# 1chizhang/OpenDCVC

Measured on AMD Instinct MI355X. Metric: 1080p YUV420 encode+decode FPS (frames/s through encode AND decode, whole job), higher is better.
Workload: dtype f16

## Files before the change

include/dcvc_amd.h:

```cpp
#ifndef DCVC_AMD_H
#define DCVC_AMD_H

#include <stddef.h>
#include <stdint.h>

#ifdef __cplusplus
extern "C" {
#endif

#define DCVC_ABI_VERSION 1

enum {
    DCVC_F16 = 0,
    DCVC_F32 = 1,
    DCVC_U8 = 2,
    DCVC_U16 = 3
};

enum {
    DCVC_EPI_BIAS = 0,
    DCVC_EPI_BIAS_QUANT = 1,
    DCVC_EPI_SHUFFLE2 = 2,
    DCVC_EPI_WSILU = 3
};

int dcvc_abi_version(void);
const char* dcvc_last_error(void);
int dcvc_device_count(void);

typedef struct dcvc_dcb dcvc_dcb;
typedef struct dcvc_conv dcvc_conv;
int dcvc_dcb_create(int dtype, int cin, int c, int shortcut, const float* adaptor_w,
                    const float* adaptor_b, const float* w1, const float* b1, const float* wd,
                    const float* bd, const float* w2, const float* b2, const float* w3,
                    const float* b3, const float* w4, const float* b4, dcvc_dcb** out);
void dcvc_dcb_destroy(dcvc_dcb* h);
size_t dcvc_dcb_scratch_bytes(const dcvc_dcb* h, int H, int W);
int dcvc_dcb_forward(const dcvc_dcb* h, const void* x0, int64_t ld0, int c0, const void* x1,
                     int64_t ld1, int c1, int H, int W, const float* quant, void* out, int64_t ldo,
                     void* scratch, void* stream);
int dcvc_dcb_forward_chained(const dcvc_dcb* h, const void* x0, int64_t ld0, int c0, const void* x1,
                             int64_t ld1, int c1, int H, int W, const float* quant, void* out,
                             int64_t ldo, void* scratch, void* stream, int head_done, int a_slot,
                             const dcvc_dcb* next);

int dcvc_dcb_forward_then_conv(const dcvc_dcb* h, const void* x0, int64_t ld0, int c0, const void* x1,
                               int64_t ld1, int c1, int H, int W, void* scratch, void* stream,
                               int head_done, int a_slot, const dcvc_conv* conv, const float* conv_quant,
                               void* conv_out, int64_t ldco);

int dcvc_dcb_profile(const dcvc_dcb* h, const void* x0, int64_t ld0, int c0, int H, int W, void* out,
                     int64_t ldo, void* scratch, void* stream, int iters, float* head_ms, float* tail_ms);
int dcvc_dcb_profile_tail(const dcvc_dcb* h, const void* x0, int64_t ld0, int c0, int H, int W, void* out,
                          int64_t ldo, void* scratch, void* stream, int iters, float* tail_ms);

int dcvc_conv_create(int dtype, int cin, int cout, int kh, int kw, int stride, int pad, int epilogue,
                     const float* w, const float* b, dcvc_conv** out);
void dcvc_conv_destroy(dcvc_conv* h);
int dcvc_conv_forward(const dcvc_conv* h, const void* x0, int64_t ld0, int c0, const void* x1,
                      int64_t ld1, int c1, int H, int W, const float* quant, void* out, int64_t ldo,
                      void* stream);
int dcvc_conv_forward_scaled(const dcvc_conv* h, const void* x0, int64_t ld0, int c0, const void* x1,
                             int64_t ld1, int c1, int H, int W, const float* in_scale, const float* quant,
                             void* out, int64_t ldo, void* stream);

int dcvc_unshuffle8(int dtype, const void* x_nchw, int C, int H, int W, void* out_hwc, int64_t ldo,
                    void* stream);
int dcvc_shuffle8_clamp(int dtype, const void* x_hwc, int64_t ld, const float* bias, int C, int H,
                        int W, int do_clamp, void* out_nchw, void* stream);
int dcvc_yuv420_to_frame(int dtype, const uint8_t* y, const uint8_t* u, const uint8_t* v, int H, int W,
                         int pad_b, int pad_r, void* out_nchw, void* stream);
int dcvc_frame_to_yuv420(int dtype, const void* x_nchw, int Hp, int Wp, int H, int W, int round_uv,
                         uint8_t* y, uint8_t* u, uint8_t* v, void* stream);
int dcvc_rgb_to_frame(int dtype, const uint8_t* rgb, int H, int W, int pad_b, int pad_r, void* out_nchw,
                      void* stream);
int dcvc_frame_to_rgb(int dtype, const void* x_nchw, int Hp, int Wp, int H, int W, void* out_chw, void* stream);
int dcvc_replicate_pad_hwc(int dtype, const void* x, int64_t ldx, int H, int W, int C, int pad_b,
                           int pad_r, void* out, int64_t ldo, void* stream);
int dcvc_scale_channels(int dtype, const void* x, int64_t ldx, const float* q, int64_t P, int C,
                        void* out, int64_t ldo, void* stream);
int dcvc_copy_channels(int dtype, const void* x, int64_t ldx, int64_t P, int C, void* out,
                       int64_t ldo, void* stream);
int dcvc_crop_hwc(int dtype, const void* x, int64_t ldx, int W, int H2, int W2, int C, void* out,
                  int64_t ldo, void* stream);

int dcvc_round_z(int dtype, void* z, int64_t ld, int H, int W, int C, int8_t* z_chw, void* stream);
int dcvc_z_from_int8(int dtype, const int8_t* z_chw, int H, int W, int C, void* out, int64_t ldo,
                     void* stream);

int dcvc_prior_enc_step(int dtype, int n_groups, int step, int q_mode, const void* y, int64_t ldy,
                        const void* qsrc, int64_t ldq, const void* scales, int64_t lds_,
                        const void* means, int64_t ldm, int H, int W, int C, float thres,
                        const void* yhat_in, int64_t ldhi, void* yhat_out, int64_t ldho,
                        int16_t* packed_chw, void* stream);
int dcvc_prior_dec_index(int dtype, int n_groups, int step, const void* scales, int64_t lds_, int H,
                         int W, int C, float thres, uint8_t* idx_chw, void* stream);
int dcvc_prior_dec_restore(int dtype, int n_groups, int step, const int8_t* sym_chw,
                           const void* means, int64_t ldm, int H, int W, int C, const void* yhat_in,
                           int64_t ldhi, void* yhat_out, int64_t ldho, void* stream);
int64_t dcvc_prior_dec_compact_ws_bytes(int H, int W, int C, int n_groups);
int dcvc_prior_dec_index_compact(int dtype, int n_groups, int step, const void* scales, int64_t lds_, int H, int W, int C,
                                 float thres, uint8_t* idx_chw, void* workspace, uint8_t* idx_host,
                                 int32_t* count_host, void* stream);
int dcvc_prior_dec_restore_compact(int dtype, int n_groups, int step, const int8_t* sym_host, const uint8_t* idx_chw,
                                   void* workspace, const void* means, int64_t ldm, int H, int W, int C,
                                   const void* yhat_in, int64_t ldhi, void* yhat_out, int64_t ldho, void* stream);
int dcvc_prior_dec_index_compact_dev(int dtype, int n_groups, int step, const void* scales, int64_t lds_, int H, int W, int C,
                                     float thres, uint8_t* idx_chw, void* workspace, uint8_t* idx_dev,
                                     int32_t* count_dev, void* stream);
int dcvc_prior_dec_restore_compact_dev(int dtype, int n_groups, int step, const int8_t* sym_dev, const uint8_t* idx_chw,
                                       void* workspace, const void* means, int64_t ldm, int H, int W, int C,
                                       const void* yhat_in, int64_t ldhi, void* yhat_out, int64_t ldho, void* stream);
int dcvc_prior_finish(int dtype, int q_mode, void* yhat, int64_t ldh, const void* qsrc, int64_t ldq,
                      int H, int W, int C, void* stream);

int dcvc_op_process_with_mask(int dtype, const void* y, const void* scales, const void* means,
                              const void* mask, float thres, void* y_res, void* y_q, void* y_hat,
                              void* s_hat, int64_t n, void* stream);
int dcvc_op_combine_for_reading_2x(int dtype, void* out, const void* x, const void* mask,
                                   int64_t half_n, void* stream);
int dcvc_op_restore_y_2x(int dtype, void* out, const void* y, const void* means, const void* mask,
                         int64_t half_n, void* stream);
int dcvc_op_restore_y_4x(int dtype, void* out, const void* y, const void* means, const void* mask,
                         int64_t quarter_n, void* stream);
int dcvc_op_build_index_dec(int dtype, uint8_t* out, uint8_t* cond_out, const void* scales,
                            float scale_min, float scale_max, float log_scale_min,
                            float log_step_recip, float skip_thres, int64_t n, void* stream);
int dcvc_op_build_index_enc(int dtype, int16_t* out, uint8_t* cond_out, const void* symbols,
                            const void* scales, float scale_min, float scale_max,
                            float log_scale_min, float log_step_recip, float skip_thres, int64_t n,
                            void* stream);
int dcvc_op_round_and_to_int8(int dtype, void* z, int8_t* z_int8, int64_t n, void* stream);
int dcvc_op_clamp_reciprocal_with_quant(int dtype, const void* q_dec, void* y, float min_val,
                                        void* q_out, int64_t n, void* stream);
int dcvc_op_add_and_multiply(int dtype, void* x0, const void* x1, const void* q, int64_t n,
                             void* stream);
int dcvc_op_bias_quant(int dtype, void* x, const void* bias, const void* quant, int C, int64_t HW,
                       void* stream);
int dcvc_op_bias_pixel_shuffle_8(int dtype, void* out, const void* x, const void* bias, int C, int H,
                                 int W, int do_clamp, void* stream);
int dcvc_op_replicate_pad(int dtype, const void* x, int C, int H, int W, int pad_b, int pad_r,
                          void* out, void* stream);
int dcvc_op_bias_wsilu_depthwise_conv2d(int dtype, const void* x, const void* weight,
                                        const void* bias, int C, int H, int W, void* out,
                                        void* stream);
int dcvc_nchw_to_hwc(int dtype, const void* x, int C, int64_t HW, void* out, int64_t ldo, void* stream);
int dcvc_hwc_to_nchw(int dtype, const void* x, int64_t ldx, int C, int64_t HW, void* out, void* stream);

typedef struct dcvc_rans_enc dcvc_rans_enc;
typedef struct dcvc_rans_dec dcvc_rans_dec;
dcvc_rans_enc* dcvc_rans_enc_create(void);
void dcvc_rans_enc_destroy(dcvc_rans_enc*);
int dcvc_rans_enc_add_cdf(dcvc_rans_enc*, const int32_t* cdf, int n, int stride,
                          const int32_t* sizes, const int32_t* offsets);
int dcvc_rans_enc_empty_cdf(dcvc_rans_enc*);
void dcvc_rans_enc_set_use_two(dcvc_rans_enc*, int two);
int dcvc_rans_enc_reset(dcvc_rans_enc*);
int dcvc_rans_enc_encode_y(dcvc_rans_enc*, const int16_t* symbols, int64_t n, int group);
int dcvc_rans_enc_encode_y_borrowed(dcvc_rans_enc*, const int16_t* symbols, int64_t n, int group);
int dcvc_rans_enc_encode_z(dcvc_rans_enc*, const int8_t* symbols, int64_t n, int group,
                           int start_offset, int per_channel_size);
int dcvc_rans_enc_flush(dcvc_rans_enc*);
int64_t dcvc_rans_enc_get_stream(dcvc_rans_enc*, const uint8_t** data);

dcvc_rans_dec* dcvc_rans_dec_create(void);
void dcvc_rans_dec_destroy(dcvc_rans_dec*);
int dcvc_rans_dec_add_cdf(dcvc_rans_dec*, const int32_t* cdf, int n, int stride,
                          const int32_t* sizes, const int32_t* offsets);
int dcvc_rans_dec_empty_cdf(dcvc_rans_dec*);
void dcvc_rans_dec_set_use_two(dcvc_rans_dec*, int two);
int dcvc_rans_dec_set_stream(dcvc_rans_dec*, const uint8_t* data, int64_t n);
int dcvc_rans_dec_decode_y(dcvc_rans_dec*, const uint8_t* indexes, int64_t n, int group);
int dcvc_rans_dec_decode_z(dcvc_rans_dec*, int64_t total, int group, int start_offset,
                           int per_channel_size);
int64_t dcvc_rans_dec_get(dcvc_rans_dec*, int8_t* out, int64_t capacity);
int dcvc_rans_dec_decode_and_get_y(dcvc_rans_dec*, const uint8_t* indexes, int64_t n, int group,
                                   int8_t* out);
int dcvc_rans_dec_decode_compact(dcvc_rans_dec*, const uint8_t* indexes, int64_t count, int group, int8_t* out);
int dcvc_rans_dec_check_end(dcvc_rans_dec*);
int64_t dcvc_rans_chunked_encode_y(dcvc_rans_enc*, const int16_t* symbols, int64_t count, int group, int log2_s,
                                   uint8_t* out, int64_t capacity);
int dcvc_rans_chunked_decode_y(dcvc_rans_dec*, const uint8_t* unit, int64_t unit_bytes, const uint8_t* indexes,
                               int64_t count, int group, int log2_s, int8_t* out);
int dcvc_pmf_to_quantized_cdf(const float* pmf, int n, int precision, uint32_t* out);

void* dcvc_host_alloc(size_t bytes);
void dcvc_host_free(void* p);
void* dcvc_host_device_ptr(void* host);
#define DCVC_COMPACT_BLOCKS 256
int dcvc_compact_symbols(const int16_t* packed, int n_per_part, int n_parts, int16_t* out_host, int32_t* counts_host,
                         int32_t* workspace, void* stream);
int dcvc_compact_symbols_dev(const int16_t* packed, int n_per_part, int n_parts, int16_t* out_dev, int32_t* counts_dev,
                             int32_t* workspace, void* stream);
#define DCVC_RANS_DEV_E_COUNT 1
#define DCVC_RANS_DEV_E_TABLE 2
#define DCVC_RANS_DEV_E_CHUNK 4
#define DCVC_RANS_DEV_E_RANGE 8
typedef struct dcvc_rans_dev dcvc_rans_dev;
int dcvc_rans_dev_create(const int32_t* cdf, int n, int stride, const int32_t* sizes, const int32_t* offsets,
                         dcvc_rans_dev** out);
void dcvc_rans_dev_destroy(dcvc_rans_dev*);
int64_t dcvc_rans_dev_enc_ws_bytes(int64_t max_symbols, int log2_s, int slot_bytes);
// ... 48 lines not shown
```

opendcvc_amd/_lib.py:

```python
import ctypes
import os
import subprocess
from ctypes import (POINTER, c_char_p, c_double, c_float, c_int, c_int8, c_int16, c_int32, c_int64, c_size_t,
                    c_uint8, c_uint32, c_uint64, c_void_p)

_HERE = os.path.dirname(os.path.abspath(__file__))
LIB_PATH = os.path.join(_HERE, os.environ.get("DCVC_AMD_LIB") or
                        ("libdcvc_amd_diag.so" if os.environ.get("DCVC_AMD_DIAG") else "libdcvc_amd.so"))

F16, F32 = 0, 1
U8 = 2
U16 = 3
SSE_BLOCKS = 1024
DIGEST_PASS_WORDS = 1 << 20
EPI_BIAS, EPI_BIAS_QUANT, EPI_SHUFFLE2, EPI_WSILU = 0, 1, 2, 3


class DcvcError(RuntimeError):
    pass


class DigestMismatch(DcvcError):

    def __init__(self, index, is_i, expected, got):
        super().__init__(f"frame {index} ({'I' if is_i else 'P'}): the decoder's reference state has digest {got:#018x}, "
                         f"the stream carries {expected:#018x}")
        self.index, self.is_i, self.expected, self.got = index, is_i, expected, got


def build(force=False):
    csrc = os.path.join(_HERE, "csrc")
    if force:
        subprocess.check_call(["make", "-C", csrc, "clean"])
    subprocess.check_call(["make", "-C", csrc, "-j8"])
    return LIB_PATH


_P = c_void_p
_I = c_int
_L = c_int64
_F = c_float

_SIGS = {
    "dcvc_abi_version": (_I, []),
    "dcvc_last_error": (c_char_p, []),
    "dcvc_device_count": (_I, []),
    "dcvc_dcb_create": (_I, [_I, _I, _I, _I] + [_P] * 12 + [POINTER(_P)]),
    "dcvc_dcb_destroy": (None, [_P]),
    "dcvc_dcb_scratch_bytes": (c_size_t, [_P, _I, _I]),
    "dcvc_dcb_forward": (_I, [_P, _P, _L, _I, _P, _L, _I, _I, _I, _P, _P, _L, _P, _P]),
    "dcvc_dcb_forward_chained": (_I, [_P, _P, _L, _I, _P, _L, _I, _I, _I, _P, _P, _L, _P, _P, _I, _I, _P]),
    "dcvc_dcb_forward_then_conv": (_I, [_P, _P, _L, _I, _P, _L, _I, _I, _I, _P, _P, _I, _I, _P, _P, _P, _L]),
    "dcvc_dcb_profile": (_I, [_P, _P, _L, _I, _I, _I, _P, _L, _P, _P, _I, POINTER(c_float), POINTER(c_float)]),
    "dcvc_dcb_profile_tail": (_I, [_P, _P, _L, _I, _I, _I, _P, _L, _P, _P, _I, POINTER(c_float)]),
    "dcvc_conv_create": (_I, [_I, _I, _I, _I, _I, _I, _I, _I, _P, _P, POINTER(_P)]),
    "dcvc_conv_destroy": (None, [_P]),
    "dcvc_conv_forward": (_I, [_P, _P, _L, _I, _P, _L, _I, _I, _I, _P, _P, _L, _P]),
    "dcvc_conv_forward_scaled": (_I, [_P, _P, _L, _I, _P, _L, _I, _I, _I, _P, _P, _P, _L, _P]),
    "dcvc_unshuffle8": (_I, [_I, _P, _I, _I, _I, _P, _L, _P]),
    "dcvc_shuffle8_clamp": (_I, [_I, _P, _L, _P, _I, _I, _I, _I, _P, _P]),
    "dcvc_yuv420_to_frame": (_I, [_I, _P, _P, _P, _I, _I, _I, _I, _P, _P]),
    "dcvc_frame_to_yuv420": (_I, [_I, _P, _I, _I, _I, _I, _I, _P, _P, _P, _P]),
    "dcvc_rgb_to_frame": (_I, [_I, _P, _I, _I, _I, _I, _P, _P]),
    "dcvc_frame_to_rgb": (_I, [_I, _P, _I, _I, _I, _I, _P, _P]),
    "dcvc_replicate_pad_hwc": (_I, [_I, _P, _L, _I, _I, _I, _I, _I, _P, _L, _P]),
    "dcvc_scale_channels": (_I, [_I, _P, _L, _P, _L, _I, _P, _L, _P]),
    "dcvc_copy_channels": (_I, [_I, _P, _L, _L, _I, _P, _L, _P]),
    "dcvc_crop_hwc": (_I, [_I, _P, _L, _I, _I, _I, _I, _P, _L, _P]),
    "dcvc_round_z": (_I, [_I, _P, _L, _I, _I, _I, _P, _P]),
    "dcvc_z_from_int8": (_I, [_I, _P, _I, _I, _I, _P, _L, _P]),
    "dcvc_prior_enc_step": (_I, [_I, _I, _I, _I, _P, _L, _P, _L, _P, _L, _P, _L, _I, _I, _I, _F, _P, _L, _P, _L, _P, _P]),
    "dcvc_prior_dec_index": (_I, [_I, _I, _I, _P, _L, _I, _I, _I, _F, _P, _P]),
    "dcvc_prior_dec_restore": (_I, [_I, _I, _I, _P, _P, _L, _I, _I, _I, _P, _L, _P, _L, _P]),
    "dcvc_prior_dec_compact_ws_bytes": (_L, [_I, _I, _I, _I]),
    "dcvc_prior_dec_index_compact": (_I, [_I, _I, _I, _P, _L, _I, _I, _I, _F, _P, _P, _P, _P, _P]),
    "dcvc_prior_dec_restore_compact": (_I, [_I, _I, _I, _P, _P, _P, _P, _L, _I, _I, _I, _P, _L, _P, _L, _P]),
    "dcvc_prior_finish": (_I, [_I, _I, _P, _L, _P, _L, _I, _I, _I, _P]),
    "dcvc_op_process_with_mask": (_I, [_I, _P, _P, _P, _P, _F, _P, _P, _P, _P, _L, _P]),
    "dcvc_op_combine_for_reading_2x": (_I, [_I, _P, _P, _P, _L, _P]),
    "dcvc_op_restore_y_2x": (_I, [_I, _P, _P, _P, _P, _L, _P]),
    "dcvc_op_restore_y_4x": (_I, [_I, _P, _P, _P, _P, _L, _P]),
    "dcvc_op_build_index_dec": (_I, [_I, _P, _P, _P, _F, _F, _F, _F, _F, _L, _P]),
    "dcvc_op_build_index_enc": (_I, [_I, _P, _P, _P, _P, _F, _F, _F, _F, _F, _L, _P]),
    "dcvc_op_round_and_to_int8": (_I, [_I, _P, _P, _L, _P]),
    "dcvc_op_clamp_reciprocal_with_quant": (_I, [_I, _P, _P, _F, _P, _L, _P]),
    "dcvc_op_add_and_multiply": (_I, [_I, _P, _P, _P, _L, _P]),
    "dcvc_op_bias_quant": (_I, [_I, _P, _P, _P, _I, _L, _P]),
    "dcvc_op_bias_pixel_shuffle_8": (_I, [_I, _P, _P, _P, _I, _I, _I, _I, _P]),
    "dcvc_op_replicate_pad": (_I, [_I, _P, _I, _I, _I, _I, _I, _P, _P]),
    "dcvc_op_bias_wsilu_depthwise_conv2d": (_I, [_I, _P, _P, _P, _I, _I, _I, _P, _P]),
    "dcvc_nchw_to_hwc": (_I, [_I, _P, _I, _L, _P, _L, _P]),
    "dcvc_hwc_to_nchw": (_I, [_I, _P, _L, _I, _L, _P, _P]),
    "dcvc_rans_enc_create": (_P, []),
    "dcvc_rans_enc_destroy": (None, [_P]),
    "dcvc_rans_enc_add_cdf": (_I, [_P, _P, _I, _I, _P, _P]),
    "dcvc_rans_enc_empty_cdf": (_I, [_P]),
    "dcvc_rans_enc_set_use_two": (None, [_P, _I]),
    "dcvc_rans_enc_reset": (_I, [_P]),
    "dcvc_rans_enc_encode_y": (_I, [_P, _P, _L, _I]),
    "dcvc_rans_enc_encode_y_borrowed": (_I, [_P, _P, _L, _I]),
    "dcvc_rans_enc_encode_z": (_I, [_P, _P, _L, _I, _I, _I]),
    "dcvc_rans_enc_flush": (_I, [_P]),
    "dcvc_rans_enc_get_stream": (_L, [_P, POINTER(_P)]),
    "dcvc_rans_dec_create": (_P, []),
    "dcvc_rans_dec_destroy": (None, [_P]),
    "dcvc_rans_dec_add_cdf": (_I, [_P, _P, _I, _I, _P, _P]),
    "dcvc_rans_dec_empty_cdf": (_I, [_P]),
    "dcvc_rans_dec_set_use_two": (None, [_P, _I]),
    "dcvc_rans_dec_set_stream": (_I, [_P, _P, _L]),
    "dcvc_rans_dec_decode_y": (_I, [_P, _P, _L, _I]),
    "dcvc_rans_dec_decode_z": (_I, [_P, _L, _I, _I, _I]),
    "dcvc_rans_dec_get": (_L, [_P, _P, _L]),
    "dcvc_rans_dec_decode_and_get_y": (_I, [_P, _P, _L, _I, _P]),
    "dcvc_rans_dec_decode_compact": (_I, [_P, _P, _L, _I, _P]),
    "dcvc_rans_dec_check_end": (_I, [_P]),
    "dcvc_pmf_to_quantized_cdf": (_I, [_P, _I, _I, _P]),
    "dcvc_rans_chunked_encode_y": (_L, [_P, _P, _L, _I, _I, _P, _L]),
    "dcvc_rans_chunked_decode_y": (_I, [_P, _P, _L, _P, _L, _I, _I, _P]),
    "dcvc_rans_dev_create": (_I, [_P, _I, _I, _P, _P, POINTER(_P)]),
    "dcvc_rans_dev_destroy": (None, [_P]),
    "dcvc_rans_dev_enc_ws_bytes": (_L, [_L, _I, _I]),
    "dcvc_rans_dev_encode_y": (_I, [_P, _P, _P, _L, _I, _I, _P, _P, _L, _P]),
    "dcvc_rans_dev_dec_ws_bytes": (_L, [_L, _I]),
    "dcvc_rans_dev_decode_y": (_I, [_P, _P, _L, _P, _P, _P, _L, _I, _P, _P, _P, _P]),
    "dcvc_prior_dec_index_compact_dev": (_I, [_I, _I, _I, _P, _L, _I, _I, _I, _F, _P, _P, _P, _P, _P]),
    "dcvc_prior_dec_restore_compact_dev": (_I, [_I, _I, _I, _P, _P, _P, _P, _L, _I, _I, _I, _P, _L, _P, _L, _P]),
    "dcvc_compact_symbols_dev": (_I, [_P, _I, _I, _P, _P, _P, _P]),
    "dcvc_host_alloc": (_P, [c_size_t]),
    "dcvc_host_free": (None, [_P]),
    "dcvc_host_device_ptr": (_P, [_P]),
    "dcvc_compact_symbols": (_I, [_P, _I, _I, _P, _P, _P, _P]),
    "dcvc_frame_to_yuv420_planes": (_I, [_I, _P, _I, _I, _I, _I, _P, _P, _P, _P]),
    "dcvc_sse": (_I, [_I, _P, _I, _P, _L, _P, _P, _P]),
    "dcvc_msssim_ws_bytes": (_L, [_I, _I]),
    "dcvc_msssim_stats": (_I, [_I, _P, _I, _P, _I, _I, c_double, _P, _P, POINTER(_I), _P]),
    "dcvc_planes_to_frame": (_I, [_I, _I, _I, _I, _I, _P, _P, _P, _L, _L, _I, _I, _I, _I, _P, _P]),
    "dcvc_frame_to_planes": (_I, [_I, _I, _I, _I, _I, _P, _I, _I, _I, _I, _P, _P, _P, _L, _L, _P]),
    "dcvc_frame_to_metric_planes": (_I, [_I, _I, _I, _P, _I, _I, _I, _I, _P, _P, _P, _P]),
    "dcvc_resize_frame": (_I, [_I, _P, _I, _I, _I, _I, _P, _I, _I, _I, _I, _P, _P, _I, _P, _P, _I, _P]),
    "dcvc_frame_analysis_ws_bytes": (_L, [_I, _I]),
    "dcvc_frame_analyze": (_I, [_I, _P, _L, _I, _I, _P, _P, _P, _P, _P]),
    "dcvc_rate_estimate_ws_bytes": (_L, [_I, _I, _I]),
    "dcvc_rate_estimate": (_I, [_P, _I, _I, _P, _I, _I, _P, _I, _I, _P, _I, _I, _I, _P, _P, _P]),
    "dcvc_state_digest_ws_bytes": (_L, [_L]),
    "dcvc_state_digest": (_I, [_P, _L, _P, c_uint64, _I, _P, _P]),
    "dcvc_copy_f32": (_I, [_P, _P, _I, _P]),
    "dcvc_memcpy_d2h": (_I, [_P, _P, c_size_t, _P]),
    "dcvc_memcpy_h2d": (_I, [_P, _P, c_size_t, _P]),
    "dcvc_stream_sync": (_I, [_P]),
}

EXPORTS = tuple(_SIGS.keys())
_lib = None


def lib():
    global _lib
    if _lib is None:
        if not os.path.exists(LIB_PATH):
            raise DcvcError(
                f"{LIB_PATH} not found: the HIP extension has not been built "
                "(run `python -c 'import __graft_entry__ as g; g.build()'` or `make -C opendcvc_amd/csrc`). "
                "There is no CPU fallback.")
        try:
            L = ctypes.CDLL(LIB_PATH)
        except OSError as e:
            raise DcvcError(f"cannot load {LIB_PATH}: {e}") from e
        for name, (res, args) in _SIGS.items():
            try:
                fn = getattr(L, name)
            except AttributeError as e:
                raise DcvcError(f"{LIB_PATH} does not export {name}") from e
            fn.restype = res
            fn.argtypes = args
        if L.dcvc_abi_version() != 1:
            raise DcvcError("libdcvc_amd.so ABI version mismatch")
        _lib = L
    return _lib


def check(rc, what=""):
    if rc is not None and rc < 0:
        msg = lib().dcvc_last_error()
        raise DcvcError(f"{what} failed ({rc}): {msg.decode() if msg else ''}")
    return rc


def require_gpu():
    n = lib().dcvc_device_count()
    if n <= 0:
        raise DcvcError("no HIP device visible: the DCVC-RT hot path needs an MI355X (no CPU fallback)")
    return n
```

opendcvc_amd/csrc/dcb_t128.hpp:

```cpp
#pragma once

namespace t128 {

typedef float floatx16 __attribute__((ext_vector_type(16)));

constexpr int TW = 16, TH = 8, M = TW * TH;
constexpr int NW = 8, NTHR = NW * 64;
constexpr int PT = M / 32;
constexpr int PTW = PT / 2;
constexpr int PAD = 8;
constexpr int VC = 64, LDV = VC + PAD;
constexpr int HALO = (TH + 2) * (TW + 2);
constexpr int DW_SLAB = 64;
constexpr int LDS_S = DW_SLAB;

constexpr int PADF = 24;

struct G128 {
    static constexpr int TW = t128::TW, TH = t128::TH, NW = t128::NW, D = 8, DW_SLAB = t128::DW_SLAB, WPS = 2;
};
struct G32 {
    static constexpr int TW = 8, TH = 4, NW = 4, D = 24 , DW_SLAB = 128, WPS = 1;
};
template <class G>
struct Geo : G {
    static constexpr int M = G::TW * G::TH, NTHR = G::NW * 64;
    static constexpr int PTW = (M / 32) / (G::NW / 4);
    static constexpr int HALO = (G::TH + 2) * (G::TW + 2);
    static constexpr int LDS_S = G::DW_SLAB;
    static_assert(M % 32 == 0 && PTW >= 1 && G::NW % 4 == 0, "tile geometry");
};

template <int C>
struct Wcfg {
    static_assert(C % 64 == 0, "DepthConvBlock widths are padded to 64");
    static constexpr int NT = C / 32;
    static constexpr int NTW = (NT + 3) / 4;
    static constexpr bool RAG = NT % 4 != 0;
    static constexpr int KS = C / 16;
    static constexpr int NCH = 2 * C / VC;
    static constexpr int F4 = 4 * NTW;
    static constexpr int LDX = C + PAD;
    static constexpr int FRAGS = KS * NTW + NCH * KS + NCH * F4;
    static constexpr int STREAM = FRAGS + PADF;
};

template <int C, class G = G128, bool HEADIN = false>
struct Cfg : Wcfg<C> {
    using GE = Geo<G>;
    using WC = Wcfg<C>;
    using WC::NT; using WC::NTW; using WC::RAG; using WC::KS; using WC::NCH; using WC::F4; using WC::LDX; using WC::FRAGS; using WC::STREAM;
    static_assert(C % G::DW_SLAB == 0, "whole depthwise slabs");
    static constexpr int D = G::D;
    static_assert(D <= PADF, "stream padding");
    static constexpr size_t slab_elems = (size_t)(HEADIN && C / G::DW_SLAB > 2 ? C / G::DW_SLAB : 2) * GE::HALO * GE::LDS_S;
    static constexpr size_t v_elems = (size_t)2 * GE::M * LDV > slab_elems ? (size_t)2 * GE::M * LDV : slab_elems;
    static constexpr size_t TAB_BYTES = (size_t)9 * C * 2 + (size_t)C * 4 + (size_t)4 * C * 4;
    static constexpr int HROWS = (GE::HALO + 31) / 32 * 32;
    static constexpr size_t HEAD_BYTES = HEADIN ? (size_t)HROWS * LDX * sizeof(half_t) : 0;
    static constexpr size_t LDS = ((size_t)GE::M * LDX + v_elems) * sizeof(half_t) + TAB_BYTES + HEAD_BYTES;
    static_assert(LDS <= 160 * 1024, "LDS budget");
    static_assert(NCH % 2 == 0 && NCH >= 4, "the chunk loop is unrolled by two");
    static_assert((2 * C) % VC == 0, "whole FFN chunks");
    static constexpr int OFF_U0 = (KS * NTW) % D;
    static constexpr int OFF_S0 = (OFF_U0 + KS) % D;
    static constexpr int OFF_ODD = (OFF_S0 + KS) % D;
    static constexpr int OFF_EVEN = (OFF_ODD + F4 + KS) % D;
    static_assert((2 * (F4 + KS)) % D == 0, "the two-step loop body must turn the ring a whole number of times");
    static constexpr int OFF_LAST = OFF_ODD;
    static constexpr int OFF_FIN = (OFF_LAST + F4) % D;
};

__device__ __forceinline__ floatx16 mfma32(const half8& a, const half8& b, const floatx16& c)
{
    return __builtin_amdgcn_mfma_f32_32x32x16_f16(a, b, c, 0, 0, 0);
}


template <int C, class G = G128, bool HEADIN = false>
__global__ __launch_bounds__(Geo<G>::NTHR, G::WPS) void dcb_tail128_kernel(TailParams p)
{
    using TR = Traits<half_t>;
    using CF = Cfg<C, G, HEADIN>;
    using GE = Geo<G>;
    constexpr int TW = GE::TW, TH = GE::TH, M = GE::M, NTHR = GE::NTHR, PTW = GE::PTW, HALO = GE::HALO, DW_SLAB = GE::DW_SLAB,
                  LDS_S = GE::LDS_S;
    constexpr int NTW = CF::NTW, KS = CF::KS, NCH = CF::NCH, D = CF::D, LDX = CF::LDX, V = 8, GC = C / V;
    extern __shared__ __attribute__((aligned(32))) char smem[];
    half_t* bufX = reinterpret_cast<half_t*>(smem);
    half_t* bufV = bufX + M * LDX;
    half_t* tabW = bufV + CF::v_elems;
    float* tabBd = reinterpret_cast<float*>(tabW + 9 * C);
    float* tabB3 = tabBd + C;
    const int tid = threadIdx.x, lane = tid & 63;
    const int wave = __builtin_amdgcn_readfirstlane(tid >> 6);
    const int cqw = wave & 3, ph = wave >> 2;
    const int pl = lane & 31, hh = lane >> 5;
    const int tiles_x = (p.W + TW - 1) / TW;
    const int ty0 = (blockIdx.x / tiles_x) * TH, tx0 = (blockIdx.x % tiles_x) * TW;
    const half_t* a = reinterpret_cast<const half_t*>(p.a);
    const half_t* ident = reinterpret_cast<const half_t*>(p.ident);
    [[maybe_unused]] unsigned long long ts0 = 0, ts1 = 0, ts2 = 0, ts3 = 0, ts4 = 0, ts5 = 0, ts6 = 0;
    [[maybe_unused]] unsigned long long td[8] = {0, 0, 0, 0, 0, 0, 0, 0};
    STAMP(ts0);

    const __amdgpu_buffer_rsrc_t wrsrc = __builtin_amdgcn_make_buffer_rsrc(
        const_cast<char*>(reinterpret_cast<const char*>(p.wt)) + (size_t)cqw * CF::STREAM * 1024, 0, CF::STREAM * 1024, 0x00020000);
    const int wlane = lane * 16;
    int woff = 0;
    auto wload = [&]() __attribute__((always_inline)) {
        typedef unsigned u32x4 __attribute__((ext_vector_type(4)));
        const u32x4 v = __builtin_amdgcn_raw_buffer_load_b128(wrsrc, wlane, woff, 0);
        woff += 1024;
        return __builtin_bit_cast(half8, v);
    };
    half8 ring[D];

    constexpr int HW_ = TW + 2, GS = DW_SLAB / V, NLD = (HALO * GS + NTHR - 1) / NTHR;
    constexpr int nslab = C / DW_SLAB;
    const half_t* wd = reinterpret_cast<const half_t*>(p.wd);
    const int dcs = (tid % GS) * V;
    typedef unsigned u32x4 __attribute__((ext_vector_type(4)));
    constexpr int OOB = 0x7FFFFFF0;
    const __amdgpu_buffer_rsrc_t arsrc = __builtin_amdgcn_make_buffer_rsrc(
        const_cast<half_t*>(a), 0, (int)((long)p.H * p.W * p.lda * 2), 0x00020000);
    int hoff[NLD];
#pragma unroll
    for (int k = 0; k < NLD; ++k) {
        const int hp = tid / GS + k * (NTHR / GS);
        const int y = ty0 - 1 + hp / HW_, x = tx0 - 1 + hp % HW_;
        hoff[k] = (hp < HALO && y >= 0 && y < p.H && x >= 0 && x < p.W) ? ((y * p.W + x) * (int)p.lda + dcs) * 2 : OOB;
#ifdef DCVC_DIAG
        if (p.ablate & 32) hoff[k] = (tid & 255) * 16;
#endif
    }
    Vec16 pre[nslab][NLD];
    auto fetch = [&](int slab) __attribute__((always_inline)) {
#pragma unroll
        for (int k = 0; k < NLD; ++k)
            pre[slab][k] = __builtin_bit_cast(Vec16, __builtin_amdgcn_raw_buffer_load_b128(arsrc, hoff[k], slab * DW_SLAB * 2, 0));
    };
    Vec16 wtap[9];
    floatx4 bd0, bd1;
    auto taps_fetch = [&](int slab) __attribute__((always_inline)) {
        const int c = slab * DW_SLAB + dcs;
#pragma unroll
        for (int t = 0; t < 9; ++t) wtap[t] = *reinterpret_cast<const Vec16*>(tabW + t * C + c);
        bd0 = *reinterpret_cast<const floatx4*>(tabBd + c);
        bd1 = *reinterpret_cast<const floatx4*>(tabBd + c + 4);
    };
    if constexpr (!HEADIN) fetch(0);
    {
        constexpr int NW16 = 9 * C * 2 / 16, NB16 = C * 4 / 16, N316 = 4 * C * 4 / 16;
        for (int i = tid; i < NW16 + NB16 + N316; i += NTHR) {
            const Vec16* src = i < NW16 ? reinterpret_cast<const Vec16*>(wd) + i
                               : i < NW16 + NB16 ? reinterpret_cast<const Vec16*>(p.bd) + (i - NW16)
                                                 : reinterpret_cast<const Vec16*>(p.b3) + (i - NW16 - NB16);
            reinterpret_cast<Vec16*>(tabW)[i] = *src;
        }
    }
    if constexpr (!HEADIN) {
#pragma unroll
        for (int sl = 1; sl < nslab; ++sl) fetch(sl);
    }
    if constexpr (HEADIN) {
        constexpr int HROWS = CF::HROWS, HT = HROWS / 32, NLX = (HROWS * GC + NTHR - 1) / NTHR;
        half_t* xs = reinterpret_cast<half_t*>(reinterpret_cast<char*>(tabW) + CF::TAB_BYTES);
        const __amdgpu_buffer_rsrc_t xrsrc = __builtin_amdgcn_make_buffer_rsrc(
            const_cast<void*>(p.hx), 0, (int)((long)p.H * p.W * p.ldhx * 2), 0x00020000);
        Vec16 xv[NLX];
#pragma unroll
        for (int k = 0; k < NLX; ++k) {
            const int it = tid + k * NTHR, hp = it / GC, c = (it % GC) * V;
            const int y = ty0 - 1 + hp / HW_, x = tx0 - 1 + hp % HW_;
            const int off = (hp < HALO && y >= 0 && y < p.H && x >= 0 && x < p.W) ? ((y * p.W + x) * (int)p.ldhx + c) * 2 : OOB;
            xv[k] = __builtin_bit_cast(Vec16, __builtin_amdgcn_raw_buffer_load_b128(xrsrc, off, 0, 0));
        }
        const __amdgpu_buffer_rsrc_t hrsrc = __builtin_amdgcn_make_buffer_rsrc(
            const_cast<char*>(reinterpret_cast<const char*>(p.hwt)) + (size_t)cqw * (KS * NTW + PADF) * 1024, 0,
            (KS * NTW + PADF) * 1024, 0x00020000);
        constexpr int NF = KS * NTW, HD = NF < D ? NF : D;
        int hoff = 0;
        auto hload = [&]() __attribute__((always_inline)) {
            typedef unsigned u32x4h __attribute__((ext_vector_type(4)));
            const u32x4h v = __builtin_amdgcn_raw_buffer_load_b128(hrsrc, wlane, hoff, 0);
            hoff += 1024;
            return __builtin_bit_cast(half8, v);
        };
#pragma unroll
        for (int k = 0; k < HD; ++k) ring[k] = hload();
#pragma unroll
        for (int k = 0; k < NLX; ++k) {
            const int it = tid + k * NTHR, hp = it / GC, c = (it % GC) * V;
            if (hp < HROWS) *reinterpret_cast<Vec16*>(xs + hp * LDX + c) = xv[k];
        }
        __syncthreads();
        floatx16 hacc[NTW][HT];
#pragma unroll
        for (int s = 0; s < KS; ++s) {
            half8 hb_[HT];
#pragma unroll
            for (int t = 0; t < HT; ++t) hb_[t] = *reinterpret_cast<const half8*>(xs + (32 * t + pl) * LDX + 8 * hh + 16 * s);
#pragma unroll
            for (int i = 0; i < NTW; ++i) {
                const int f = s * NTW + i, k = f % HD;
#pragma unroll
                for (int t = 0; t < HT; ++t) {
                    if (s == 0) {
                        floatx16 zero;
#pragma unroll
                        for (int r = 0; r < 16; ++r) zero[r] = 0.f;
                        hacc[i][t] = mfma32(ring[k], hb_[t], zero);
                    } else {
                        hacc[i][t] = mfma32(ring[k], hb_[t], hacc[i][t]);
                    }
                }
                if (f + HD < NF) ring[k] = hload();
            }
        }
#pragma unroll
        for (int i = 0; i < NTW; ++i) {
            const int chb = 32 * (cqw + 4 * i) + 4 * hh;
#pragma unroll
            for (int g = 0; g < 4; ++g) {
                const floatx4 bias = load_f4(p.hb1 + chb + 8 * g);
#pragma unroll
                for (int t = 0; t < HT; ++t) {
                    const int hp = 32 * t + pl;
                    const int y = ty0 - 1 + hp / HW_, x = tx0 - 1 + hp % HW_;
                    const bool inside = hp < HALO && y >= 0 && y < p.H && x >= 0 && x < p.W;
                    floatx4 v = {hacc[i][t][4 * g], hacc[i][t][4 * g + 1], hacc[i][t][4 * g + 2], hacc[i][t][4 * g + 3]};
                    v = v + bias;
#pragma unroll
// ... 158 lines not shown
#pragma unroll
        for (int g = 0; g < 4; ++g) {
            const floatx4 bias = ebias_get(p.b2, i, g);
#pragma unroll
            for (int t = 0; t < PTW; ++t) {
                floatx4 v = {acc[i][t][4 * g], acc[i][t][4 * g + 1], acc[i][t][4 * g + 2], acc[i][t][4 * g + 3]};
                lds_store_quad<half_t>(bufX, LDX, prow + 32 * t, chb + 8 * g, v + bias);
            }
        }
    }
    __syncthreads();
#pragma unroll
    for (int k = 0; k < NID; ++k) {
        int m, icg;
        idmap(k, m, icg);
        const half8 o = __builtin_bit_cast(half8, lds_load_vec<half_t>(bufX, LDX, m, icg)) + __builtin_bit_cast(half8, idv[k]);
        lds_store_vec<half_t>(bufX, LDX, m, icg, __builtin_bit_cast(Vec16, o));
    }
    __syncthreads();

    STAMP(ts3);
#pragma unroll
    for (int i = 0; i < NTW; ++i)
#pragma unroll
        for (int t = 0; t < PTW; ++t)
#pragma unroll
            for (int r = 0; r < 16; ++r) acc[i][t][r] = 0.f;
    floatx16 ua[PTW], ub[PTW];
    const float* b3w = tabB3 + 16 * cqw + 4 * hh;
    floatx16 biasv;
    auto bias_load = [&](int j) __attribute__((always_inline)) {
        j = j < NCH ? j : NCH - 1;
        const floatx4 l0 = load_f4(b3w + 64 * j), l1 = load_f4(b3w + 64 * j + 8);
        const floatx4 h0 = load_f4(b3w + 64 * j + 2 * C), h1 = load_f4(b3w + 64 * j + 2 * C + 8);
#pragma unroll
        for (int r = 0; r < 4; ++r) {
            biasv[r] = l0[r];
            biasv[4 + r] = l1[r];
            biasv[8 + r] = h0[r];
            biasv[12 + r] = h1[r];
        }
    };
    constexpr int NPIECE = 4 * PTW * 6;
    float ge[4], gr[4];
    floatx4 vq;
    auto gate_piece = [&](const floatx16 (&u)[PTW], half_t* vbuf, int i) __attribute__((always_inline)) {
        const int n = i / 6, phs = i % 6, t = n >> 2, g = (n >> 1) & 1, hf = n & 1;
        const float lo0 = u[t][4 * g + 2 * hf], lo1 = u[t][4 * g + 2 * hf + 1];
        const float hi0 = u[t][8 + 4 * g + 2 * hf], hi1 = u[t][8 + 4 * g + 2 * hf + 1];
        if (phs == 0) {
            ge[0] = __builtin_amdgcn_exp2f(lo0);
            ge[1] = __builtin_amdgcn_exp2f(lo1);
        } else if (phs == 1) {
            ge[2] = __builtin_amdgcn_exp2f(hi0);
            ge[3] = __builtin_amdgcn_exp2f(hi1);
        } else if (phs == 2) {
            gr[0] = __builtin_amdgcn_rcpf(1.0f + ge[0]);
            gr[1] = __builtin_amdgcn_rcpf(1.0f + ge[1]);
        } else if (phs == 3) {
            gr[2] = __builtin_amdgcn_rcpf(1.0f + ge[2]);
            gr[3] = __builtin_amdgcn_rcpf(1.0f + ge[3]);
        } else if (phs == 4) {
            vq[2 * hf] = DCVC_FMAF(hi0, gr[2], lo0 * gr[0]);
        } else {
            vq[2 * hf + 1] = DCVC_FMAF(hi1, gr[3], lo1 * gr[1]);
            if (hf == 1) lds_store_quad<half_t>(vbuf, LDV, prow + 32 * t, 16 * cqw + 8 * g + 4 * hh, vq);
        }
    };
    auto wload_ffn = [&]() __attribute__((always_inline)) {
#ifdef DCVC_DIAG
        if (p.ablate & 256) {
            typedef unsigned u32x4 __attribute__((ext_vector_type(4)));
            return __builtin_bit_cast(half8, __builtin_amdgcn_raw_buffer_load_b128(wrsrc, wlane, 0, 0));
        }
#endif
        return wload();
    };
    auto step = [&](auto G4c, auto G3c, auto GATEc, auto OFFc, const floatx16 (&ug)[PTW], floatx16 (&un)[PTW], half_t* vcur,
                    const half_t* vprev, int jb) __attribute__((always_inline)) {
        constexpr bool G4 = decltype(G4c)::value, G3 = decltype(G3c)::value, GATE = decltype(GATEc)::value;
        constexpr int OFF = decltype(OFFc)::value;
        constexpr int N4 = G4 ? 4 : 0, NS = N4 + (G3 ? KS : 0);
        constexpr int TM = N4 * NTW * PTW + (G3 ? KS * PTW : 0);
        constexpr int PPS = GATE ? (NPIECE + TM - 1) / TM : 0;
        auto load_b1 = [&](int idx, int t) __attribute__((always_inline)) {
#ifdef DCVC_DIAG
            if (p.ablate & 512) idx = idx < N4 ? 0 : N4;
#endif
            if (idx < N4) return *reinterpret_cast<const half8*>(vprev + (prow + 32 * t) * LDV + 8 * hh + idx * 16);
            return bfrag_x(t, idx - N4);
        };
        half8 bc[PTW], bn[PTW];
#pragma unroll
        for (int t = 0; t < PTW; ++t) bc[t] = load_b1(0, t);
        __builtin_amdgcn_sched_barrier(0);
        int m = 0;
#pragma unroll
        for (int idx = 0; idx < NS; ++idx) {
            const int nm = idx < N4 ? NTW * PTW : PTW;
#pragma unroll
            for (int q = 0; q < NTW * PTW; ++q) {
                if (q < nm) {
                    if (idx + 1 < NS && q < PTW) bn[q] = load_b1(idx + 1, q);
                    const int t = q % PTW;
                    if (idx < N4) {
                        const int i = q / PTW, k = (OFF + idx * NTW + i) % D;
                        acc[i][t] = mfma32(ring[k], bc[t], acc[i][t]);
                        if (t == PTW - 1) ring[k] = wload_ffn();
                    } else {
                        const int k = (OFF + N4 * NTW + (idx - N4)) % D;
                        un[t] = mfma32(ring[k], bc[t], idx == N4 ? biasv : un[t]);
                        if (t == PTW - 1) ring[k] = wload_ffn();
                        if (idx == N4 && t == PTW - 1) bias_load(jb);
                    }
                    if constexpr (GATE) {
#ifdef DCVC_DIAG
                        if (!(p.ablate & 64))
#endif
#pragma unroll
                        for (int pp = 0; pp < PPS; ++pp)
                            if (m * PPS + pp < NPIECE) gate_piece(ug, vcur, m * PPS + pp);
                    }
                    ++m;
                    __builtin_amdgcn_sched_barrier(0);
                }
            }
#pragma unroll
            for (int t = 0; t < PTW; ++t) bc[t] = bn[t];
        }
#ifdef DCVC_DIAG
        if (p.ablate & 128) return;
#endif
        if constexpr (GATE) __syncthreads();
    };
    using T_ = std::true_type;
    using F_ = std::false_type;
    half_t* vA = bufV;
    half_t* vB = bufV + M * LDV;
#define T128_OFF(x) std::integral_constant<int, CF::x>{}
    bias_load(0);
    step(F_{}, T_{}, F_{}, T128_OFF(OFF_U0), ub, ua, vA, vB, 1);
    STAMP(ts4);
    step(F_{}, T_{}, T_{}, T128_OFF(OFF_S0), ua, ub, vA, vB, 2);
    for (int j = 1; j + 2 < NCH; j += 2) {
        step(T_{}, T_{}, T_{}, T128_OFF(OFF_ODD), ub, ua, vB, vA, j + 2);
        step(T_{}, T_{}, T_{}, T128_OFF(OFF_EVEN), ua, ub, vA, vB, j + 3);
    }
    step(T_{}, F_{}, T_{}, T128_OFF(OFF_LAST), ub, ua, vB, vA, 0);
    ebias_load(p.b4);
    step(T_{}, F_{}, F_{}, T128_OFF(OFF_FIN), ub, ua, vA, vB, 0);
#undef T128_OFF

    STAMP(ts5);
    const bool fused_next = p.nwt != nullptr;
    const __amdgpu_buffer_rsrc_t nrsrc = __builtin_amdgcn_make_buffer_rsrc(
        const_cast<char*>(reinterpret_cast<const char*>(fused_next ? p.nwt : p.wt)) + (size_t)cqw * (KS * NTW + PADF) * 1024, 0,
        (KS * NTW + PADF) * 1024, 0x00020000);
    int noff = 0;
    auto nload = [&]() __attribute__((always_inline)) {
        typedef unsigned u32x4_ __attribute__((ext_vector_type(4)));
        const u32x4_ v = __builtin_amdgcn_raw_buffer_load_b128(nrsrc, wlane, noff, 0);
        noff += 1024;
        return __builtin_bit_cast(half8, v);
    };
    if (fused_next) {
#pragma unroll
        for (int k = 0; k < D; ++k) ring[k] = nload();
    }
#pragma unroll
    for (int i = 0; i < NTW; ++i) {
        if (!tile_exists(i)) continue;
        const int chb = 32 * tile_of(i) + 4 * hh;
#pragma unroll
        for (int g = 0; g < 4; ++g) {
            const floatx4 bias = ebias_get(p.b4, i, g);
#pragma unroll
            for (int t = 0; t < PTW; ++t) {
                const floatx4 o = lds_load_quad<half_t>(bufX, LDX, prow + 32 * t, chb + 8 * g);
                floatx4 v = {acc[i][t][4 * g], acc[i][t][4 * g + 1], acc[i][t][4 * g + 2], acc[i][t][4 * g + 3]};
                lds_store_quad<half_t>(bufX, LDX, prow + 32 * t, chb + 8 * g, (v + bias) + o);
            }
        }
    }
    __syncthreads();
    half_t* out = reinterpret_cast<half_t*>(p.out);
    if (out != nullptr) {
#pragma unroll
        for (int k = 0; k < NID; ++k) {
            int m, icg;
            idmap(k, m, icg);
            const int y = ty0 + m / TW, x = tx0 + m % TW;
            if (y < p.H && x < p.W) {
                const long pix = (long)y * p.W + x;
                float r[V];
                unpack16<half_t>(lds_load_vec<half_t>(bufX, LDX, m, icg), r);
                if (p.shortcut) {
                    float id[V];
                    unpack16<half_t>(*reinterpret_cast<const Vec16*>(ident + pix * p.ldi + icg), id);
#pragma unroll
                    for (int j = 0; j < V; ++j) r[j] = r[j] + id[j];
                }
                if (p.q != nullptr) {
#pragma unroll
                    for (int j = 0; j < V; ++j) r[j] = r[j] * ((icg + j) < p.c_log ? p.q[icg + j] : 1.0f);
                }
                *reinterpret_cast<Vec16*>(out + pix * p.ldo + icg) = pack16<half_t>(r);
            }
        }
    }
    STAMP(ts6);
#ifdef DCVC_DIAG
    if (p.stamps && tid == 0) {
        unsigned long long* o = p.stamps + (size_t)blockIdx.x * 16;
#pragma unroll
        for (int k = nslab + 1; k <= 4; ++k) td[k] = td[nslab < 4 ? nslab : 4];
        o[0] = ts1 - ts0;
        o[1] = ts2 - ts1;
        o[2] = ts3 - ts2;
        o[3] = ts4 - ts3;
        o[4] = ts5 - ts4;
        o[5] = ts6 - ts5;
        o[6] = ts0;
        o[7] = ts6;
        o[8] = td[0] - ts0;
        o[9] = td[1] - td[0];
        o[10] = td[2] - td[1];
        o[11] = td[3] - td[2];
        o[12] = td[4] - td[3];
        o[13] = ts1 - td[4];
    }
#endif
    if (fused_next) {
        gemm_c(nload);
        __syncthreads();
#pragma unroll
        for (int i = 0; i < NTW; ++i) {
            if (!tile_exists(i)) continue;
            const int chb = 32 * tile_of(i) + 4 * hh;
#pragma unroll
            for (int g = 0; g < 4; ++g) {
                const int ch0 = chb + 8 * g;
                const floatx4 bias = load_f4(p.nb1 + ch0);
                floatx4 qv = {1.f, 1.f, 1.f, 1.f};
                if (p.nplain && p.nq != nullptr) {
#pragma unroll
                    for (int r = 0; r < 4; ++r) qv[r] = (ch0 + r) < p.n_log ? p.nq[ch0 + r] : 1.0f;
                }
#pragma unroll
                for (int t = 0; t < PTW; ++t) {
                    floatx4 v = {acc[i][t][4 * g], acc[i][t][4 * g + 1], acc[i][t][4 * g + 2], acc[i][t][4 * g + 3]};
                    v = v + bias;
                    if (p.nplain) {
                        if (p.nq != nullptr) v = v * qv;
                    } else {
#pragma unroll
                        for (int r = 0; r < 4; ++r) v[r] = TR::gate(v[r]);
                    }
                    lds_store_quad<half_t>(bufX, LDX, prow + 32 * t, ch0, v);
                }
            }
        }
        __syncthreads();
        half_t* na = reinterpret_cast<half_t*>(p.na_out);
#pragma unroll
        for (int k = 0; k < NID; ++k) {
            int m, icg;
            idmap(k, m, icg);
            const int y = ty0 + m / TW, x = tx0 + m % TW;
            if (y < p.H && x < p.W)
                *reinterpret_cast<Vec16*>(na + ((long)y * p.W + x) * p.nlda + icg) = lds_load_vec<half_t>(bufX, LDX, m, icg);
        }
    }
#ifdef DCVC_DIAG
    if (p.stamps && tid == 0) {
        unsigned long long ts7 = 0;
        STAMP(ts7);
        p.stamps[(size_t)blockIdx.x * 16 + 14] = ts7 - ts6;
    }
#endif
}

template <int C, class G = G128>
struct HeadCfg {
    using CF = Wcfg<C>;
    static constexpr int DH = 4 * CF::NTW;
    static constexpr int KCH = 128;
    static constexpr int LDS_S = KCH + PAD;
    static constexpr size_t LDS = ((size_t)Geo<G>::M * LDS_S + (size_t)Geo<G>::M * CF::LDX) * sizeof(half_t);
};

template <int C, bool ADAPT, class G = G128>
__global__ __launch_bounds__(Geo<G>::NTHR, 1) void dcb_head128_kernel(HeadParams p)
{
    using TR = Traits<half_t>;
    using CF = Wcfg<C>;
    using HC = HeadCfg<C, G>;
    using GE = Geo<G>;
    constexpr int TW = GE::TW, TH = GE::TH, M = GE::M, NTHR = GE::NTHR, PTW = GE::PTW;
    constexpr int RPP = NTHR / 8, NPASS = M / RPP;
    static_assert(M % RPP == 0, "staging passes");
    constexpr int NTW = CF::NTW, KS = CF::KS, LDX = CF::LDX, V = 8, DH = HC::DH, KCH = HC::KCH, LDS_S = HC::LDS_S, G8 = C / 64;
    extern __shared__ __attribute__((aligned(32))) char smem[];
    half_t* bufY = reinterpret_cast<half_t*>(smem);
    half_t* bufS = bufY + M * LDX;
    const int tid = threadIdx.x, lane = tid & 63;
    const int wave = __builtin_amdgcn_readfirstlane(tid >> 6);
    const int cqw = wave & 3, ph = wave >> 2;
    const int pl = lane & 31, hh = lane >> 5;
    const int tiles_x = (p.W + TW - 1) / TW;
    const int ty0 = (blockIdx.x / tiles_x) * TH, tx0 = (blockIdx.x % tiles_x) * TW;
    const int prow = (ph * PTW) * 32 + pl;
    typedef unsigned u32x4 __attribute__((ext_vector_type(4)));
    constexpr int OOB = 0x7FFFFFF0;
    auto tile_of = [&](int i) __attribute__((always_inline)) { return cqw + 4 * i; };
    auto tile_exists = [&](int i) __attribute__((always_inline)) { return !CF::RAG || cqw + 4 * i < CF::NT; };

    int pix2[NPASS];
#pragma unroll
    for (int k = 0; k < NPASS; ++k) {
        const int m = (tid >> 3) + RPP * k;
        const int y = ty0 + m / TW, x = tx0 + m % TW;
        pix2[k] = (y < p.H && x < p.W) ? y * p.W + x : -1;
    }
    auto make_stream = [&](const void* base, int frags) __attribute__((always_inline)) {
        return __builtin_amdgcn_make_buffer_rsrc(
            const_cast<char*>(reinterpret_cast<const char*>(base)) + (size_t)cqw * (frags + PADF) * 1024, 0, (frags + PADF) * 1024,
            0x00020000);
    };
    floatx16 acc[NTW][PTW];
    half8 ring[DH];
    auto zero_all = [&]() __attribute__((always_inline)) {
#pragma unroll
        for (int i = 0; i < NTW; ++i)
#pragma unroll
            for (int t = 0; t < PTW; ++t)
#pragma unroll
                for (int r = 0; r < 16; ++r) acc[i][t][r] = 0.f;
    };
    auto gemm = [&](const half_t* X, int ldx, int nb, auto next) __attribute__((always_inline)) {
        const half_t* xb = X + prow * ldx + 8 * hh;
        half8 bc[PTW], bn[PTW];
#pragma unroll
        for (int t = 0; t < PTW; ++t) bc[t] = *reinterpret_cast<const half8*>(xb + t * 32 * ldx);
        __builtin_amdgcn_sched_barrier(0);
        for (int b = 0; b < nb; ++b) {
#pragma unroll
            for (int ss = 0; ss < 4; ++ss) {
                const int sn = (ss < 3 || b + 1 < nb) ? 4 * b + ss + 1 : 4 * b + ss;
#pragma unroll
                for (int q = 0; q < NTW * PTW; ++q) {
                    const int i = q / PTW, t = q % PTW, k = ss * NTW + i;
                    if (q < PTW) bn[q] = *reinterpret_cast<const half8*>(xb + q * 32 * ldx + sn * 16);
                    acc[i][t] = mfma32(ring[k], bc[t], acc[i][t]);
                    if (t == PTW - 1) ring[k] = next();
                    __builtin_amdgcn_sched_barrier(0);
                }
#pragma unroll
                for (int t = 0; t < PTW; ++t) bc[t] = bn[t];
            }
        }
    };
    auto store_tile = [&](void* g, long ldg) __attribute__((always_inline)) {
        half_t* gp = reinterpret_cast<half_t*>(g);
#pragma unroll
        for (int k = 0; k < NPASS * G8; ++k) {
            const int m = (tid >> 3) + RPP * (k / G8), c = ((tid & 7) + 8 * (k % G8)) * V;
            const int px = pix2[k / G8];
            if (px >= 0) *reinterpret_cast<Vec16*>(gp + (long)px * ldg + c) = *reinterpret_cast<const Vec16*>(bufY + m * LDX + c);
        }
    };
    auto epilogue = [&](const float* bias_p, bool gate) __attribute__((always_inline)) {
#pragma unroll
        for (int i = 0; i < NTW; ++i) {
            if (!tile_exists(i)) continue;
            const int chb = 32 * tile_of(i) + 4 * hh;
#pragma unroll
            for (int g = 0; g < 4; ++g) {
                const floatx4 bias = load_f4(bias_p + chb + 8 * g);
#pragma unroll
                for (int t = 0; t < PTW; ++t) {
                    floatx4 v = {acc[i][t][4 * g], acc[i][t][4 * g + 1], acc[i][t][4 * g + 2], acc[i][t][4 * g + 3]};
                    v = v + bias;
                    if (gate) {
#pragma unroll
                        for (int r = 0; r < 4; ++r) v[r] = TR::gate(v[r]);
                    }
                    lds_store_quad<half_t>(bufY, LDX, prow + 32 * t, chb + 8 * g, v);
                }
            }
        }
    };

    const __amdgpu_buffer_rsrc_t wrs = make_stream(p.w1128, KS * NTW);
    int woff = lane * 16;
    auto wnext = [&]() __attribute__((always_inline)) {
        const u32x4 v = __builtin_amdgcn_raw_buffer_load_b128(wrs, woff, 0, 0);
        woff += 1024;
        return __builtin_bit_cast(half8, v);
    };
    zero_all();
    if constexpr (ADAPT) {
        const int Kin = p.src.c0 + p.src.c1;
        const __amdgpu_buffer_rsrc_t ars = make_stream(p.wa128, (Kin / 16) * NTW);
        int aoff = lane * 16;
        auto anext = [&]() __attribute__((always_inline)) {
            const u32x4 v = __builtin_amdgcn_raw_buffer_load_b128(ars, aoff, 0, 0);
            aoff += 1024;
            return __builtin_bit_cast(half8, v);
        };
        const __amdgpu_buffer_rsrc_t rs0 = __builtin_amdgcn_make_buffer_rsrc(
            const_cast<void*>(p.src.x0), 0, (int)((long)p.H * p.W * p.src.ld0 * 2), 0x00020000);
        const __amdgpu_buffer_rsrc_t rs1 = __builtin_amdgcn_make_buffer_rsrc(
            const_cast<void*>(p.src.c1 > 0 ? p.src.x1 : p.src.x0), 0, (int)((long)p.H * p.W * (p.src.c1 > 0 ? p.src.ld1 : p.src.ld0) * 2),
            0x00020000);
        const int n0 = (p.src.c0 + KCH - 1) / KCH, nchunk = n0 + (p.src.c1 + KCH - 1) / KCH;
        u32x4 pre[2 * NPASS];
        auto fetch = [&](int i) __attribute__((always_inline)) {
            const bool s1 = i >= n0;
            const int cb = (s1 ? i - n0 : i) * KCH;
            const int left = (s1 ? p.src.c1 : p.src.c0) - cb, cnt = left < KCH ? left : KCH;
            const int ld = (int)(s1 ? p.src.ld1 : p.src.ld0);
#pragma unroll
            for (int k = 0; k < 2 * NPASS; ++k) {
                const int c = ((tid & 7) + 8 * (k & 1)) * V, px = pix2[k >> 1];
// ... 319 lines not shown
```

opendcvc_amd/csrc/dcvc_nn.hip:

```cpp
#include <algorithm>
#include <cstdio>
#include <cstdlib>
#include <functional>
#include <memory>
#include <mutex>
#include <type_traits>
#include <unordered_map>
#include <vector>

#include "common.hpp"
#include "gemm_core.hpp"

namespace {

using dcvc::round_up;

template <int MT>
struct Tile {
    static constexpr int M = 16 * MT;
    static constexpr int TW = MT >= 8 ? 16 : 8;
    static constexpr int TH = M / TW;
};

#ifndef DCVC_PF_SMALL
#define DCVC_PF_SMALL 4
#endif
template <typename T, int MT = 4>
struct Pf {
    static constexpr int value = (sizeof(T) == 2 && MT == 2) ? DCVC_PF_SMALL : 2;
};

struct SrcPair {
    const void* x0;
    long ld0;
    int c0;
    const void* x1;
    long ld1;
    int c1;
};

template <typename T>
__device__ __forceinline__ Vec16 load_src(const SrcPair& s, long pix, int c, bool valid)
{
    Vec16 v = VEC16_ZERO;
    if (valid) {
        if (c < s.c0)
            v = *reinterpret_cast<const Vec16*>(reinterpret_cast<const T*>(s.x0) + pix * s.ld0 + c);
        else
            v = *reinterpret_cast<const Vec16*>(reinterpret_cast<const T*>(s.x1) + pix * s.ld1 + (c - s.c0));
    }
    return v;
}

__device__ __forceinline__ floatx4 load_f4(const float* p) { return *reinterpret_cast<const floatx4*>(p); }

template <typename T>
__device__ __forceinline__ Vec16 scale_vec(const Vec16& v, const float* __restrict__ q, int c, int qn)
{
    constexpr int V = Traits<T>::kVec;
    float f[V];
    unpack16<T>(v, f);
#pragma unroll
    for (int j = 0; j < V; ++j) f[j] = f[j] * ((c + j) < qn ? q[c + j] : 1.0f);
    return pack16<T>(f);
}

struct HeadParams {
    SrcPair src;
    int H, W, C;
    const void* wa;
    const float* ba;
    void* ident;
    long ldi;
    const void* w1;
    const float* b1;
    void* a_out;
    long lda;
    int split;
    const void* wa128;
    const void* w1128;
};

template <typename T, int MT, int NTW, bool ADAPT>
__global__ __launch_bounds__(NTHREADS) void dcb_head_kernel(HeadParams p)
{
    using TR = Traits<T>;
    using frag_t = typename TR::frag_t;
    constexpr int M = Tile<MT>::M, TW = Tile<MT>::TW, TH = Tile<MT>::TH, V = TR::kVec, PF = Pf<T, MT>::value;
    extern __shared__ __attribute__((aligned(32))) char smem[];
    const int tid = threadIdx.x, lane = tid & 63, wave = tid >> 6;
    const int Kin = p.src.c0 + p.src.c1;
    const int C = p.C;
    const bool split = ADAPT && p.split;
    const int kstage = split ? (p.src.c0 > p.src.c1 ? p.src.c0 : p.src.c1) : Kin;
    const int ldx = (kstage > C ? kstage : C) + TR::kPad;
    const int ldy = C + TR::kPad;
    T* bufX = reinterpret_cast<T*>(smem);
    T* bufY = bufX + M * ldx;

    const int tiles_x = (p.W + TW - 1) / TW;
    const int ty0 = (blockIdx.x / tiles_x) * TH, tx0 = (blockIdx.x % tiles_x) * TW;

    auto stage = [&](int cbeg, int cnt) {
        const int G = cnt / V;
        for (int it = tid; it < M * G; it += NTHREADS) {
            const int m = it / G, c = (it - m * G) * V;
            const int y = ty0 + m / TW, x = tx0 + m % TW;
            const bool valid = (y < p.H) && (x < p.W);
            lds_store_vec<T>(bufX, ldx, m, c, load_src<T>(p.src, (long)y * p.W + x, cbeg + c, valid));
        }
    };
    stage(0, split ? p.src.c0 : Kin);
    __syncthreads();

    int tiles[NTW];
#pragma unroll
    for (int i = 0; i < NTW; ++i) tiles[i] = wave + NWAVE * i;
    const int pl = lane & 15, cq = (lane >> 4) * 4;
    floatx4 acc[MT][NTW];
    const int GC = C / V;

    if (ADAPT) {
        zero_acc(acc);
        if (split) {
            gemm_acc<T, MT, NTW, PF>(acc, bufX, ldx, p.src.c0 / KG, reinterpret_cast<const frag_t*>(p.wa), Kin / KG, 0, tiles, lane);
            __syncthreads();
            stage(p.src.c0, p.src.c1);
            __syncthreads();
            gemm_acc<T, MT, NTW, PF>(acc, bufX, ldx, p.src.c1 / KG, reinterpret_cast<const frag_t*>(p.wa), Kin / KG, p.src.c0 / KG, tiles, lane);
        } else {
            gemm_acc<T, MT, NTW, PF>(acc, bufX, ldx, Kin / KG, reinterpret_cast<const frag_t*>(p.wa), Kin / KG, 0, tiles, lane);
        }
#pragma unroll
        for (int i = 0; i < NTW; ++i) {
            const int ch0 = tiles[i] * 16 + cq;
            const floatx4 bias = load_f4(p.ba + ch0);
#pragma unroll
            for (int m = 0; m < MT; ++m) lds_store_quad<T>(bufY, ldy, m * 16 + pl, ch0, acc[m][i] + bias);
        }
        __syncthreads();
        for (int it = tid; it < M * GC; it += NTHREADS) {
            const int m = it / GC, c = (it - m * GC) * V;
            const int y = ty0 + m / TW, x = tx0 + m % TW;
            if (y < p.H && x < p.W)
                *reinterpret_cast<Vec16*>(reinterpret_cast<T*>(p.ident) + ((long)y * p.W + x) * p.ldi + c) =
                    lds_load_vec<T>(bufY, ldy, m, c);
        }
    }

    zero_acc(acc);
    if (ADAPT)
        gemm_acc<T, MT, NTW, PF>(acc, bufY, ldy, C / KG, reinterpret_cast<const frag_t*>(p.w1), C / KG, 0, tiles, lane);
    else
        gemm_acc<T, MT, NTW, PF>(acc, bufX, ldx, Kin / KG, reinterpret_cast<const frag_t*>(p.w1), Kin / KG, 0, tiles, lane);
    if (!ADAPT) __syncthreads();
#pragma unroll
    for (int i = 0; i < NTW; ++i) {
        const int ch0 = tiles[i] * 16 + cq;
        const floatx4 bias = load_f4(p.b1 + ch0);
#pragma unroll
        for (int m = 0; m < MT; ++m) {
            floatx4 v = acc[m][i] + bias;
#pragma unroll
            for (int r = 0; r < 4; ++r) v[r] = TR::gate(v[r]);
            lds_store_quad<T>(bufX, ldx, m * 16 + pl, ch0, v);
        }
    }
    __syncthreads();
    for (int it = tid; it < M * GC; it += NTHREADS) {
        const int m = it / GC, c = (it - m * GC) * V;
        const int y = ty0 + m / TW, x = tx0 + m % TW;
        if (y < p.H && x < p.W)
            *reinterpret_cast<Vec16*>(reinterpret_cast<T*>(p.a_out) + ((long)y * p.W + x) * p.lda + c) =
                lds_load_vec<T>(bufX, ldx, m, c);
    }
}

struct TailParams {
    const void* a;
    long lda;
    const void* ident;
    long ldi;
    int H, W, C, c_log;
    const void* wd;
    const float* bd;
    const void* w2;
    const float* b2;
    const void* w3;
    const float* b3;
    const void* w4;
    const float* b4;
    int shortcut;
    const float* q;
    void* out;
    long ldo;
    const void* nw1;
    const float* nb1;
    void* na_out;
    long nlda;
    int nplain;
    const float* nq;
    int n_log;
    const void* hx;
    long ldhx;
    const void* hw1;
    const float* hb1;
    const void* hwt;
    const void* wt;
    const void* nwt;
    int ablate;
    unsigned long long* stamps;
};

#ifdef DCVC_DIAG
#define ABLATED(bit) ((p.ablate & (bit)) != 0)
#define STAMP(var)                                                   \
    do {                                                             \
        if (p.stamps) {                                              \
            __builtin_amdgcn_sched_barrier(0);                       \
            var = __builtin_amdgcn_s_memtime();                      \
            __builtin_amdgcn_sched_barrier(0);                       \
        }                                                            \
    } while (0)
#else
#define ABLATED(bit) false
#define STAMP(var) \
    do {           \
    } while (0)
#endif

template <typename T>
__host__ __device__ constexpr int dw_slab_max() { return sizeof(T) == 2 ? 128 : 64; }

template <int MT, int NTW, int NW>
struct TailCfg {
    static constexpr bool two_per_cu = (MT <= 4 && NTW * NW <= 16);
    static constexpr int NTV = (two_per_cu || NW == 8) ? 1 : 2;
    static constexpr int waves_per_simd = (two_per_cu ? 2 : 1) * NW / 4;
};

template <typename T, int MT, int NTV, int NW>
struct TailLds {
    using TR = Traits<T>;
    static constexpr int M = Tile<MT>::M;
    static constexpr int VC = NW * NTV * 16;
    static constexpr int HALO = (Tile<MT>::TH + 2) * (Tile<MT>::TW + 2);
    static constexpr int HPASS = (HALO + M - 1) / M;
    static constexpr int lds_slab = dw_slab_max<T>() + TR::kPad;
    static constexpr int ldv = VC + TR::kPad;
    static constexpr size_t v_elems = (size_t)M * ldv > (size_t)HALO * lds_slab ? (size_t)M * ldv : (size_t)HALO * lds_slab;
    static size_t bytes(int C, bool headin = false)
    {
        const size_t halo_elems = (size_t)HPASS * M * (C + TR::kPad);
        return ((size_t)M * (C + TR::kPad) + (headin && halo_elems > v_elems ? halo_elems : v_elems)) * sizeof(T);
    }
};

template <typename T, int MT, int NTW, int NW, bool RAG = false, bool HEADIN = false>
__global__ __launch_bounds__(NW * 64, (TailCfg<MT, NTW, NW>::waves_per_simd)) void dcb_tail_kernel(TailParams p)
{
    using TR = Traits<T>;
    using frag_t = typename TR::frag_t;
    constexpr int NTV = TailCfg<MT, NTW, NW>::NTV;
    constexpr int NTHREADS_ = NW * 64;
    using LD = TailLds<T, MT, NTV, NW>;
    constexpr int M = Tile<MT>::M, TW = Tile<MT>::TW, TH = Tile<MT>::TH, V = TR::kVec;
    constexpr int PF = Pf<T, MT>::value;
    constexpr int PF3 = PF;
    constexpr int VC = NW * NTV * 16;
    static_assert(VC == LD::VC, "chunk width");
    extern __shared__ __attribute__((aligned(32))) char smem[];
    const int tid = threadIdx.x, lane = tid & 63, wave = tid >> 6;
    const int C = p.C;
    const int ldx = C + TR::kPad;
    constexpr int ldv = LD::ldv;
    T* bufX = reinterpret_cast<T*>(smem);
    T* bufV = bufX + M * ldx;

    const int tiles_x = (p.W + TW - 1) / TW;
    const int ty0 = (blockIdx.x / tiles_x) * TH, tx0 = (blockIdx.x % tiles_x) * TW;
    const T* a = reinterpret_cast<const T*>(p.a);
    const T* ident = reinterpret_cast<const T*>(p.ident);
    const int GC = C / V;
    [[maybe_unused]] unsigned long long ts0 = 0, ts1 = 0, ts2 = 0, ts3 = 0, ts4 = 0, tg3 = 0, tep = 0, tg4 = 0, tt = 0, tt2 = 0;
    STAMP(ts0);
    const int pl = lane & 15, cq = (lane >> 4) * 4;
    int tiles[NTW], wtiles[NTW];
#pragma unroll
    for (int i = 0; i < NTW; ++i) {
        tiles[i] = wave + NW * i;
        wtiles[i] = RAG ? min(tiles[i], C / 16 - 1) : tiles[i];
    }
    auto tile_exists = [&](int i) { return !RAG || tiles[i] < C / 16; };
    WPre<T, NTW, PF> pre2;
    if constexpr (!HEADIN)
        gemm_prefetch<T, NTW, PF>(pre2, C / KG, reinterpret_cast<const frag_t*>(p.w2), C / KG, 0, wtiles, lane);

    if constexpr (HEADIN) {
        constexpr int HW_ = TW + 2, HALO = LD::HALO, HROWS = LD::HPASS * M;
        const T* hx = reinterpret_cast<const T*>(p.hx);
        for (int it = tid; it < HROWS * GC; it += NTHREADS_) {
            const int hp = it / GC, c = (it - hp * GC) * V;
            const int y = ty0 - 1 + hp / HW_, x = tx0 - 1 + hp % HW_;
            Vec16 v = VEC16_ZERO;
            if (hp < HALO && y >= 0 && y < p.H && x >= 0 && x < p.W)
                v = *reinterpret_cast<const Vec16*>(hx + ((long)y * p.W + x) * p.ldhx + c);
            lds_store_vec<T>(bufV, ldx, hp, c, v);
        }
        __syncthreads();
        floatx4 hacc[LD::HPASS][MT][NTW];
#pragma unroll
        for (int ps = 0; ps < LD::HPASS; ++ps) {
            zero_acc(hacc[ps]);
            gemm_acc<T, MT, NTW, PF>(hacc[ps], bufV + ps * M * ldx, ldx, C / KG, reinterpret_cast<const frag_t*>(p.hw1), C / KG, 0,
                                     wtiles, lane);
        }
        __syncthreads();
#pragma unroll
        for (int i = 0; i < NTW; ++i) {
            const int ch0 = tiles[i] * 16 + cq;
            const floatx4 bias = load_f4(p.hb1 + wtiles[i] * 16 + cq);
            if (tile_exists(i)) {
#pragma unroll
                for (int ps = 0; ps < LD::HPASS; ++ps)
#pragma unroll
                    for (int m = 0; m < MT; ++m) {
                        const int hp = ps * M + m * 16 + pl;
                        const int y = ty0 - 1 + hp / HW_, x = tx0 - 1 + hp % HW_;
                        const bool inside = hp < HALO && y >= 0 && y < p.H && x >= 0 && x < p.W;
                        floatx4 v = hacc[ps][m][i] + bias;
#pragma unroll
                        for (int r = 0; r < 4; ++r) v[r] = inside ? TR::gate(v[r]) : 0.f;
                        lds_store_quad<T>(bufV, ldx, hp, ch0, v);
                    }
            }
        }
        gemm_prefetch<T, NTW, PF>(pre2, C / KG, reinterpret_cast<const frag_t*>(p.w2), C / KG, 0, wtiles, lane);
        __syncthreads();
    }

    {
        constexpr int DW_SLAB = (!RAG && dw_slab_max<T>() == 128 && (NTW * NW) % 8 == 0) ? 128 : 64;
        constexpr int HW_ = TW + 2, HALO = LD::HALO, GS = DW_SLAB / V, lds_s = LD::lds_slab;
        constexpr int NLD = (HALO * GS + NTHREADS_ - 1) / NTHREADS_;
        const T* wd = reinterpret_cast<const T*>(p.wd);
        const int nslab = C / DW_SLAB;
        const int tap_ld = HEADIN ? ldx : lds_s;
        Vec16 pre[HEADIN ? 1 : NLD];
        auto fetch = [&](int slab) {
            if constexpr (!HEADIN) {
#pragma unroll
                for (int k = 0; k < NLD; ++k) {
                    const int it = tid + k * NTHREADS_;
                    Vec16 v = VEC16_ZERO;
                    if (it < HALO * GS) {
                        const int hp = it / GS, c = slab * DW_SLAB + (it - hp * GS) * V;
                        const int y = ty0 - 1 + hp / HW_, x = tx0 - 1 + hp % HW_;
                        if (y >= 0 && y < p.H && x >= 0 && x < p.W && !ABLATED(1))
                            v = *reinterpret_cast<const Vec16*>(a + ((long)y * p.W + x) * p.lda + c);
                    }
                    pre[k] = v;
                }
            }
        };
        fetch(0);
        for (int slab = 0; slab < nslab; ++slab) {
// ... 378 lines not shown
#pragma unroll
            for (int u = 0; u < U; ++u) {
                const int it = it0 + u * NTHREADS;
                const int hp = it / G, c = (it - hp * G) * TR::kVec;
                if (p.in_q != nullptr) v[u] = scale_vec<T>(v[u], p.in_q, c, p.in_qn);
                if (it < total) lds_store_vec<T>(bufX, ldx, hp, c, v[u]);
            }
        }
        __syncthreads();
#pragma unroll
        for (int m = 0; m < MT; ++m) {
            const int pix = m * 16 + (lane & 15);
            xrow[m] = bufX + ((pix / TW) * p.stride * HT_W + (pix % TW) * p.stride) * ldx + (lane >> 4) * 8;
        }
    }
    const int pass_lo = p.split_n ? (int)blockIdx.y : 0, pass_hi = p.split_n ? (int)blockIdx.y + 1 : passes;
    for (int pass = pass_lo; pass < pass_hi; ++pass) {
        int tiles[NTW];
        bool tvalid[NTW];
#pragma unroll
        for (int i = 0; i < NTW; ++i) {
            const int t = pass * NWAVE * NTW + wave + NWAVE * i;
            tvalid[i] = t < ntiles;
            tiles[i] = tvalid[i] ? t : ntiles - 1;
        }
        floatx4 acc[MT][NTW];
        zero_acc(acc);
        if (taps == 1) {
            gemm_acc<T, MT, NTW, PF>(acc, bufX, ldx, kgin, reinterpret_cast<const frag_t*>(p.w), kgin, 0, tiles, lane);
        } else if constexpr (HALO) {
            gemm_taps<T, MT, NTW, PF>(acc, xrow, ldx, taps, p.KW, HT_W, kgin, reinterpret_cast<const frag_t*>(p.w), tiles, lane);
        } else {
            for (int tap = 0; tap < taps; ++tap) {
                __syncthreads();
                stage(tap);
                __syncthreads();
                gemm_acc<T, MT, NTW, PF>(acc, bufX, ldx, kgin, reinterpret_cast<const frag_t*>(p.w), taps * kgin,
                                         tap * kgin, tiles, lane);
            }
        }
#pragma unroll
        for (int i = 0; i < NTW; ++i) {
            if (!tvalid[i]) continue;
            const int ch0 = tiles[i] * 16 + cq;
            const floatx4 bias = load_f4(p.b + ch0);
            floatx4 qv = {1.f, 1.f, 1.f, 1.f};
            if (p.epi == DCVC_EPI_BIAS_QUANT) {
#pragma unroll
                for (int r = 0; r < 4; ++r) qv[r] = (ch0 + r) < p.n_log ? p.q[ch0 + r] : 1.0f;
            }
            int sdy = 0, sdx = 0, sch0 = ch0;
            if (p.epi == DCVC_EPI_SHUFFLE2) {
                const int s = ch0 / p.cs_p;
                sch0 = ch0 - s * p.cs_p;
                sdy = s >> 1;
                sdx = s & 1;
            }
#pragma unroll
            for (int m = 0; m < MT; ++m) {
                const int row = m * 16 + pl;
                const int oy = ty0 + row / TW, ox = tx0 + row % TW;
                if (oy >= p.Ho || ox >= p.Wo) continue;
                floatx4 v = acc[m][i] + bias;
                if (p.epi == DCVC_EPI_BIAS_QUANT) v = v * qv;
                if (p.epi == DCVC_EPI_WSILU) {
#pragma unroll
                    for (int r = 0; r < 4; ++r) v[r] = TR::wsilu(v[r]);
                }
                if (p.epi == DCVC_EPI_SHUFFLE2)
                    global_store_quad<T>(out + ((long)(2 * oy + sdy) * (2 * p.Wo) + (2 * ox + sdx)) * p.ldo + sch0, v);
                else
                    global_store_quad<T>(out + ((long)oy * p.Wo + ox) * p.ldo + ch0, v);
            }
        }
    }
}

struct DevBuf {
    void* p = nullptr;
    ~DevBuf()
    {
        if (p) (void)hipFree(p);
    }
    int upload(const void* src, size_t bytes)
    {
        if (hipMalloc(&p, bytes ? bytes : 16) != hipSuccess) {
            p = nullptr;
            dcvc::set_error("hipMalloc(%zu) failed", bytes);
            return dcvc::E_MEM;
        }
        if (bytes && hipMemcpy(p, src, bytes, hipMemcpyHostToDevice) != hipSuccess) {
            dcvc::set_error("hipMemcpy H2D failed");
            return dcvc::E_HIP;
        }
        return 0;
    }
};

using Mat = std::function<float(int, int)>;
using Taps = std::function<float(int, int, int)>;

template <typename T>
int pack_upload(DevBuf& dst, int Np, int Kp, const Mat& get)
{
    const int kgs = Kp / KG, nt = Np / 16;
    std::vector<T> buf((size_t)nt * kgs * 64 * 8);
    for (int t = 0; t < nt; ++t)
        for (int g = 0; g < kgs; ++g)
            for (int lane = 0; lane < 64; ++lane) {
                const int r = lane & 15, q = lane >> 4;
                for (int j = 0; j < 8; ++j) {
                    const int k = g * KG + (sizeof(T) == 2 ? 8 * q + j : 4 * j + q);
                    buf[(((size_t)t * kgs + g) * 64 + lane) * 8 + j] = (T)get(t * 16 + r, k);
                }
            }
    return dst.upload(buf.data(), buf.size() * sizeof(T));
}

int pack_any(int dtype, DevBuf& dst, int Np, int Kp, const Mat& get)
{
    return dtype == DCVC_F16 ? pack_upload<half_t>(dst, Np, Kp, get) : pack_upload<float>(dst, Np, Kp, get);
}

int upload_f32(DevBuf& dst, int n, const std::function<float(int)>& get)
{
    std::vector<float> v(n);
    for (int i = 0; i < n; ++i) v[i] = get(i);
    return dst.upload(v.data(), v.size() * sizeof(float));
}

template <typename T>
int upload_T(DevBuf& dst, int n, const std::function<float(int)>& get)
{
    std::vector<T> v(n);
    for (int i = 0; i < n; ++i) v[i] = (T)get(i);
    return dst.upload(v.data(), v.size() * sizeof(T));
}


}

struct dcvc_dcb {
    int dtype, cin, c, cin_p, c_p, shortcut, adapt;
    DevBuf wa, ba, w1, b1, wd, bd, w2, b2, w3, b3, w4, b4;
    DevBuf wa_t128;
    DevBuf w1_t128;
    DevBuf wt128;
};

struct dcvc_conv {
    int dtype, cin, cout, cin_p, n_p, cs_p, kh, kw, stride, pad, epi;
    DevBuf w, b;
    DevBuf w_t128;
    DevBuf w_c128[2];
    DevBuf w_s2;
};

namespace {

template <typename T, int MT>
size_t head_lds(int kstage, int c, bool adapt)
{
    const int kx = kstage > c ? kstage : c;
    return (size_t)Tile<MT>::M * ((kx + Traits<T>::kPad) + (adapt ? c + Traits<T>::kPad : 0)) * sizeof(T);
}
template <typename K>
int set_lds(K kernel, size_t bytes)
{
    if (bytes > 160 * 1024) {
        dcvc::set_error("kernel needs %zu bytes of LDS (> 160 KiB)", bytes);
        return dcvc::E_ARG;
    }
    if (bytes > 64 * 1024) {
        static std::mutex mu;
        static std::unordered_map<const void*, size_t> granted;
        const void* key = reinterpret_cast<const void*>(kernel);
        std::lock_guard<std::mutex> lk(mu);
        size_t& have = granted[key];
        if (have < bytes) {
            DCVC_HIP(hipFuncSetAttribute(key, hipFuncAttributeMaxDynamicSharedMemorySize, (int)bytes));
            have = bytes;
        }
    }
    return 0;
}


template <typename F, typename R>
void put_frag(half_t* o, F&& W, R&& row, int s)
{
    for (int l = 0; l < 64; ++l)
        for (int j = 0; j < 8; ++j) o[l * 8 + j] = (half_t)W(row(l & 31), 16 * s + 8 * (l >> 5) + j);
}

template <int C>
int pack_t128(DevBuf& dst, const Mat& W2, const Mat& W3, const Mat& W4)
{
    using CF = t128::Wcfg<C>;
    std::vector<half_t> buf((size_t)4 * CF::STREAM * 512, (half_t)0.f);
    for (int wave = 0; wave < 4; ++wave) {
        size_t f = 0;
        auto next = [&] { return &buf[((size_t)wave * CF::STREAM + f++) * 512]; };
        auto tile = [&](int i) { return [=](int r) { return 32 * (wave + 4 * i) + r; }; };
        auto g3 = [&](int j) {
            for (int s = 0; s < CF::KS; ++s)
                put_frag(next(), W3, [&](int r) { return (r < 16 ? 0 : 2 * C - 16) + 64 * j + 16 * wave + r; }, s);
        };
        auto g4 = [&](int j) {
            for (int s4 = 0; s4 < 4; ++s4)
                for (int i = 0; i < CF::NTW; ++i) put_frag(next(), W4, tile(i), 4 * j + s4);
        };
        for (int s = 0; s < CF::KS; ++s)
            for (int i = 0; i < CF::NTW; ++i) put_frag(next(), W2, tile(i), s);
        g3(0);
        for (int j = 0; j < CF::NCH; ++j) {
            if (j >= 1) g4(j - 1);
            if (j + 1 < CF::NCH) g3(j + 1);
        }
        g4(CF::NCH - 1);
        if (f != (size_t)CF::FRAGS) {
            dcvc::set_error("pack_t128: %zu fragments packed, %d expected", f, CF::FRAGS);
            return dcvc::E_ARG;
        }
    }
    return dst.upload(buf.data(), buf.size() * sizeof(half_t));
}

inline bool t128_width_ok(int c_p) { return c_p == 128 || c_p == 256 || c_p == 320 || c_p == 384 || c_p == 512; }

inline int pack_quarters(DevBuf& dst, int nsl, int ntw, int taps, int ks, int padf, const Taps& W)
{
    const int LEN = taps * ks * ntw + padf;
    std::vector<half_t> buf((size_t)nsl * 4 * LEN * 512, (half_t)0.f);
    for (int q = 0; q < nsl * 4; ++q) {
        half_t* o = &buf[(size_t)q * LEN * 512];
        for (int tap = 0; tap < taps; ++tap)
            for (int s = 0; s < ks; ++s)
                for (int i = 0; i < ntw; ++i, o += 512)
                    put_frag(o, [&](int n, int k) { return W(n, tap, k); },
                             [&](int r) { return (q / 4) * 128 * ntw + 32 * (q % 4 + 4 * i) + r; }, s);
    }
    return dst.upload(buf.data(), buf.size() * sizeof(half_t));
}

template <typename F>
int visit_t128_width(int c_p, F&& f)
{
    switch (c_p) {
    case 128: return f(std::integral_constant<int, 128>());
    case 256: return f(std::integral_constant<int, 256>());
    case 320: return f(std::integral_constant<int, 320>());
    case 384: return f(std::integral_constant<int, 384>());
    case 512: return f(std::integral_constant<int, 512>());
    default: dcvc::set_error("no fragment-stream form for width %d", c_p); return dcvc::E_ARG;
    }
}

inline int pack_t128_matrix(DevBuf& dst, int c_p, int Kp, const Mat& W)
{
    return visit_t128_width(c_p, [&](auto w) {
        return pack_quarters(dst, 1, t128::Wcfg<decltype(w)::value>::NTW, 1, Kp / 16, t128::PADF, [&](int n, int, int k) { return W(n, k); });
    });
}

struct Switches {
    bool t128, t32, h128, c128;
#ifdef DCVC_DIAG
    int mt, conv_mt, ablate;
    bool stamps;
#endif
};

static const Switches& switches()
{
    static const Switches sw = [] {
        auto on = [](const char* name) { const char* v = getenv(name); return !(v && atoi(v) == 0); };
        auto num = [](const char* name) { const char* v = getenv(name); return v ? atoi(v) : 0; };
        Switches s{};
        s.t128 = on("DCVC_T128");
        s.t32 = on("DCVC_T32");
        s.h128 = on("DCVC_H128");
        s.c128 = on("DCVC_C128");
#ifdef DCVC_DIAG
        s.mt = num("DCVC_MT");
        s.conv_mt = num("DCVC_CONV_MT");
        s.ablate = num("DCVC_ABLATE");
        s.stamps = getenv("DCVC_STAMPS") != nullptr;
#endif
        (void)num;
        return s;
    }();
    return sw;
}

constexpr int tile_grid(int H, int W, int th, int tw) { return ((H + th - 1) / th) * ((W + tw - 1) / tw); }

template <typename K, typename P>
int launch_kernel(K kernel, dim3 grid, int threads, size_t lds, hipStream_t st, const P& p)
{
    int rc = set_lds(kernel, lds);
    if (rc) return rc;
    hipLaunchKernelGGL(kernel, grid, dim3(threads), lds, st, p);
    return 0;
}

#ifdef DCVC_DIAG
static int stamp_medians(unsigned long long* d, int grid, int per, const char* const* names, const char* tag, int& calls,
                         hipStream_t st, std::vector<unsigned long long>& hs, bool& printed)
{
    DCVC_HIP(hipStreamSynchronize(st));
    hs.resize((size_t)grid * per);
    DCVC_HIP(hipMemcpy(hs.data(), d, hs.size() * 8, hipMemcpyDeviceToHost));
    (void)hipFree(d);
    printed = calls++ % 16 == 15;
    if (!printed) return 0;
    fprintf(stderr, "[%s]", tag);
    for (int k = 0; k < per; ++k) {
        if (!names[k]) continue;
        std::vector<unsigned long long> v(grid);
        for (int b = 0; b < grid; ++b) v[b] = hs[(size_t)b * per + k];
        std::sort(v.begin(), v.end());
        fprintf(stderr, " %s=%llu", names[k], v[grid / 2]);
    }
    return 0;
}

template <int C, class G, bool HEADIN>
int stamped_tail128(TailParams tp, int grid, size_t lds, hipStream_t st)
{
    DCVC_HIP(hipMalloc(&tp.stamps, (size_t)grid * 16 * sizeof(unsigned long long)));
    int rc = launch_kernel(t128::dcb_tail128_kernel<C, G, HEADIN>, dim3(grid), t128::Geo<G>::NTHR, lds, st, tp);
    if (rc) return rc;
    const char* names[16] = {"loads+dw", "gemm2", "o_pass", "u0", "ffn", "r+store", nullptr, nullptr, "dw:issue+stage0",
                             "barrier0", "slab0", "slab1", "slab2", "slab3", "fused", nullptr};
    for (int k = C / G::DW_SLAB; k < 4; ++k) names[10 + k] = nullptr;
    char tag[64];
    snprintf(tag, sizeof tag, "t128 stamps C=%d tile=%d grid=%d", C, t128::Geo<G>::M, grid);
    static int calls = 0;
    std::vector<unsigned long long> hs;
    bool printed = false;
    rc = stamp_medians(tp.stamps, grid, 16, names, tag, calls, st, hs, printed);
    if (rc || !printed) return rc;
    std::vector<unsigned long long> du(grid);
    for (int b = 0; b < grid; ++b) du[b] = hs[(size_t)b * 16 + 7] - hs[(size_t)b * 16 + 6];
    std::sort(du.begin(), du.end());
    fprintf(stderr, " | wg total min/med/max %llu %llu %llu\n", du[0], du[grid / 2], du[grid - 1]);
    return 0;
}

template <int MT, typename K>
int stamped_tail(K kernel, int threads, TailParams tp, int grid, size_t lds, hipStream_t st)
{
    DCVC_HIP(hipMalloc(&tp.stamps, (size_t)grid * 8 * sizeof(unsigned long long)));
    int rc = launch_kernel(kernel, dim3(grid), threads, lds, st, tp);
    if (rc) return rc;
    const char* names[8] = {"dw", "gemm2", "o_pass", "gemm3", "ffn_epi", "gemm4", "final", "total"};
    char tag[64];
    snprintf(tag, sizeof tag, "stamps C=%d MT=%d grid=%d", tp.C, MT, grid);
    static int calls = 0;
    std::vector<unsigned long long> hs;
    bool printed = false;
    rc = stamp_medians(tp.stamps, grid, 8, names, tag, calls, st, hs, printed);
    if (rc || !printed) return rc;
    fprintf(stderr, "\n");
    if (tp.ablate & 16) {
        unsigned long long t0 = ~0ull, t1 = 0;
        for (int b = 0; b < grid; ++b) {
            t0 = std::min(t0, hs[(size_t)b * 8]);
            t1 = std::max(t1, hs[(size_t)b * 8 + 1]);
        }
        std::vector<unsigned long long> s(grid), e(grid), du(grid);
        for (int b = 0; b < grid; ++b) {
            s[b] = hs[(size_t)b * 8] - t0;
            e[b] = hs[(size_t)b * 8 + 1] - t0;
            du[b] = hs[(size_t)b * 8 + 7];
        }
        std::sort(s.begin(), s.end());
        std::sort(e.begin(), e.end());
        std::sort(du.begin(), du.end());
        fprintf(stderr, "[span %llu] start min/med/p90/max %llu %llu %llu %llu | end med/p90/max %llu %llu %llu | dur min/med/p90/max %llu %llu %llu %llu\n",
                t1 - t0, s[0], s[grid / 2], s[grid * 9 / 10], s[grid - 1], e[grid / 2], e[grid * 9 / 10],
                e[grid - 1], du[0], du[grid / 2], du[grid * 9 / 10], du[grid - 1]);
    }
    return 0;
}
#endif

template <int C, class G = t128::G128, bool HEADIN = false>
int launch_tail128(const TailParams& tp, int H, int W, hipStream_t st)
{
    const int grid = tile_grid(H, W, G::TH, G::TW);
    const size_t lds = t128::Cfg<C, G, HEADIN>::LDS;
#ifdef DCVC_DIAG
    if (switches().stamps) return stamped_tail128<C, G, HEADIN>(tp, grid, lds, st);
#endif
    return launch_kernel(t128::dcb_tail128_kernel<C, G, HEADIN>, dim3(grid), t128::Geo<G>::NTHR, lds, st, tp);
}

template <typename T, int MT, int NTW, int NW, bool RAG = false, bool HEADIN = false>
int launch_tail(const TailParams& tp, int grid, int C, hipStream_t st)
{
    const size_t lds = TailLds<T, MT, TailCfg<MT, NTW, NW>::NTV, NW>::bytes(C, HEADIN);
#ifdef DCVC_DIAG
    if (switches().stamps) return stamped_tail<MT>(dcb_tail_kernel<T, MT, NTW, NW, RAG, HEADIN>, NW * 64, tp, grid, lds, st);
#endif
    return launch_kernel(dcb_tail_kernel<T, MT, NTW, NW, RAG, HEADIN>, dim3(grid), NW * 64, lds, st, tp);
}

struct ChainArgs {
    int head_done = 0, a_slot = 0;
    int separate_head = 0;
    const dcvc_dcb* next = nullptr;
    const dcvc_conv* conv = nullptr;
    const float* conv_q = nullptr;
    void* conv_out = nullptr;
    int64_t ldco = 0;
};

static int pick_mt_f16(int H, int W)
{
#ifdef DCVC_DIAG
    if (switches().mt == 2 || switches().mt == 4) return switches().mt;
#endif
    return (long)H * W >= 12000 ? 4 : 2;
}

constexpr bool has_tail128(bool f16, int mt, int ntw, bool headin)
{
    return f16 && (mt == 4 ? !headin && (ntw == 4 || ntw == 5 || ntw == 6)
                           : headin ? (ntw == 2 || ntw == 4) : (ntw == 4 || ntw == 6 || ntw == 8));
}
constexpr bool has_head128(bool f16, int mt, int ntw)
{
    return f16 && (mt == 4 ? (ntw == 4 || ntw == 5 || ntw == 6) : (ntw == 4 || ntw == 6 || ntw == 8));
}
constexpr bool has_tail_headin(bool f16, int mt, int ntw) { return f16 && mt == 2 && (ntw <= 4 || ntw == 6); }

struct TailForm {
    int ntw, nw;
    bool rag;
};
constexpr TailForm tail_form(bool f16, int ntw)
{
    return !f16 ? TailForm{ntw, 4, false} : ntw == 5 ? TailForm{3, 8, true}
                                          : ntw >= 6 && ntw % 2 == 0 ? TailForm{ntw / 2, 8, false} : TailForm{ntw, 4, false};
}

struct DcbPlan {
    enum class Head { none, head128, head } head = Head::none;
    bool head_adapt = false;
    bool head_t32 = false;
    enum class Tail { tail128, tail } tail = Tail::tail;
    bool headin = false;
    int mt = 2, ntw = 1;
    TailForm form{1, 4, false};
    const void* nwt = nullptr;
};

static DcbPlan plan_dcb(const dcvc_dcb* h, const SrcPair& src, int H, int W, const ChainArgs& ch)
{
    const Switches& sw = switches();
    const bool f16 = h->dtype == DCVC_F16;
    DcbPlan pl;
    pl.mt = f16 ? pick_mt_f16(H, W) : 2;
    pl.ntw = h->c_p / 64;
    const int mt = pl.mt, ntw = pl.ntw;
    pl.nwt = ch.next ? ch.next->w1_t128.p : ch.conv ? ch.conv->w_t128.p : nullptr;
    const bool t128 = sw.t128 && h->wt128.p != nullptr && (pl.nwt != nullptr || (!ch.next && !ch.conv));
    const bool own_head = !ch.head_done && !ch.separate_head && !h->adapt && src.c1 == 0;

    if (has_tail128(f16, mt, ntw, true) && t128 && sw.t32 && h->w1_t128.p != nullptr && own_head) {
        pl.tail = DcbPlan::Tail::tail128;
        pl.headin = true;
    } else if (has_tail128(f16, mt, ntw, false) && t128 && (mt == 4 || sw.t32)) {
        pl.tail = DcbPlan::Tail::tail128;
    } else {
        pl.tail = DcbPlan::Tail::tail;
        pl.headin = has_tail_headin(f16, mt, ntw) && own_head;
        pl.form = tail_form(f16, ntw);
    }

    const int kin = src.c0 + src.c1;
    if (ch.head_done || pl.headin) {
        pl.head = DcbPlan::Head::none;
    } else if (sw.t128 && sw.h128 && has_head128(f16, mt, ntw) && (mt == 4 || pl.tail == DcbPlan::Tail::tail128) &&
               h->w1_t128.p != nullptr &&
               (h->adapt ? (h->wa_t128.p != nullptr && src.c0 % 64 == 0 && src.c1 % 64 == 0 && kin == h->cin_p)
                         : (src.c1 == 0 && src.c0 == ntw * 64))) {
        pl.head = DcbPlan::Head::head128;
        pl.head_adapt = h->adapt;
    } else {
        pl.head = DcbPlan::Head::head;
        pl.head_adapt = h->adapt;
        const int kstage = src.c1 > 0 ? std::max(src.c0, src.c1) : kin;
        pl.head_t32 = h->adapt && mt == 4 && head_lds<half_t, 4>(kstage, h->c_p, true) > 80 * 1024;
    }
    return pl;
}

static int not_built(const char* what, const DcbPlan& pl)
{
    dcvc::set_error("%s is not instantiated for mt %d, ntw %d", what, pl.mt, pl.ntw);
    return dcvc::E_ARG;
}

template <typename T, int MT, int NTW>
int launch_dcb(const DcbPlan& pl, const dcvc_dcb* h, const SrcPair& src, int H, int W, const float* quant, void* out,
               int64_t ldo, void* scratch, hipStream_t st, hipEvent_t* ev, const ChainArgs& ch)
{
    constexpr bool f16 = sizeof(T) == 2;
    using G = typename std::conditional<MT == 4, t128::G128, t128::G32>::type;
    const int C = h->c_p;
    const int grid = tile_grid(H, W, Tile<MT>::TH, Tile<MT>::TW);
    const size_t P = (size_t)H * W;
    T* slots = reinterpret_cast<T*>(scratch);
    T* a_buf = slots + (size_t)(ch.a_slot & 1) * P * C;
    T* a_next = slots + (size_t)((ch.a_slot & 1) ^ 1) * P * C;
    T* id_buf = slots + 2 * P * C;
    HeadParams hp{};
    hp.src = src;
    hp.H = H;
    hp.W = W;
    hp.C = C;
    hp.wa = h->wa.p;
    hp.ba = (const float*)h->ba.p;
    hp.ident = id_buf;
    hp.ldi = C;
    hp.w1 = h->w1.p;
    hp.b1 = (const float*)h->b1.p;
    hp.a_out = a_buf;
    hp.lda = C;
    hp.split = src.c1 > 0;
    hp.wa128 = h->wa_t128.p;
    hp.w1128 = h->w1_t128.p;
    TailParams tp{};
    tp.a = a_buf;
    tp.lda = C;
    tp.ident = h->adapt ? (const void*)id_buf : src.x0;
    tp.ldi = h->adapt ? C : src.ld0;
    tp.H = H;
    tp.W = W;
    tp.C = C;
    tp.c_log = h->c;
    tp.wd = h->wd.p;
    tp.bd = (const float*)h->bd.p;
    tp.w2 = h->w2.p;
    tp.b2 = (const float*)h->b2.p;
    tp.w3 = h->w3.p;
    tp.b3 = (const float*)h->b3.p;
    tp.w4 = h->w4.p;
    tp.b4 = (const float*)h->b4.p;
    tp.shortcut = h->shortcut;
    tp.q = quant;
    tp.out = out;
    tp.ldo = ldo;
    tp.hx = src.x0;
    tp.ldhx = src.ld0;
    tp.hw1 = h->w1.p;
    tp.hb1 = (const float*)h->b1.p;
    tp.hwt = h->w1_t128.p;
    tp.wt = h->wt128.p;
    tp.nwt = pl.nwt;
    if (ch.next) {
        tp.nw1 = ch.next->w1.p;
        tp.nb1 = (const float*)ch.next->b1.p;
        tp.na_out = a_next;
        tp.nlda = C;
    } else if (ch.conv) {
        tp.nw1 = ch.conv->w.p;
        tp.nb1 = (const float*)ch.conv->b.p;
        tp.na_out = ch.conv_out;
        tp.nlda = ch.ldco;
        tp.nplain = 1;
        tp.nq = ch.conv_q;
        tp.n_log = ch.conv->cout;
    }
#ifdef DCVC_DIAG
    tp.ablate = switches().ablate;
#endif

    if (ev) DCVC_HIP(hipEventRecord(ev[0], st));
    int rc = 0;
    if (pl.head == DcbPlan::Head::head128) {
        if constexpr (has_head128(f16, MT, NTW)) {
            const dim3 g128(tile_grid(H, W, G::TH, G::TW));
            const size_t lds = t128::HeadCfg<NTW * 64, G>::LDS;
            rc = pl.head_adapt ? launch_kernel(t128::dcb_head128_kernel<NTW * 64, true, G>, g128, t128::Geo<G>::NTHR, lds, st, hp)
                               : launch_kernel(t128::dcb_head128_kernel<NTW * 64, false, G>, g128, t128::Geo<G>::NTHR, lds, st, hp);
        } else {
            rc = not_built("dcb_head128_kernel", pl);
        }
    } else if (pl.head == DcbPlan::Head::head) {
        const int kstage = pl.head_adapt && hp.split ? std::max(src.c0, src.c1) : src.c0 + src.c1;
        if (!pl.head_adapt) {
            rc = launch_kernel(dcb_head_kernel<T, MT, NTW, false>, dim3(grid), NTHREADS, head_lds<T, MT>(kstage, C, false), st, hp);
        } else if (pl.head_t32) {
            const int grid2 = tile_grid(H, W, Tile<2>::TH, Tile<2>::TW);
            rc = launch_kernel(dcb_head_kernel<T, 2, NTW, true>, dim3(grid2), NTHREADS, head_lds<T, 2>(kstage, C, true), st, hp);
        } else {
            rc = launch_kernel(dcb_head_kernel<T, MT, NTW, true>, dim3(grid), NTHREADS, head_lds<T, MT>(kstage, C, true), st, hp);
        }
    }
    if (rc) return rc;
    DCVC_LAUNCH_CHECK();
    if (ev) DCVC_HIP(hipEventRecord(ev[1], st));

    if (pl.tail == DcbPlan::Tail::tail128) {
        if (pl.headin) {
            if constexpr (has_tail128(f16, MT, NTW, true)) rc = launch_tail128<NTW * 64, G, true>(tp, H, W, st);
            else rc = not_built("dcb_tail128_kernel<..., HEADIN>", pl);
        } else {
            if constexpr (has_tail128(f16, MT, NTW, false)) rc = launch_tail128<NTW * 64, G>(tp, H, W, st);
            else rc = not_built("dcb_tail128_kernel", pl);
        }
    } else {
        constexpr TailForm F = tail_form(f16, NTW);
        if (pl.headin) {
            if constexpr (has_tail_headin(f16, MT, NTW)) rc = launch_tail<T, MT, F.ntw, F.nw, F.rag, true>(tp, grid, C, st);
            else rc = not_built("dcb_tail_kernel<..., HEADIN>", pl);
        } else {
            rc = launch_tail<T, MT, F.ntw, F.nw, F.rag>(tp, grid, C, st);
        }
    }
    if (rc) return rc;
    DCVC_LAUNCH_CHECK();
    if (ev) DCVC_HIP(hipEventRecord(ev[2], st));
    return 0;
}

template <typename T, int MT>
int dispatch_dcb(const DcbPlan& pl, const dcvc_dcb* h, const SrcPair& src, int H, int W, const float* quant, void* out,
                 int64_t ldo, void* scratch, hipStream_t st, hipEvent_t* ev, const ChainArgs& ch)
{
    switch (pl.ntw) {
    case 1: return launch_dcb<T, MT, 1>(pl, h, src, H, W, quant, out, ldo, scratch, st, ev, ch);
    case 2: return launch_dcb<T, MT, 2>(pl, h, src, H, W, quant, out, ldo, scratch, st, ev, ch);
    case 3: return launch_dcb<T, MT, 3>(pl, h, src, H, W, quant, out, ldo, scratch, st, ev, ch);
    case 4: return launch_dcb<T, MT, 4>(pl, h, src, H, W, quant, out, ldo, scratch, st, ev, ch);
    case 5: return launch_dcb<T, MT, 5>(pl, h, src, H, W, quant, out, ldo, scratch, st, ev, ch);
    case 6: return launch_dcb<T, MT, 6>(pl, h, src, H, W, quant, out, ldo, scratch, st, ev, ch);
    case 8: return launch_dcb<T, MT, 8>(pl, h, src, H, W, quant, out, ldo, scratch, st, ev, ch);
    default: dcvc::set_error("DepthConvBlock width %d not instantiated", h->c_p); return dcvc::E_ARG;
    }
}

static int run_dcb(const dcvc_dcb* h, const SrcPair& src, int H, int W, const float* quant, void* out, int64_t ldo,
                   void* scratch, hipStream_t st, hipEvent_t* ev, ChainArgs ch = ChainArgs())
{
    const DcbPlan pl = plan_dcb(h, src, H, W, ch);
    if (h->dtype != DCVC_F16) return dispatch_dcb<float, 2>(pl, h, src, H, W, quant, out, ldo, scratch, st, ev, ch);
    if (pl.mt == 2) return dispatch_dcb<half_t, 2>(pl, h, src, H, W, quant, out, ldo, scratch, st, ev, ch);
    return dispatch_dcb<half_t, 4>(pl, h, src, H, W, quant, out, ldo, scratch, st, ev, ch);
}

template <typename T, int MT, int NTW>
int launch_conv(const ConvParams& cp, hipStream_t st)
{
    const int grid = tile_grid(cp.Ho, cp.Wo, Tile<MT>::TH, Tile<MT>::TW);
    const size_t row = (size_t)(cp.src.c0 + cp.src.c1 + Traits<T>::kPad) * sizeof(T);
    size_t lds = (size_t)Tile<MT>::M * row;
    ConvParams p = cp;
    if (cp.KH * cp.KW > 1) {
        const size_t halo = (size_t)((Tile<MT>::TH - 1) * cp.stride + cp.KH) * ((Tile<MT>::TW - 1) * cp.stride + cp.KW) * row;
        p.halo = cp.stride == 1 && halo <= 96 * 1024;
        if (p.halo) lds = halo;
    }
    const int passes = (cp.N / 16 + NWAVE * NTW - 1) / (NWAVE * NTW);
    p.split_n = passes > 1 && grid < 400;
    const dim3 g(grid, p.split_n ? passes : 1);
    int rc = p.halo ? launch_kernel(conv_kernel<T, MT, NTW, true>, g, NTHREADS, lds, st, p)
                    : launch_kernel(conv_kernel<T, MT, NTW, false>, g, NTHREADS, lds, st, p);
    if (rc) return rc;
    DCVC_LAUNCH_CHECK();
    return 0;
}

template <typename T, int MT>
int dispatch_conv(int ntw, const ConvParams& cp, hipStream_t st)
{
    if (ntw == 2) return launch_conv<T, MT, 2>(cp, st);
    if (ntw == 3) return launch_conv<T, MT, 3>(cp, st);
    return launch_conv<T, MT, 4>(cp, st);
}

struct ConvPlan {
    enum class Kind { s2_t32, c3_t128, conv } kind = Kind::conv;
    int ntw = 2;
    int mt = 2;
};

static ConvPlan plan_conv(const dcvc_conv* h, const ConvParams& cp)
{
    const Switches& sw = switches();
    ConvPlan pl;
    if (h->dtype == DCVC_F16 && h->w_s2.p != nullptr && sw.c128 && cp.src.c1 == 0 && (long)cp.Ho * cp.Wo < 12000) {
        pl.kind = ConvPlan::Kind::s2_t32;
        pl.ntw = cp.N / 128;
    } else if (h->dtype == DCVC_F16 && h->w_c128[0].p != nullptr && sw.c128 && cp.src.c1 == 0 && cp.in_q == nullptr) {
        const int tiles = tile_grid(cp.H, cp.W, t128::TH, t128::TW);
        pl.kind = ConvPlan::Kind::c3_t128;
        pl.ntw = tiles * (cp.N / 256) <= 256 ? 2 : 1;
    } else {
        const int nt = cp.N / 16;
        pl.ntw = nt <= 8 ? 2 : nt <= 12 ? 3 : 4;
        pl.mt = h->dtype != DCVC_F16 ? 2 : (long)cp.Ho * cp.Wo >= 12000 ? 4 : 2;
#ifdef DCVC_DIAG
        if (h->dtype == DCVC_F16 && (sw.conv_mt == 2 || sw.conv_mt == 4 || sw.conv_mt == 8)) pl.mt = sw.conv_mt;
#endif
    }
    return pl;
}

static int run_conv(const dcvc_conv* h, const ConvParams& cp, hipStream_t st)
{
    const ConvPlan pl = plan_conv(h, cp);
    int rc = 0;
    switch (pl.kind) {
    case ConvPlan::Kind::s2_t32: {
        t128::ConvS2Params p{};
        p.x = cp.src.x0;
        p.ldx = cp.src.ld0;
        p.H = cp.H;
        p.W = cp.W;
        p.Ho = cp.Ho;
        p.Wo = cp.Wo;
        p.kin = cp.src.c0;
        p.k = cp.KH;
        p.pad = cp.pad;
        p.wt = h->w_s2.p;
        p.b = cp.b;
        p.in_q = cp.in_q;
        p.in_qn = cp.in_qn;
        p.out = cp.out;
        p.ldo = cp.ldo;
        const size_t lds = t128::conv_s2_lds(p.kin, p.k, pl.ntw);
        const dim3 g(tile_grid(cp.Ho, cp.Wo, t128::S2_TH, t128::S2_TW));
        rc = pl.ntw == 2 ? launch_kernel(t128::conv_s2_t32_kernel<2>, g, 256, lds, st, p)
                         : launch_kernel(t128::conv_s2_t32_kernel<1>, g, 256, lds, st, p);
        break;
    }
    case ConvPlan::Kind::c3_t128: {
        t128::Conv128Params p{};
        p.x = cp.src.x0;
        p.ldx = cp.src.ld0;
        p.H = cp.H;
        p.W = cp.W;
        p.kin = cp.src.c0;
        p.wt = h->w_c128[pl.ntw - 1].p;
        p.b = cp.b;
        p.out = cp.out;
        p.ldo = cp.ldo;
        p.shuffle = cp.epi == DCVC_EPI_SHUFFLE2;
        p.cs_p = cp.cs_p;
        const size_t lds = t128::conv128_lds(p.kin, pl.ntw);
        const dim3 g(tile_grid(cp.H, cp.W, t128::TH, t128::TW), cp.N / (128 * pl.ntw));
        rc = pl.ntw == 2 ? launch_kernel(t128::conv3x3_t128_kernel<2>, g, t128::NTHR, lds, st, p)
                         : launch_kernel(t128::conv3x3_t128_kernel<1>, g, t128::NTHR, lds, st, p);
        break;
    }
    case ConvPlan::Kind::conv:
        if (h->dtype != DCVC_F16) return dispatch_conv<float, 2>(pl.ntw, cp, st);
#ifdef DCVC_DIAG
        if (pl.mt == 8) return dispatch_conv<half_t, 8>(pl.ntw, cp, st);
#endif
        return pl.mt == 4 ? dispatch_conv<half_t, 4>(pl.ntw, cp, st) : dispatch_conv<half_t, 2>(pl.ntw, cp, st);
    }
    if (rc) return rc;
    DCVC_LAUNCH_CHECK();
    return 0;
}

static int check_src(const char* who, const SrcPair& s, int cin_p, bool two_ok, int dtype, int H, int W, bool head_done = false)
{
    DCVC_REQUIRE(H > 0 && W > 0, "%s: empty input %dx%d", who, H, W);
    DCVC_REQUIRE(s.c0 % 32 == 0 && s.c1 % 32 == 0 && s.c0 + s.c1 == cin_p,
                 "%s: input channels %d+%d do not match the layer (%d physical)", who, s.c0, s.c1, cin_p);
    DCVC_REQUIRE((s.x1 != nullptr) == (s.c1 > 0), "%s: x1/c1 mismatch", who);
    DCVC_REQUIRE(two_ok || s.c1 == 0, "%s: a block without adaptor takes a single source", who);
    DCVC_REQUIRE(!head_done || !two_ok, "%s: a block with adaptor computes its own head", who);
    DCVC_REQUIRE(s.ld0 >= s.c0 && (s.c1 == 0 || s.ld1 >= s.c1), "%s: input row stride too small", who);
    const size_t es = dcvc::elem_size(dtype);
    DCVC_REQUIRE(((uintptr_t)s.x0 % 16) == 0 && (s.ld0 * es) % 16 == 0 &&
                     (s.c1 == 0 || (((uintptr_t)s.x1 % 16) == 0 && (s.ld1 * es) % 16 == 0)),
                 "%s: inputs must be 16-byte aligned", who);
    return 0;
}

}

extern "C" {

int dcvc_dcb_create(int dtype, int cin, int c, int shortcut, const float* adaptor_w, const float* adaptor_b,
                    const float* w1, const float* b1, const float* wd, const float* bd, const float* w2,
                    const float* b2, const float* w3, const float* b3, const float* w4, const float* b4,
                    dcvc_dcb** out)
{
    DCVC_REQUIRE(out && w1 && b1 && wd && bd && w2 && b2 && w3 && b3 && w4 && b4, "dcvc_dcb_create: null weight pointer");
    DCVC_REQUIRE(dtype == DCVC_F16 || dtype == DCVC_F32, "dcvc_dcb_create: bad dtype %d", dtype);
    DCVC_REQUIRE(c > 0 && cin > 0 && (adaptor_w != nullptr || cin == c), "dcvc_dcb_create: cin %d != c %d needs an adaptor", cin, c);
    std::unique_ptr<dcvc_dcb> h(new dcvc_dcb());
    h->dtype = dtype;
    h->cin = cin;
    h->c = c;
    h->shortcut = shortcut ? 1 : 0;
    h->adapt = adaptor_w != nullptr;
    const int Cp = h->c_p = round_up(c, 64);
    const int Kp = h->cin_p = h->adapt ? round_up(cin, 32) : Cp;
    const int C = c;
    const float ka = dtype == DCVC_F16 ? Traits<half_t>::kAct : 1.0f;
    auto u_row = [&](int n) { const int half = n / (2 * Cp), cc = n % (2 * Cp); return cc < 2 * C ? half * 2 * C + cc : -1; };
    const Mat WA = [&](int n, int k) { return (n < C && k < cin) ? adaptor_w[(size_t)n * cin + k] : 0.f; };
    const Mat W1 = [&](int n, int k) { return (n < C && k < C) ? ka * w1[(size_t)n * C + k] : 0.f; };
    const Mat W2 = [&](int n, int k) { return (n < C && k < C) ? w2[(size_t)n * C + k] : 0.f; };
    const Mat W3 = [&](int n, int k) { const int rr = u_row(n); return (rr >= 0 && k < C) ? ka * w3[(size_t)rr * C + k] : 0.f; };
    const Mat W4 = [&](int n, int k) { return (n < C && k < 2 * C) ? w4[(size_t)n * 2 * C + k] / ka : 0.f; };
    int rc = 0;
    if (h->adapt) {
        rc |= pack_any(dtype, h->wa, Cp, Kp, WA);
        rc |= upload_f32(h->ba, Cp, [&](int n) { return n < C ? adaptor_b[n] : 0.f; });
    }
    rc |= pack_any(dtype, h->w1, Cp, Cp, W1);
    rc |= upload_f32(h->b1, Cp, [&](int n) { return n < C ? ka * b1[n] : 0.f; });
    auto dwget = [&](int i) { const int t = i / Cp, ch = i % Cp; return ch < C ? wd[(size_t)ch * 9 + t] / ka : 0.f; };
    rc |= dtype == DCVC_F16 ? upload_T<half_t>(h->wd, 9 * Cp, dwget) : upload_T<float>(h->wd, 9 * Cp, dwget);
    rc |= upload_f32(h->bd, Cp, [&](int n) { return n < C ? bd[n] : 0.f; });
    rc |= pack_any(dtype, h->w2, Cp, Cp, W2);
    rc |= upload_f32(h->b2, Cp, [&](int n) { return n < C ? b2[n] : 0.f; });
    rc |= pack_any(dtype, h->w3, 4 * Cp, Cp, W3);
    rc |= upload_f32(h->b3, 4 * Cp, [&](int n) { const int rr = u_row(n); return rr >= 0 ? ka * b3[rr] : 0.f; });
    rc |= pack_any(dtype, h->w4, Cp, 2 * Cp, W4);
    rc |= upload_f32(h->b4, Cp, [&](int n) { return n < C ? b4[n] : 0.f; });
    if (rc == 0 && dtype == DCVC_F16 && t128_width_ok(Cp)) {
        if (h->adapt && Kp % 64 == 0) rc |= pack_t128_matrix(h->wa_t128, Cp, Kp, WA);
        rc |= pack_t128_matrix(h->w1_t128, Cp, Cp, W1);
        rc |= visit_t128_width(Cp, [&](auto w) { return pack_t128<decltype(w)::value>(h->wt128, W2, W3, W4); });
    }
    if (rc) return rc < 0 ? rc : dcvc::E_MEM;
    *out = h.release();
    return 0;
}

void dcvc_dcb_destroy(dcvc_dcb* h) { delete h; }

size_t dcvc_dcb_scratch_bytes(const dcvc_dcb* h, int H, int W)
{
    if (!h) return 0;
    return (size_t)H * W * h->c_p * dcvc::elem_size(h->dtype) * 3;
}

int dcvc_dcb_forward(const dcvc_dcb* h, const void* x0, int64_t ld0, int c0, const void* x1, int64_t ld1, int c1,
                     int H, int W, const float* quant, void* out, int64_t ldo, void* scratch, void* stream)
{
    return dcvc_dcb_forward_chained(h, x0, ld0, c0, x1, ld1, c1, H, W, quant, out, ldo, scratch, stream, 0, 0, nullptr);
}

int dcvc_dcb_forward_chained(const dcvc_dcb* h, const void* x0, int64_t ld0, int c0, const void* x1, int64_t ld1, int c1,
                             int H, int W, const float* quant, void* out, int64_t ldo, void* scratch, void* stream,
                             int head_done, int a_slot, const dcvc_dcb* next)
{
    DCVC_REQUIRE(h && x0 && out && scratch, "dcvc_dcb_forward: null pointer");
    if (next)
        DCVC_REQUIRE(!next->adapt && next->c_p == h->c_p && next->dtype == h->dtype && !quant && !h->shortcut,
                     "dcvc_dcb_forward_chained: cannot fuse the next block's head (needs same width and type, no "
                     "adaptor there, no shortcut / quant step here)");
    const SrcPair src{x0, (long)ld0, c0, x1, (long)ld1, c1};
    if (int rc = check_src("dcvc_dcb_forward", src, h->cin_p, h->adapt != 0, h->dtype, H, W, head_done != 0)) return rc;
    DCVC_REQUIRE(ldo >= h->c_p, "dcvc_dcb_forward: output row stride too small");
    hipStream_t st = (hipStream_t)stream;
    ChainArgs ch;
    ch.head_done = head_done;
    ch.a_slot = a_slot;
    ch.next = next;
    return run_dcb(h, src, H, W, quant, out, ldo, scratch, st, nullptr, ch);
}

int dcvc_dcb_forward_then_conv(const dcvc_dcb* h, const void* x0, int64_t ld0, int c0, const void* x1, int64_t ld1, int c1,
                               int H, int W, void* scratch, void* stream, int head_done, int a_slot,
                               const dcvc_conv* conv, const float* conv_quant, void* conv_out, int64_t ldco)
{
    DCVC_REQUIRE(h && x0 && scratch && conv && conv_out, "dcvc_dcb_forward_then_conv: null pointer");
    DCVC_REQUIRE(!h->shortcut, "dcvc_dcb_forward_then_conv: a block with shortcut cannot feed a fused conv");
    DCVC_REQUIRE(conv->dtype == h->dtype && conv->kh == 1 && conv->kw == 1 && conv->stride == 1 && conv->pad == 0 &&
                     conv->cin_p == h->c_p && conv->n_p == h->c_p && conv->cin == h->c &&
                     (conv->epi == DCVC_EPI_BIAS || conv->epi == DCVC_EPI_BIAS_QUANT),
                 "dcvc_dcb_forward_then_conv: the conv must be 1x1, stride 1, of the block's width (%d -> %d given, block %d), "
                 "epilogue bias or bias*quant", conv->cin, conv->cout, h->c);
    DCVC_REQUIRE((conv->epi == DCVC_EPI_BIAS_QUANT) == (conv_quant != nullptr), "dcvc_dcb_forward_then_conv: quant vector / epilogue mismatch");
    const SrcPair src{x0, (long)ld0, c0, x1, (long)ld1, c1};
    if (int rc = check_src("dcvc_dcb_forward_then_conv", src, h->cin_p, h->adapt != 0, h->dtype, H, W, head_done != 0)) return rc;
    DCVC_REQUIRE(ldco >= h->c_p && ((uintptr_t)conv_out % 16) == 0 && (ldco * dcvc::elem_size(h->dtype)) % 16 == 0,
                 "dcvc_dcb_forward_then_conv: output row stride too small or not 16-byte aligned");
    ChainArgs ch;
    ch.head_done = head_done;
    ch.a_slot = a_slot;
    ch.conv = conv;
    ch.conv_q = conv_quant;
    ch.conv_out = conv_out;
    ch.ldco = ldco;
    return run_dcb(h, src, H, W, nullptr, nullptr, 0, scratch, (hipStream_t)stream, nullptr, ch);
}

int dcvc_dcb_profile(const dcvc_dcb* h, const void* x0, int64_t ld0, int c0, int H, int W, void* out, int64_t ldo,
                     void* scratch, void* stream, int iters, float* head_ms, float* tail_ms)
{
    DCVC_REQUIRE(h && x0 && out && scratch && head_ms && tail_ms && iters > 0, "dcvc_dcb_profile: bad arguments");
    DCVC_REQUIRE(c0 == h->cin_p && ld0 >= c0 && ldo >= h->c_p, "dcvc_dcb_profile: shape mismatch");
    SrcPair src{x0, (long)ld0, c0, nullptr, 0, 0};
    hipStream_t st = (hipStream_t)stream;
    std::vector<hipEvent_t> ev((size_t)iters * 3);
    for (auto& e : ev) DCVC_HIP(hipEventCreate(&e));
    int rc = 0;
    for (int i = 0; i < iters && rc == 0; ++i)
        rc = run_dcb(h, src, H, W, nullptr, out, ldo, scratch, st, &ev[3 * i]);
    if (rc == 0) {
        DCVC_HIP(hipStreamSynchronize(st));
        double th = 0, tt = 0;
        for (int i = 0; i < iters; ++i) {
            float a = 0, b = 0;
            DCVC_HIP(hipEventElapsedTime(&a, ev[3 * i], ev[3 * i + 1]));
            DCVC_HIP(hipEventElapsedTime(&b, ev[3 * i + 1], ev[3 * i + 2]));
            th += a;
            tt += b;
        }
        *head_ms = (float)(th / iters);
        *tail_ms = (float)(tt / iters);
    }
    for (auto& e : ev) (void)hipEventDestroy(e);
    return rc;
}

int dcvc_dcb_profile_tail(const dcvc_dcb* h, const void* x0, int64_t ld0, int c0, int H, int W, void* out, int64_t ldo,
                          void* scratch, void* stream, int iters, float* tail_ms)
{
    DCVC_REQUIRE(h && x0 && out && scratch && tail_ms && iters > 0, "dcvc_dcb_profile_tail: bad arguments");
    DCVC_REQUIRE(c0 == h->cin_p && ld0 >= c0 && ldo >= h->c_p && !h->adapt, "dcvc_dcb_profile_tail: shape mismatch or block with adaptor");
    SrcPair src{x0, (long)ld0, c0, nullptr, 0, 0};
    hipStream_t st = (hipStream_t)stream;
    hipEvent_t e0, e1;
    DCVC_HIP(hipEventCreate(&e0));
    DCVC_HIP(hipEventCreate(&e1));
    ChainArgs first;
    first.separate_head = 1;
    int rc = run_dcb(h, src, H, W, nullptr, out, ldo, scratch, st, nullptr, first);
    ChainArgs tail_only;
    tail_only.head_done = 1;
    if (rc == 0) rc = hipEventRecord(e0, st) == hipSuccess ? 0 : dcvc::E_HIP;
    for (int i = 0; i < iters && rc == 0; ++i) rc = run_dcb(h, src, H, W, nullptr, out, ldo, scratch, st, nullptr, tail_only);
    if (rc == 0) {
        float ms = 0;
        DCVC_HIP(hipEventRecord(e1, st));
        DCVC_HIP(hipStreamSynchronize(st));
        DCVC_HIP(hipEventElapsedTime(&ms, e0, e1));
        *tail_ms = ms / iters;
    }
    (void)hipEventDestroy(e0);
    (void)hipEventDestroy(e1);
    return rc;
}

int dcvc_conv_create(int dtype, int cin, int cout, int kh, int kw, int stride, int pad, int epilogue,
                     const float* w, const float* b, dcvc_conv** out)
{
    DCVC_REQUIRE(out && w && b, "dcvc_conv_create: null pointer");
    DCVC_REQUIRE(dtype == DCVC_F16 || dtype == DCVC_F32, "dcvc_conv_create: bad dtype %d", dtype);
    DCVC_REQUIRE(kh >= 1 && kh <= 3 && kw >= 1 && kw <= 3 && stride >= 1 && stride <= 2 && pad >= 0 && pad <= 1,
                 "dcvc_conv_create: unsupported geometry k=%dx%d s=%d p=%d", kh, kw, stride, pad);
    DCVC_REQUIRE(epilogue >= DCVC_EPI_BIAS && epilogue <= DCVC_EPI_WSILU, "dcvc_conv_create: bad epilogue %d", epilogue);
    DCVC_REQUIRE(epilogue != DCVC_EPI_SHUFFLE2 || cout % 4 == 0, "dcvc_conv_create: shuffle needs cout %% 4 == 0");
    std::unique_ptr<dcvc_conv> h(new dcvc_conv());
    h->dtype = dtype;
    h->cin = cin;
    h->cout = cout;
    h->kh = kh;
    h->kw = kw;
    h->stride = stride;
    h->pad = pad;
    h->epi = epilogue;
    const int Kp = h->cin_p = round_up(cin, 32);
    const int taps = kh * kw;
    int Np;
    std::function<int(int)> to_log;
    if (epilogue == DCVC_EPI_SHUFFLE2) {
        const int cs = cout / 4, csp = h->cs_p = round_up(cs, 32);
        Np = 4 * csp;
        to_log = [=](int n) { const int s = n / csp, cc = n % csp; return cc < cs ? cc * 4 + s : -1; };
    } else {
        h->cs_p = 0;
        Np = round_up(cout, 32);
        to_log = [=](int n) { return n < cout ? n : -1; };
    }
    h->n_p = Np;
    const Taps WC = [&](int n, int t, int ci) {
        const int nl = to_log(n);
        return (nl >= 0 && ci < cin) ? w[((size_t)nl * cin + ci) * taps + t] : 0.f;
    };
    int rc = pack_any(dtype, h->w, Np, taps * Kp, [&](int n, int k) { return WC(n, k / Kp, k % Kp); });
    rc |= upload_f32(h->b, Np, [&](int n) { const int nl = to_log(n); return nl >= 0 ? b[nl] : 0.f; });
    const bool f16 = rc == 0 && dtype == DCVC_F16;
    if (f16 && taps == 1 && epilogue != DCVC_EPI_SHUFFLE2 && Np == Kp && Np == round_up(cout, 64) && t128_width_ok(Np))
        rc |= pack_t128_matrix(h->w_t128, Np, Kp, [&](int n, int k) { return WC(n, 0, k); });
    if (f16 && kh == 3 && kw == 3 && stride == 1 && pad == 1 && Kp % 64 == 0 && Kp <= 256 && Np % 256 == 0 &&
        (epilogue == DCVC_EPI_BIAS || (epilogue == DCVC_EPI_SHUFFLE2 && h->cs_p % 256 == 0))) {
        rc |= pack_quarters(h->w_c128[0], Np / 128, 1, 9, Kp / 16, 4, WC);
        rc |= pack_quarters(h->w_c128[1], Np / 256, 2, 9, Kp / 16, 8, WC);
    }
    if (f16 && stride == 2 && ((kh == 2 && kw == 2 && pad == 0) || (kh == 3 && kw == 3 && pad == 1)) &&
        Kp % 128 == 0 && Kp <= 384 && (Np == 128 || Np == 256) && epilogue == DCVC_EPI_BIAS)
        rc |= pack_quarters(h->w_s2, 1, Np / 128, taps, Kp / 16, 8 * (Np / 128), WC);
    if (rc) return rc < 0 ? rc : dcvc::E_MEM;
    *out = h.release();
    return 0;
}

void dcvc_conv_destroy(dcvc_conv* h) { delete h; }

int dcvc_conv_forward(const dcvc_conv* h, const void* x0, int64_t ld0, int c0, const void* x1, int64_t ld1, int c1,
                      int H, int W, const float* quant, void* out, int64_t ldo, void* stream)
{
    return dcvc_conv_forward_scaled(h, x0, ld0, c0, x1, ld1, c1, H, W, nullptr, quant, out, ldo, stream);
}

int dcvc_conv_forward_scaled(const dcvc_conv* h, const void* x0, int64_t ld0, int c0, const void* x1, int64_t ld1, int c1,
                             int H, int W, const float* in_scale, const float* quant, void* out, int64_t ldo, void* stream)
{
    DCVC_REQUIRE(h && x0 && out, "dcvc_conv_forward: null pointer");
    DCVC_REQUIRE(h->epi != DCVC_EPI_BIAS_QUANT || quant != nullptr, "dcvc_conv_forward: quant vector required");
    ConvParams cp{};
    cp.src = SrcPair{x0, (long)ld0, c0, x1, (long)ld1, c1};
    if (int rc = check_src("dcvc_conv_forward", cp.src, h->cin_p, true, h->dtype, H, W)) return rc;
    cp.H = H;
    cp.W = W;
    cp.Ho = (H + 2 * h->pad - h->kh) / h->stride + 1;
    cp.Wo = (W + 2 * h->pad - h->kw) / h->stride + 1;
    DCVC_REQUIRE(cp.Ho > 0 && cp.Wo > 0, "dcvc_conv_forward: empty output");
    cp.KH = h->kh;
    cp.KW = h->kw;
    cp.stride = h->stride;
    cp.pad = h->pad;
    cp.N = h->n_p;
    cp.n_log = h->cout;
    cp.cs_p = h->cs_p;
    cp.w = h->w.p;
    cp.b = (const float*)h->b.p;
    cp.q = quant;
    cp.in_q = in_scale;
    cp.in_qn = h->cin;
    cp.epi = h->epi;
    cp.out = out;
    cp.ldo = ldo;
    DCVC_REQUIRE(ldo >= (h->epi == DCVC_EPI_SHUFFLE2 ? h->cs_p : h->n_p), "dcvc_conv_forward: output row stride too small");
    hipStream_t st = (hipStream_t)stream;
    return run_conv(h, cp, st);
}

}
```

opendcvc_amd/models.py:

```python
import ctypes
import functools
import os

import numpy as np
import torch
from torch import nn as tnn

from . import _lib, arch, entropy, handoff
from . import nn as L
from ._lib import DcvcError, check
from .entropy import CHUNK_LOG2_DEFAULT


def _register(root, dotted, tensor):
    parts = dotted.split(".")
    m = root
    for p in parts[:-1]:
        if not hasattr(m, p):
            m.add_module(p, tnn.Module())
        m = getattr(m, p)
    m.register_parameter(parts[-1], tnn.Parameter(tensor, requires_grad=False))


class _CaptureGuard:
# ... 226 lines not shown
    def load_state_dict(self, state_dict, *args, **kwargs):
        pre = "bit_estimator_z."
        z_in = {k[len(pre):]: v for k, v in state_dict.items() if k.startswith(pre) and torch.is_tensor(v)}
        res = super().load_state_dict(state_dict, *args, **kwargs)
        master = {k: v.detach().float().cpu().clone() for k, v in z_in.items() if v.dtype == torch.float32}
        if master:
            self._z_master = master
        elif z_in and self._z_master is not None:
            same = set(z_in) == set(self._z_master) and all(
                z_in[k].dtype == torch.float16 and z_in[k].shape == self._z_master[k].shape and
                torch.equal(z_in[k].detach().cpu(), self._z_master[k].half()) for k in z_in)
            if not same:
                self._z_master = None
        return res

    def set_use_two_entropy_coders(self, use_two_entropy_coders):
        self.entropy_coder.set_use_two_entropy_coders(use_two_entropy_coders)

    def _dtype_device(self):
        p = next(self.parameters())
        return p.dtype, p.device

    def _ensure_layers(self):
        dtype, device = self._dtype_device()
        if device.type != "cuda":
            raise DcvcError("the DCVC-RT hot path runs on an MI355X only: move the model to a cuda device "
                            "(there is no CPU fallback)")
        if self.entropy_coder is None:
            raise DcvcError("call update(force_zero_thres) before compress/decompress")
        key = (dtype, str(device))
        if self._layers_key != key:
            _lib.require_gpu()
            torch.cuda.set_device(device)
            sd = {k: v.detach().float().cpu() for k, v in self.state_dict().items()}
            self._layers = self._build_layers(sd, dtype)
            self._q = {k: v.reshape(v.shape[0], v.shape[1]).to(device=device, dtype=torch.float32).contiguous()
                       for k, v in sd.items() if k.startswith("q_")}
            self._layers_key = key
            self._graphs.clear()
            self._persist = {}
            names = sorted(self._q)
            self._q_cat = torch.cat([self._q[k] for k in names], dim=1).contiguous() if names else None
            self._q_row = torch.zeros_like(self._q_cat[0]) if names else None
            self._qv, off = {}, 0
            for k in names:
                n = self._q[k].shape[1]
                self._qv[k] = self._q_row[off:off + n]
                off += n
        return dtype, device

    def _stage_q(self, qp):
        row = self._q_cat[qp]
        check(_lib.lib().dcvc_copy_f32(L._p(self._q_row), L._p(row), row.numel(), self._stream()), "copy_f32")
        return self._qv

    def _buffer(self, name, shape, dtype, device):
        key = (name, tuple(shape), dtype)
        b = self._persist.get(key)
        if b is None:
            b = self._persist[key] = torch.zeros(shape, dtype=dtype, device=device)
        return b

    def _picture_out(self, head):
        return self._shuffle8_clamp(head)

    def _thres(self):
        return -1.0 if self.force_zero_thres is None else float(self.force_zero_thres)

    def _stream(self):
        return ctypes.c_void_p(torch.cuda.current_stream().cuda_stream)

    def _pad_for_y(self, y):
        H, W, C = y.shape
        pr, pb = self.get_padding_size(H, W, 4)
        if pr == 0 and pb == 0:
            return y
        out = torch.empty((H + pb, W + pr, C), dtype=y.dtype, device=y.device)
        check(_lib.lib().dcvc_replicate_pad_hwc(L.dtype_code(y.dtype), L._p(y), C, H, W, C, pb, pr, L._p(out), C,
                                                self._stream()), "replicate_pad")
        return out

    def _unshuffle8(self, x, out=None):
        _, C, H, W = x.shape
        x = x.contiguous()
        if out is None:
            out = torch.empty((H // 8, W // 8, C * 64), dtype=x.dtype, device=x.device)
        check(_lib.lib().dcvc_unshuffle8(L.dtype_code(x.dtype), L._p(x), C, H, W, L._p(out), C * 64, self._stream()),
              "unshuffle8")
        return out

    def _shuffle8_clamp(self, x, bias=None, out=None):
        H, W, C, ld = L._geom(x)
        if out is None:
            out = torch.empty((1, 3, H * 8, W * 8), dtype=x.dtype, device=x.device)
        check(_lib.lib().dcvc_shuffle8_clamp(L.dtype_code(x.dtype), L._p(x), ld, L._p(bias), 3, H, W, 1, L._p(out),
                                             self._stream()), "shuffle8_clamp")
        return out

    def _crop(self, x, H2, W2, out=None):
        H, W, C, ld = L._geom(x)
        if out is None:
            if (H, W) == (H2, W2):
                return x
            out = torch.empty((H2, W2, C), dtype=x.dtype, device=x.device)
        _, _, _, ldo = L._geom(out)
        check(_lib.lib().dcvc_crop_hwc(L.dtype_code(x.dtype), L._p(x), ld, W, H2, W2, C, L._p(out), ldo,
                                       self._stream()), "crop")
        return out

    def _quantize_z(self, z):
        H, W, C, ld = L._geom(z)
        z8 = torch.empty(C * H * W, dtype=torch.int8, device=z.device)
        check(_lib.lib().dcvc_round_z(L.dtype_code(z.dtype), L._p(z), ld, H, W, C, L._p(z8), self._stream()), "round_z")
        return z, z8

    def _z_to_device(self, z_pinned, zh, zw, dtype, device):
        out = torch.empty((zh, zw, self.z_channel), dtype=dtype, device=device)
        check(_lib.lib().dcvc_z_from_int8(L.dtype_code(dtype), ctypes.c_void_p(z_pinned.dptr), zh, zw, self.z_channel,
                                          L._p(out), self.z_channel, self._stream()), "z_from_int8")
        return out

    def _device_coder(self):
        if self._dev_coder is None:
            self._dev_coder = entropy.DeviceCoder(*self._g_tables)
        return self._dev_coder

    def _open_frame(self, bit_stream, sps, chunked, units, prefix):
        chunked = self.entropy == "device" if chunked is None else bool(chunked)
        return handoff.open_frame(self, bit_stream, sps, units, prefix, chunked, DEC_COMPACT)

    def _prior_enc_step(self, groups, step, q_mode, y, qsrc, scales, means, yhat, packed):
        H, W, C, ldy = L._geom(y)
        check(_lib.lib().dcvc_prior_enc_step(
            L.dtype_code(y.dtype), groups, step, q_mode, L._p(y), ldy, L._p(qsrc), qsrc.stride(1), L._p(scales),
            scales.stride(1), L._p(means), means.stride(1), H, W, C, self._thres(), L._p(yhat), yhat.stride(1),
            L._p(yhat), yhat.stride(1), L._p(packed), self._stream()), "prior_enc_step")

    def _prior_finish(self, q_mode, yhat, qsrc):
        H, W, C, ld = L._geom(yhat)
        check(_lib.lib().dcvc_prior_finish(L.dtype_code(yhat.dtype), q_mode, L._p(yhat), ld, L._p(qsrc), qsrc.stride(1),
                                           H, W, C, self._stream()), "prior_finish")



class DMC(CompressionModel):

    def __init__(self, entropy="host", chunk_log2=None):
        super().__init__("dmc", arch.DMC_CH_Z, arch.QP_NUM + arch.DMC_EXTRA_QP, entropy=entropy, chunk_log2=chunk_log2)
        self.qp_shift = list(arch.DMC_QP_SHIFT)
        self.dpb = []
        self.max_dpb_size = 1
        self.curr_poc = 0
        self._ahead = None
        self._pending = None
        self._stream_pending = None
        self._stream_parity = 0
        self._branch = None

    def _build_layers(self, sd, dt):
        D, C2, R = L.DepthConvBlock, L.Conv2d, L.ResidualBlockWithStride2
        n = {}
        n["fa_i"] = D(sd, "feature_adaptor_i", dt)
        fused = {"m" + k[len("feature_extractor.conv1.0"):]: v for k, v in sd.items() if k.startswith("feature_extractor.conv1.0.")}
        fused["m.adaptor.weight"], fused["m.adaptor.bias"] = sd["feature_adaptor_p.weight"], sd["feature_adaptor_p.bias"]
        n["fe1_p"] = [D(fused, "m", dt)]
        n["fe1"] = [D(sd, f"feature_extractor.conv1.{i}", dt) for i in range(2)]
        n["fe2"] = [D(sd, f"feature_extractor.conv2.{i}", dt) for i in range(4)]
        n["enc_conv1"] = C2(sd, "encoder.conv1", dt)
        n["enc_conv2"] = [D(sd, f"encoder.conv2.{i}", dt) for i in range(2)]
        n["enc_conv3"] = D(sd, "encoder.conv3", dt)
        n["enc_down"] = C2(sd, "encoder.down", dt, 2, 1)
        n["hyper_enc"] = [D(sd, "hyper_encoder.conv.0", dt), R(sd, "hyper_encoder.conv.1", dt), R(sd, "hyper_encoder.conv.2", dt)]
        n["hyper_dec"] = [L.ResidualBlockUpsample(sd, "hyper_decoder.conv.0", dt),
                          L.ResidualBlockUpsample(sd, "hyper_decoder.conv.1", dt), D(sd, "hyper_decoder.conv.2", dt)]
        n["temporal"] = R(sd, "temporal_prior_encoder", dt)
        n["fusion"] = [D(sd, f"y_prior_fusion.conv.{i}", dt) for i in range(3)]
        n["fusion_out"] = C2(sd, "y_prior_fusion.conv.3", dt)
        n["spatial"] = [D(sd, "y_spatial_prior.conv.0", dt), D(sd, "y_spatial_prior.conv.1", dt)]
        w, b = sd["y_spatial_prior.conv.2.weight"], sd["y_spatial_prior.conv.2.bias"]
        if w.shape[0] < w.shape[1] and w.shape[2:] == (1, 1):
            wp = torch.zeros((w.shape[1], w.shape[1], 1, 1), dtype=w.dtype)
            wp[:w.shape[0]] = w
            bp = torch.zeros(w.shape[1], dtype=b.dtype)
            bp[:b.shape[0]] = b
            n["spatial_out"] = C2({"c.weight": wp, "c.bias": bp}, "c", dt)
        else:
            n["spatial_out"] = C2(sd, "y_spatial_prior.conv.2", dt)
        n["dec_up"] = L.SubpelConv2x(sd, "decoder.up", dt, 1)
        n["dec_conv1"] = [D(sd, f"decoder.conv1.{i}", dt) for i in range(3)]
        n["dec_conv2"] = C2(sd, "decoder.conv2", dt, epilogue=_lib.EPI_BIAS_QUANT)
        n["recon"] = [D(sd, f"recon_generation_net.conv.{i}", dt) for i in range(4)]
        n["recon_head"] = C2(sd, "recon_generation_net.head", dt)
        return n

    def reset_ref_feature(self):
        self._ahead = None
        if len(self.dpb) > 0:
            self.dpb[0].feature = None

    def add_ref_frame(self, feature=None, frame=None, increase_poc=True):
        self._ahead = None
        ref = RefFrame()
        ref.poc = self.curr_poc
        ref.frame = frame
        ref.feature = feature
        if len(self.dpb) >= self.max_dpb_size:
            self.dpb.pop(-1)
        self.dpb.insert(0, ref)
        if increase_poc:
            self.curr_poc += 1

    def clear_dpb(self):
        self._ahead = None
        self.dpb.clear()

    def set_curr_poc(self, poc):
        self.curr_poc = poc

    def shift_qp(self, qp, fa_idx):
        return qp + self.qp_shift[fa_idx]

    def prepare_feature_adaptor_i(self, last_qp):
        if self.dpb[0].frame is None:
            self._ensure_layers()
            self.dpb[0].frame = self._recon(self.dpb[0].feature, self._q["q_recon"][last_qp])
            self.reset_ref_feature()

    def _fe1(self, variant):
        n = self._layers
        return n["fe1_p"] + n["fe1"][1:] if variant == "p" else [n["fa_i"]] + n["fe1"]

    def _fe_input(self, variant, ref_buf):
        return ref_buf if variant == "p" else self._unshuffle8(ref_buf)

    def _extractor_part1(self, variant, ref_buf):
        return L.dcb_chain(self._fe1(variant), self._fe_input(variant, ref_buf))

    def _extractor_part2(self, x1):
        return L.dcb_chain(self._layers["fe2"], x1)

    def _extractor_both(self, variant, ref_buf):
        blocks = self._fe1(variant)
        outs = L.dcb_chain(blocks + self._layers["fe2"], self._fe_input(variant, ref_buf), return_all=True)
        return outs[len(blocks) - 1], outs[-1]

    def _branch_stream(self, device):
        if self._branch is None:
            self._branch = torch.cuda.Stream(device)
        return self._branch

    def _prior_params(self, z_hat, x1, q_feature, yh, yw):
        n = self._layers
        cat = torch.empty((yh, yw, 3 * arch.DMC_CH_Y), dtype=z_hat.dtype, device=z_hat.device)
        main = torch.cuda.current_stream()
        side = self._branch_stream(z_hat.device) if _FORK else None
        if side is not None:
            side.wait_stream(main)
            with torch.cuda.stream(side):
                n["temporal"](x1, in_scale=q_feature, out=cat[:, :, arch.DMC_CH_Y:])
        h = n["hyper_dec"][1](n["hyper_dec"][0](z_hat))
        if h.shape[0] == yh and h.shape[1] == yw:
            n["hyper_dec"][2](h, out=cat[:, :, :arch.DMC_CH_Y])
        else:
            self._crop(n["hyper_dec"][2](h), yh, yw, out=cat[:, :, :arch.DMC_CH_Y])
        if side is not None:
            main.wait_stream(side)
        else:
            n["temporal"](x1, in_scale=q_feature, out=cat[:, :, arch.DMC_CH_Y:])
        return L.dcb_chain(n["fusion"], cat, then_conv=n["fusion_out"])

    def _spatial_prior(self, y_hat, params):
        n = self._layers
        return L.dcb_chain(n["spatial"], y_hat, params, then_conv=n["spatial_out"])

    def _decoder(self, y_hat, ctx, q_decoder, out=None):
        n = self._layers
        return L.dcb_chain(n["dec_conv1"], n["dec_up"](y_hat), ctx, then_conv=n["dec_conv2"], conv_quant=q_decoder, out=out)

    def _recon_head(self, feature, q_recon):
        n = self._layers
        o = L.dcb_chain(n["recon"], feature, quant=q_recon)
        return n["recon_head"](o)

    def _recon(self, feature, q_recon):
        return self._picture_out(self._recon_head(feature, q_recon))

    def _recon_first(self, feature):
        return L.dcb_chain(self._layers["recon"][:2], feature)

    def _recon_second(self, mid, q_recon):
        n = self._layers
        return n["recon_head"](L.dcb_chain(n["recon"][2:], mid, quant=q_recon))

    def _pending_half(self, which):
        pd = self._pending
        if pd is None:
            return
        if which == 0 and pd["mid"] is None:
            pd["mid"] = self._graphs.run(("dec_ra",) + pd["key"], lambda: self._recon_first(pd["feature"]))
        elif which == 1 and pd["mid"] is not None and pd["x_hat"] is None:
            mid, qrec = pd["mid"], pd["q_recon"]
            head = self._graphs.run(("dec_rb",) + pd["key"], lambda: self._recon_second(mid, qrec))
            pd["x_hat"] = self._picture_out(head)

    @_frame_scoped
    def finish_output(self):
        if self._pending is None:
            return None
        self._pending_half(0)
        self._pending_half(1)
        x_hat = self._pending["x_hat"]
        self._pending = None
        if self.dpb and self.dpb[0].frame is None:
            self.dpb[0].frame = x_hat
        return x_hat

    def _stage_reference(self, dtype, device):
        ref = self.dpb[0]
        if ref.feature is None:
            f = ref.frame
            buf = self._buffer("ref_frame", f.shape, dtype, device)
            buf.copy_(f, non_blocking=True)
            return "i", buf
        if ref.feature.data_ptr() != self._feature_buf(ref.feature.shape, dtype, device).data_ptr():
            self._feature_buf(ref.feature.shape, dtype, device).copy_(ref.feature, non_blocking=True)
        return "p", self._feature_buf(ref.feature.shape, dtype, device)

    def _feature_buf(self, shape, dtype, device):
        return self._buffer("feature", shape, dtype, device)

    @_frame_scoped
    def finish_stream(self):
        job, self._stream_pending = self._stream_pending, None
        return None if job is None else handoff.code(self, job)

    @_frame_scoped
    def compress(self, x, qp, defer_stream=False, chunked=None):
        dtype, device = self._ensure_layers()
        form = handoff.encoder_form(self, chunked)
        n = self._layers
        C = arch.DMC_CH_Y
        x = x.to(device=device, dtype=dtype)
        _, _, H, W = x.shape
        xin = self._buffer("x_unshuffled", (H // 8, W // 8, 192), dtype, device)
        self._unshuffle8(x, out=xin)
        q = self._stage_q(qp)
        variant, ref_buf = self._stage_reference(dtype, device)
        fbuf = self._feature_buf((H // 8, W // 8, arch.DMC_CH_D), dtype, device)
        key = (variant, H, W)
        ahead = self._ahead if (variant == "p" and self._ahead is not None and self._ahead[:2] == (H, W)) else None

        def front():
            if ahead is not None:
                x1, ctx = ahead[2], ahead[3]
            else:
                x1, ctx = self._extractor_both(variant, ref_buf)
            e = L.dcb_chain(n["enc_conv2"] + [n["enc_conv3"]], n["enc_conv1"](xin), ctx, quant=q["q_encoder"])
            y = n["enc_down"](e)
            yh, yw = y.shape[0], y.shape[1]
            z = n["hyper_enc"][2](n["hyper_enc"][1](n["hyper_enc"][0](self._pad_for_y(y))))
            z_hat, z8 = self._quantize_z(z)
            params = self._prior_params(z_hat, x1, q["q_feature"], yh, yw)
            nsym = (C // 2) * yh * yw
            y_hat = torch.empty((yh, yw, C), dtype=dtype, device=device)
            packed = torch.empty((2, nsym), dtype=torch.int16, device=device)
            self._prior_enc_step(2, 0, 0, y, params[:, :, :C], params[:, :, C:2 * C], params[:, :, 2 * C:], y_hat, packed[0])
            sp = self._spatial_prior(y_hat, params)
            self._prior_enc_step(2, 1, 0, y, params[:, :, :C], sp[:, :, :C], sp[:, :, C:], y_hat, packed[1])
            self._prior_finish(0, y_hat, params[:, :, :C])
            return y_hat, ctx, z8, packed, z.shape[0] * z.shape[1]

        y_hat, ctx, z8, packed, zhw = self._graphs.run(
            ("enc_front_ahead" if ahead is not None else "enc_front",) + key, front)
        par = self._stream_parity
        self._stream_parity ^= 1
        job = handoff.stage(self, f"enc{par}", form, z8, packed, qp, zhw)
        self._graphs.run(("enc_back", "ahead" if ahead is not None else "full") + key,
                         lambda: self._decoder(y_hat, ctx, q["q_decoder"], out=fbuf))
        nxt = None
        if self._graphs.enabled:
            def extractor_ahead():
                return self._extractor_both("p", fbuf)
            nxt = (H, W) + tuple(self._graphs.run(("enc_ahead", H, W), extractor_ahead))

        prev = self.finish_stream()
        self.add_ref_frame(fbuf, None)
        self._ahead = nxt
        mode = {} if form == handoff.REFERENCE else {"chunked": True}
        if job.est is not None:
            mode["est_bytes"] = handoff.estimated_bytes(self, job)
        if defer_stream:
            self._stream_pending = job
            return dict({"bit_stream": None, "bit_stream_prev": prev}, **mode)
        bit_stream = handoff.code(self, job)
        return dict({"bit_stream": bit_stream} if prev is None else {"bit_stream": bit_stream, "bit_stream_prev": prev}, **mode)

    @_frame_scoped
    def decompress(self, bit_stream, sps, qp, defer_output=False, chunked=None):
        dtype, device = self._ensure_layers()
        C = arch.DMC_CH_Y
        forced = None
        if self._pending is not None and (not defer_output or (self.dpb and self.dpb[0].feature is None)):
            forced = self.finish_output()
        prev = self._pending
        ec = self.entropy_coder
        fr = self._open_frame(bit_stream, sps, chunked, 2, "p")
        zh, zw = self.get_downsampled_shape(sps["height"], sps["width"], 64)
        yh, yw = self.get_downsampled_shape(sps["height"], sps["width"], 16)
        nz = self.z_channel * zh * zw
        ec.decode_z(nz, self._z_group, qp * self.z_channel, zh * zw)

        q = self._stage_q(qp)
        variant, ref_buf = self._stage_reference(dtype, device)
        fbuf = self._feature_buf((2 * yh, 2 * yw, arch.DMC_CH_D), dtype, device)
        key = (variant, sps["height"], sps["width"])
        zb = ec.pinned("z_dec", nz)

        x1 = self._graphs.run(("dec_0",) + key, lambda: self._extractor_part1(variant, ref_buf))
        ec.get_decoded(zb.view(np.int8, nz))
        fr.end_z()
        key = key + fr.suffix

        def after_z():
            z_hat = self._z_to_device(zb, zh, zw, dtype, device)
            params = self._prior_params(z_hat, x1, q["q_feature"], yh, yw)
            y_hat = torch.empty((yh, yw, C), dtype=dtype, device=device)
            return params, y_hat, fr.index(2, 0, params[:, :, C:2 * C], yh, yw, C)

        params, y_hat, st0 = self._graphs.run(("dec_1",) + key, after_z)
        ev = torch.cuda.Event()
        ev.record()
        ctx = self._graphs.run(("dec_2",) + key[:3], lambda: self._extractor_part2(x1))
        self._pending_half(0)
        if fr.host_waits:
            ev.synchronize()
        fr.decode(0, st0)

        def after_step0():
            fr.restore(st0, 2, 0, params[:, :, 2 * C:], y_hat, yh, yw, C, out=y_hat)
            sp = self._spatial_prior(y_hat, params)
            return sp, fr.index(2, 1, sp[:, :, :C], yh, yw, C)

        sp, st1 = self._graphs.run(("dec_3",) + key, after_step0)
        ev = torch.cuda.Event()
        ev.record()
        self._pending_half(1)
        if fr.host_waits:
            ev.synchronize()
        fr.decode(1, st1)

        def after_step1():
            y_fin = torch.empty_like(y_hat)
            fr.restore(st1, 2, 1, sp[:, :, C:], y_hat, yh, yw, C, out=y_fin)
            self._prior_finish(0, y_fin, params[:, :, :C])
            feature = self._decoder(y_fin, ctx, q["q_decoder"], out=fbuf)
            return None if defer_output else self._recon_head(feature, q["q_recon"])

        x_prev = None
        if prev is not None:
            x_prev = prev["x_hat"]
            self._pending = None
        head = self._graphs.run(("dec_4d" if defer_output else "dec_4",) + key, after_step1)
        x_hat = None if head is None else self._picture_out(head)
        try:
            fr.close()
        except DcvcError:
            if prev is not None:
                self._pending = prev
            raise
        self.add_ref_frame(fbuf, x_hat)
        if defer_output:
            qrec = self._buffer("q_recon_pending", q["q_recon"].shape, torch.float32, device)
            qrec.copy_(q["q_recon"], non_blocking=True)
            self._pending = dict(key=(sps["height"], sps["width"]), feature=fbuf, q_recon=qrec, mid=None, x_hat=None)
            return {"x_hat": None, "x_hat_prev": x_prev if x_prev is not None else forced}
        return {"x_hat": x_hat} if forced is None else {"x_hat": x_hat, "x_hat_prev": forced}


DMC.encode_one_frame = DMC.compress
DMC.decode_one_frame = DMC.decompress



class DMCI(CompressionModel):

    def __init__(self, N=arch.DMCI_N, z_channel=arch.DMCI_CH_Z, entropy="host", chunk_log2=None):
        if N != arch.DMCI_N or z_channel != arch.DMCI_CH_Z:
            raise DcvcError("only the published DCVC-RT-Intra configuration (N=256, z=128) is built")
        super().__init__("dmci", z_channel, arch.QP_NUM, entropy=entropy, chunk_log2=chunk_log2)

    def _build_layers(self, sd, dt):
        D, C2, R, U = L.DepthConvBlock, L.Conv2d, L.ResidualBlockWithStride2, L.ResidualBlockUpsample
        n = {}
        n["enc_1"] = D(sd, "enc.enc_1", dt)
        n["enc_2"] = [D(sd, f"enc.enc_2.{i}", dt) for i in range(6)]
        n["enc_down"] = C2(sd, "enc.enc_2.6", dt, 2, 1)
        n["hyper_enc"] = [D(sd, "hyper_enc.0", dt), R(sd, "hyper_enc.1", dt), R(sd, "hyper_enc.2", dt)]
        n["hyper_dec"] = [U(sd, "hyper_dec.0", dt), U(sd, "hyper_dec.1", dt), D(sd, "hyper_dec.2", dt)]
        n["fusion"] = [D(sd, f"y_prior_fusion.{i}", dt) for i in range(3)]
        n["fusion_out"] = C2(sd, "y_prior_fusion.3", dt)
        n["reduction"] = C2(sd, "y_spatial_prior_reduction", dt)
        n["sp_adaptor"] = [None] + [D(sd, f"y_spatial_prior_adaptor_{i}", dt) for i in (1, 2, 3)]
        n["spatial"] = [D(sd, f"y_spatial_prior.{i}", dt) for i in range(3)]
        n["spatial_out"] = C2(sd, "y_spatial_prior.3", dt)
        n["dec_up"] = U(sd, "dec.dec_1.0", dt)
        n["dec_1"] = [D(sd, f"dec.dec_1.{i}", dt) for i in range(1, 13)]
        n["dec_2"] = D(sd, "dec.dec_2", dt)
        return n

    def _enc(self, x, q):
        n = self._layers
        o = n["enc_1"](self._unshuffle8(x), quant=q)
        return n["enc_down"](L.dcb_chain(n["enc_2"], o))

    def _dec(self, y_hat, q):
        n = self._layers
        o = L.dcb_chain(n["dec_1"], n["dec_up"](y_hat), quant=q)
        return n["dec_2"](o)

    def _prior_params(self, z_hat, yh, yw):
        n = self._layers
        p = n["hyper_dec"][2](n["hyper_dec"][1](n["hyper_dec"][0](z_hat)))
        return self._crop(L.dcb_chain(n["fusion"], p, then_conv=n["fusion_out"]), yh, yw)

    def _spatial_prior(self, y_hat, common, step):
        n = self._layers
        return L.dcb_chain([n["sp_adaptor"][step]] + n["spatial"], y_hat, common, then_conv=n["spatial_out"])

    @_frame_scoped
    def compress(self, x, qp, chunked=None):
        dtype, device = self._ensure_layers()
        form = handoff.encoder_form(self, chunked)
        n = self._layers
        C = arch.DMCI_N
        x = x.to(device=device, dtype=dtype)
        _, _, H, W = x.shape
        xin = self._buffer("x_unshuffled", (H // 8, W // 8, 192), dtype, device)
        self._unshuffle8(x, out=xin)
        q = self._stage_q(qp)
        key = (H, W)

        def front():
            y = n["enc_down"](L.dcb_chain(n["enc_2"], n["enc_1"](xin, quant=q["q_scale_enc"])))
            yh, yw = y.shape[0], y.shape[1]
            z = n["hyper_enc"][2](n["hyper_enc"][1](n["hyper_enc"][0](self._pad_for_y(y))))
            z_hat, z8 = self._quantize_z(z)
            params = self._prior_params(z_hat, yh, yw)
            common = n["reduction"](params)
            scales, means = params[:, :, 2:2 + C], params[:, :, 2 + C:2 + 2 * C]
            nsym = (C // 4) * yh * yw
            y_hat = torch.empty((yh, yw, C), dtype=dtype, device=device)
            packed = torch.empty((4, nsym), dtype=torch.int16, device=device)
            self._prior_enc_step(4, 0, 1, y, params, scales, means, y_hat, packed[0])
            for step in (1, 2, 3):
                sp = self._spatial_prior(y_hat, common, step)
                self._prior_enc_step(4, step, 1, y, params, sp[:, :, :C], sp[:, :, C:], y_hat, packed[step])
            self._prior_finish(1, y_hat, params)
            return y_hat, z8, packed, z.shape[0] * z.shape[1]

        y_hat, z8, packed, zhw = self._graphs.run(("ienc_front",) + key, front)
        job = handoff.stage(self, "ienc", form, z8, packed, qp, zhw)
        x_hat = self._picture_out(self._graphs.run(("ienc_back",) + key, lambda: self._dec(y_hat, q["q_scale_dec"])))

        res = {"bit_stream": handoff.code(self, job), "x_hat": x_hat}
        if job.est is not None:
            res["est_bytes"] = handoff.estimated_bytes(self, job)
        return res if form == handoff.REFERENCE else dict(res, chunked=True)

    @_frame_scoped
    def decompress(self, bit_stream, sps, qp, chunked=None):
        dtype, device = self._ensure_layers()
        n = self._layers
        C = arch.DMCI_N
        ec = self.entropy_coder
        fr = self._open_frame(bit_stream, sps, chunked, 4, "i")
        zh, zw = self.get_downsampled_shape(sps["height"], sps["width"], 64)
        yh, yw = self.get_downsampled_shape(sps["height"], sps["width"], 16)
        nz = self.z_channel * zh * zw
        key = (sps["height"], sps["width"]) + fr.suffix
        q = self._stage_q(qp)
        ec.decode_z(nz, self._z_group, qp * self.z_channel, zh * zw)
        zb = ec.pinned("z_dec", nz)
        ec.get_decoded(zb.view(np.int8, nz))
        fr.end_z()

        def first():
            z_hat = self._z_to_device(zb, zh, zw, dtype, device)
            params = self._prior_params(z_hat, yh, yw)
            common = n["reduction"](params)
            return params, common, fr.index(4, 0, params[:, :, 2:2 + C], yh, yw, C)

        params, common, st = self._graphs.run(("idec_0",) + key, first)
        means = params[:, :, 2 + C:2 + 2 * C]
        y_prev = None
        for step in (0, 1, 2, 3):
            if fr.host_waits:
                ev = torch.cuda.Event()
                ev.record()
                ev.synchronize()
            fr.decode(step, st)

            def after(step=step, st=st, means=means, y_prev=y_prev):
                y_new = torch.empty((yh, yw, C), dtype=dtype, device=device)
                fr.restore(st, 4, step, means, y_new if y_prev is None else y_prev, yh, yw, C, out=y_new)
                if step == 3:
                    self._prior_finish(1, y_new, params)
                    return y_new, self._dec(y_new, q["q_scale_dec"])
                sp = self._spatial_prior(y_new, common, step + 1)
                return y_new, sp, fr.index(4, step + 1, sp[:, :, :C], yh, yw, C)

            res = self._graphs.run((f"idec_{step + 1}",) + key, after)
            if step == 3:
                x_hat = res[1]
            else:
                y_prev, sp, st = res
                means = sp[:, :, C:]
        x_hat = self._picture_out(x_hat)
        fr.close()
        return {"x_hat": x_hat}


DMCI.encode_one_frame = DMCI.compress
DMCI.decode_one_frame = DMCI.decompress
# ... 1 lines not shown
```

opendcvc_amd/nn.py:

```python
import ctypes

import numpy as np
import torch

from . import _lib
from ._lib import DcvcError, check

F16, F32 = _lib.F16, _lib.F32


def dtype_code(dt):
    if dt == torch.float16:
        return F16
    if dt == torch.float32:
        return F32
    raise DcvcError(f"unsupported dtype {dt}: the HIP path computes in float16 or float32")


def cpad(c, m=32):
    return (c + m - 1) // m * m


def _stream():
    return ctypes.c_void_p(torch.cuda.current_stream().cuda_stream)


def _p(t):
    return ctypes.c_void_p(t.data_ptr()) if t is not None else None


def _host(a):
    a = np.ascontiguousarray(a.detach().cpu().float().numpy() if isinstance(a, torch.Tensor) else a, dtype=np.float32)
    return a


def _hp(a):
    return a.ctypes.data_as(ctypes.c_void_p) if a is not None else None


def _geom(x):
    if x.dim() != 3 or x.stride(2) != 1 or x.stride(0) != x.shape[1] * x.stride(1):
        raise DcvcError(f"expected an HWC tensor with contiguous channels and uniform row stride, got "
                        f"shape {tuple(x.shape)} strides {tuple(x.stride())}")
    return x.shape[0], x.shape[1], x.shape[2], x.stride(1)


def _io(x0, x1, out, out_shape, dtype):
    for name, t in (("x0", x0), ("x1", x1), ("out", out)):
        if t is not None and t.dtype != dtype:
            raise DcvcError(f"{name} is {t.dtype}, the layer computes in {dtype}")
    H, W, c0, ld0 = _geom(x0)
    c1, ld1 = 0, 0
    if x1 is not None:
        H1, W1, c1, ld1 = _geom(x1)
        if (H1, W1) != (H, W):
            raise DcvcError(f"concat inputs differ in size: {(H, W)} and {(H1, W1)}")
    Ho, Wo, co = out_shape(H, W)
    if out is None:
        out = torch.empty((Ho, Wo, co), dtype=dtype, device=x0.device)
    H2, W2, c2, ldo = _geom(out)
    if (H2, W2) != (Ho, Wo) or c2 < co:
        raise DcvcError(f"output view {tuple(out.shape)} does not fit the layer's output {(Ho, Wo, co)}")
    return (_p(x0), ld0, c0, _p(x1), ld1, c1, H, W), out, ldo


class Scratch:
    _pool = {}
    _retired = []

    @classmethod
    def get(cls, nbytes, device):
        key = (str(device), torch.cuda.current_stream().cuda_stream)
        buf = cls._pool.get(key)
        if buf is None or buf.numel() < nbytes:
            if buf is not None:
                cls._retired.append(buf)
            buf = torch.empty(int(nbytes * 2) + 256, dtype=torch.uint8, device=device)
            cls._pool[key] = buf
        return buf


class DepthConvBlock:

    def __init__(self, sd, prefix, dtype, shortcut=False):
        L = _lib.lib()
        g = lambda n: _host(sd[prefix + n])
        self.has_adaptor = (prefix + ".adaptor.weight") in sd
        w1 = g(".dc.0.weight")
        self.c = w1.shape[0]
        wa = g(".adaptor.weight") if self.has_adaptor else None
        ba = g(".adaptor.bias") if self.has_adaptor else None
        self.cin = wa.shape[1] if self.has_adaptor else self.c
        self.c_p = cpad(self.c, 64)
        self.cin_p = cpad(self.cin, 32) if self.has_adaptor else self.c_p
        self.dtype = dtype
        self.shortcut = bool(shortcut)
        arrs = [wa, ba, w1, g(".dc.0.bias"), g(".dc.2.weight"), g(".dc.2.bias"), g(".dc.3.weight"),
                g(".dc.3.bias"), g(".ffn.0.weight"), g(".ffn.0.bias"), g(".ffn.2.weight"), g(".ffn.2.bias")]
        h = ctypes.c_void_p()
        check(L.dcvc_dcb_create(dtype_code(dtype), self.cin, self.c, int(shortcut), *[_hp(a) for a in arrs],
                                ctypes.byref(h)), "dcvc_dcb_create")
        self.h = h

    def __del__(self):
        try:
            if getattr(self, "h", None):
                _lib.lib().dcvc_dcb_destroy(self.h)
        except Exception:
            pass

    def __call__(self, x0, x1=None, quant=None, out=None, head_done=False, a_slot=0, next_block=None):
        L = _lib.lib()
        src, out, ldo = _io(x0, x1, out, lambda H, W: (H, W, self.c_p), self.dtype)
        scratch = Scratch.get(L.dcvc_dcb_scratch_bytes(self.h, *src[6:]), x0.device)
        check(L.dcvc_dcb_forward_chained(self.h, *src, _p(quant), _p(out), ldo, _p(scratch), _stream(), int(head_done),
                                         int(a_slot), next_block.h if next_block is not None else None), "dcvc_dcb_forward")
        return out

    def then_conv(self, x0, x1, conv, conv_quant=None, out=None, head_done=False, a_slot=0):
        L = _lib.lib()
        src, out, ldo = _io(x0, x1, out, lambda H, W: (H, W, conv.cout_p), self.dtype)
        scratch = Scratch.get(L.dcvc_dcb_scratch_bytes(self.h, *src[6:]), x0.device)
        check(L.dcvc_dcb_forward_then_conv(self.h, *src, _p(scratch), _stream(), int(head_done), int(a_slot), conv.h,
                                           _p(conv_quant), _p(out), ldo), "dcvc_dcb_forward_then_conv")
        return out

    def can_follow(self, prev, prev_quant):
        return (not self.has_adaptor and self.c_p == prev.c_p and self.dtype == prev.dtype and prev_quant is None
                and not prev.shortcut)


def dcb_chain(blocks, x0, x1=None, quant=None, out=None, return_all=False, then_conv=None, conv_quant=None):
    x = x0
    fused = False
    outs = []
    for i, b in enumerate(blocks):
        last = i + 1 == len(blocks)
        if last and then_conv is not None and quant is None and not return_all and then_conv.fusable_after(b):
            return b.then_conv(x, x1 if i == 0 else None, then_conv, conv_quant, out=out, head_done=fused, a_slot=i & 1)
        qi = quant if last else None
        nxt = None if last or not blocks[i + 1].can_follow(b, qi) else blocks[i + 1]
        x = b(x, x1 if i == 0 else None, quant=qi, out=out if (last and then_conv is None) else None, head_done=fused, a_slot=i & 1,
              next_block=nxt)
        fused = nxt is not None
        outs.append(x)
    if then_conv is not None:
        return then_conv(x, quant=conv_quant, out=out)
    return outs if return_all else x


class Conv2d:

    def __init__(self, sd, prefix, dtype, stride=1, pad=0, epilogue=_lib.EPI_BIAS):
        L = _lib.lib()
        w = _host(sd[prefix + ".weight"])
        b = _host(sd[prefix + ".bias"])
        self.cout, self.cin, self.kh, self.kw = w.shape
        self.stride, self.pad, self.epi, self.dtype = stride, pad, epilogue, dtype
        self.cin_p = cpad(self.cin, 32)
        if epilogue == _lib.EPI_SHUFFLE2:
            self.cout_p = cpad(self.cout // 4, 32)
        else:
            self.cout_p = cpad(self.cout, 32)
        h = ctypes.c_void_p()
        check(L.dcvc_conv_create(dtype_code(dtype), self.cin, self.cout, self.kh, self.kw, stride, pad, epilogue,
                                 _hp(w), _hp(b), ctypes.byref(h)), "dcvc_conv_create")
        self.h = h

    def __del__(self):
        try:
            if getattr(self, "h", None):
                _lib.lib().dcvc_conv_destroy(self.h)
        except Exception:
            pass

    def fusable_after(self, block):
        return (self.kh == 1 and self.kw == 1 and self.stride == 1 and self.pad == 0 and self.cin == block.c and
                self.cin_p == block.c_p and self.cout_p == block.c_p and self.dtype == block.dtype and
                not block.shortcut and self.epi in (_lib.EPI_BIAS, _lib.EPI_BIAS_QUANT))

    def out_hw(self, H, W):
        Ho = (H + 2 * self.pad - self.kh) // self.stride + 1
        Wo = (W + 2 * self.pad - self.kw) // self.stride + 1
        if self.epi == _lib.EPI_SHUFFLE2:
            return 2 * Ho, 2 * Wo
        return Ho, Wo

    def __call__(self, x0, x1=None, quant=None, out=None, in_scale=None):
        L = _lib.lib()
        if in_scale is not None and (in_scale.dtype != torch.float32 or in_scale.numel() < self.cin):
            raise DcvcError(f"in_scale must be a float32 vector of at least {self.cin} entries")
        src, out, ldo = _io(x0, x1, out, lambda H, W: (*self.out_hw(H, W), self.cout_p), self.dtype)
        check(L.dcvc_conv_forward_scaled(self.h, *src, _p(in_scale), _p(quant), _p(out), ldo, _stream()), "dcvc_conv_forward")
        return out


class SubpelConv2x:

    def __init__(self, sd, prefix, dtype, pad):
        self.conv = Conv2d(sd, prefix + ".conv.0", dtype, 1, pad, _lib.EPI_SHUFFLE2)
        self.cout_p = self.conv.cout_p

    def __call__(self, x, out=None):
        return self.conv(x, out=out)


class ResidualBlockWithStride2:

    def __init__(self, sd, prefix, dtype):
        self.down = Conv2d(sd, prefix + ".down", dtype, 2, 0)
        self.conv = DepthConvBlock(sd, prefix + ".conv", dtype, shortcut=True)

    def __call__(self, x, out=None, in_scale=None):
        return self.conv(self.down(x, in_scale=in_scale), out=out)


class ResidualBlockUpsample:

    def __init__(self, sd, prefix, dtype):
        self.up = SubpelConv2x(sd, prefix + ".up", dtype, 0)
        self.conv = DepthConvBlock(sd, prefix + ".conv", dtype, shortcut=True)

    def __call__(self, x, out=None):
        return self.conv(self.up(x), out=out)



def to_hwc(x_nchw, c_phys=None):
    L = _lib.lib()
    _, C, H, W = x_nchw.shape
    cp_ = c_phys or cpad(C)
    x = x_nchw.contiguous()
    out = torch.zeros((H, W, cp_), dtype=x.dtype, device=x.device) if cp_ != C else \
        torch.empty((H, W, cp_), dtype=x.dtype, device=x.device)
    check(L.dcvc_nchw_to_hwc(dtype_code(x.dtype), _p(x), C, H * W, _p(out), cp_, _stream()), "dcvc_nchw_to_hwc")
    return out


def to_nchw(x_hwc, C=None):
    L = _lib.lib()
    H, W, cp_, ld = _geom(x_hwc)
    C = C or cp_
    out = torch.empty((1, C, H, W), dtype=x_hwc.dtype, device=x_hwc.device)
    check(L.dcvc_hwc_to_nchw(dtype_code(x_hwc.dtype), _p(x_hwc), ld, C, H * W, _p(out), _stream()), "dcvc_hwc_to_nchw")
    return out
```

Measured before the change: 433.8.

## Chain multiple successor stages inside the DCB tail kernel and carry heads across graphs

Extends the tail128 kernel with a multi-stage mode that, after the block's own output, runs up to three chained 1x1 GEMM stages (a following conv, the next block's adaptor, the next block's head) from LDS without writing intermediates to global memory. The host planner builds these stages, falls back to separate conv or head-only launches when fusion is not possible, and the Python chain/carry logic lets a block's head be computed ahead into a carried scratch buffer across graph segments. The aim is fewer kernel launches and less global round-tripping between the decoder, extractor and following blocks. The multi-stage path is gated behind a DCVC_STAGES switch for mismatched cases and adds register/LDS pressure plus more complex scratch-slot bookkeeping.

```diff
diff --git a/include/dcvc_amd.h b/include/dcvc_amd.h
--- a/include/dcvc_amd.h
+++ b/include/dcvc_amd.h
@@ -48,6 +48,13 @@
                                int64_t ld1, int c1, int H, int W, void* scratch, void* stream,
                                int head_done, int a_slot, const dcvc_conv* conv, const float* conv_quant,
                                void* conv_out, int64_t ldco);
+
+size_t dcvc_dcb_fused_scratch_bytes(const dcvc_dcb* h, int H, int W);
+int dcvc_dcb_forward_fused(const dcvc_dcb* h, const void* x0, int64_t ld0, int c0, const void* x1, int64_t ld1,
+                           int c1, int H, int W, const float* quant, void* out, int64_t ldo, void* scratch,
+                           void* stream, int head_done, int a_slot, const dcvc_conv* conv,
+                           const float* conv_quant, void* conv_out, int64_t ldco, const dcvc_dcb* next,
+                           void* succ_scratch);
 
 int dcvc_dcb_profile(const dcvc_dcb* h, const void* x0, int64_t ld0, int c0, int H, int W, void* out,
                      int64_t ldo, void* scratch, void* stream, int iters, float* head_ms, float* tail_ms);
diff --git a/opendcvc_amd/_lib.py b/opendcvc_amd/_lib.py
--- a/opendcvc_amd/_lib.py
+++ b/opendcvc_amd/_lib.py
@@ -51,6 +51,8 @@
     "dcvc_dcb_forward": (_I, [_P, _P, _L, _I, _P, _L, _I, _I, _I, _P, _P, _L, _P, _P]),
     "dcvc_dcb_forward_chained": (_I, [_P, _P, _L, _I, _P, _L, _I, _I, _I, _P, _P, _L, _P, _P, _I, _I, _P]),
     "dcvc_dcb_forward_then_conv": (_I, [_P, _P, _L, _I, _P, _L, _I, _I, _I, _P, _P, _I, _I, _P, _P, _P, _L]),
+    "dcvc_dcb_fused_scratch_bytes": (c_size_t, [_P, _I, _I]),
+    "dcvc_dcb_forward_fused": (_I, [_P, _P, _L, _I, _P, _L, _I, _I, _I, _P, _P, _L, _P, _P, _I, _I, _P, _P, _P, _L, _P, _P]),
     "dcvc_dcb_profile": (_I, [_P, _P, _L, _I, _I, _I, _P, _L, _P, _P, _I, POINTER(c_float), POINTER(c_float)]),
     "dcvc_dcb_profile_tail": (_I, [_P, _P, _L, _I, _I, _I, _P, _L, _P, _P, _I, POINTER(c_float)]),
     "dcvc_conv_create": (_I, [_I, _I, _I, _I, _I, _I, _I, _I, _P, _P, POINTER(_P)]),
diff --git a/opendcvc_amd/csrc/dcb_t128.hpp b/opendcvc_amd/csrc/dcb_t128.hpp
--- a/opendcvc_amd/csrc/dcb_t128.hpp
+++ b/opendcvc_amd/csrc/dcb_t128.hpp
@@ -77,8 +77,8 @@
 }
 
 
-template <int C, class G = G128, bool HEADIN = false>
-__global__ __launch_bounds__(Geo<G>::NTHR, G::WPS) void dcb_tail128_kernel(TailParams p)
+template <int C, class G = G128, bool HEADIN = false, bool MULTI = false>
+__global__ __launch_bounds__(Geo<G>::NTHR, G::WPS) void dcb_tail128_kernel(typename std::conditional<MULTI, TailParamsMulti, TailParams>::type p)
 {
     using TR = Traits<half_t>;
     using CF = Cfg<C, G, HEADIN>;
@@ -543,9 +543,17 @@
 #undef T128_OFF
 
     STAMP(ts5);
-    const bool fused_next = p.nwt != nullptr;
-    const __amdgpu_buffer_rsrc_t nrsrc = __builtin_amdgcn_make_buffer_rsrc(
-        const_cast<char*>(reinterpret_cast<const char*>(fused_next ? p.nwt : p.wt)) + (size_t)cqw * (KS * NTW + PADF) * 1024, 0,
+    int nstage;
+    const void* first_wt;
+    if constexpr (MULTI) {
+        nstage = p.nstage;
+        first_wt = p.stage[0].wt;
+    } else {
+        nstage = p.nwt != nullptr ? 1 : 0;
+        first_wt = p.nwt;
+    }
+    __amdgpu_buffer_rsrc_t nrsrc = __builtin_amdgcn_make_buffer_rsrc(
+        const_cast<char*>(reinterpret_cast<const char*>(nstage > 0 ? first_wt : p.wt)) + (size_t)cqw * (KS * NTW + PADF) * 1024, 0,
         (KS * NTW + PADF) * 1024, 0x00020000);
     int noff = 0;
     auto nload = [&]() __attribute__((always_inline)) {
@@ -554,7 +562,7 @@
         noff += 1024;
         return __builtin_bit_cast(half8, v);
     };
-    if (fused_next) {
+    if (nstage > 0) {
 #pragma unroll
         for (int k = 0; k < D; ++k) ring[k] = nload();
     }
@@ -575,7 +583,7 @@
     }
     __syncthreads();
     half_t* out = reinterpret_cast<half_t*>(p.out);
-    if (out != nullptr) {
+    if (out != nullptr || (MULTI && p.q != nullptr)) {
 #pragma unroll
         for (int k = 0; k < NID; ++k) {
             int m, icg;
@@ -595,9 +603,11 @@
 #pragma unroll
                     for (int j = 0; j < V; ++j) r[j] = r[j] * ((icg + j) < p.c_log ? p.q[icg + j] : 1.0f);
                 }
-                *reinterpret_cast<Vec16*>(out + pix * p.ldo + icg) = pack16<half_t>(r);
-            }
-        }
+                if (!MULTI || out != nullptr) *reinterpret_cast<Vec16*>(out + pix * p.ldo + icg) = pack16<half_t>(r);
+                else lds_store_vec<half_t>(bufX, LDX, m, icg, pack16<half_t>(r));
+            }
+        }
+        if (MULTI && out == nullptr) __syncthreads();
     }
     STAMP(ts6);
 #ifdef DCVC_DIAG
@@ -621,8 +631,16 @@
         o[13] = ts1 - td[4];
     }
 #endif
-    if (fused_next) {
+    auto stage = [&](const TailStage sg, const void* next_wt) __attribute__((always_inline)) {
         gemm_c(nload);
+        if (MULTI && next_wt != nullptr) {
+            nrsrc = __builtin_amdgcn_make_buffer_rsrc(
+                const_cast<char*>(reinterpret_cast<const char*>(next_wt)) + (size_t)cqw * (KS * NTW + PADF) * 1024, 0,
+                (KS * NTW + PADF) * 1024, 0x00020000);
+            noff = 0;
+#pragma unroll
+            for (int k = 0; k < D; ++k) ring[k] = nload();
+        }
         __syncthreads();
 #pragma unroll
         for (int i = 0; i < NTW; ++i) {
@@ -631,19 +649,18 @@
 #pragma unroll
             for (int g = 0; g < 4; ++g) {
                 const int ch0 = chb + 8 * g;
-                const floatx4 bias = load_f4(p.nb1 + ch0);
+                const floatx4 bias = load_f4(sg.bias + ch0);
                 floatx4 qv = {1.f, 1.f, 1.f, 1.f};
-                if (p.nplain && p.nq != nullptr) {
-#pragma unroll
-                    for (int r = 0; r < 4; ++r) qv[r] = (ch0 + r) < p.n_log ? p.nq[ch0 + r] : 1.0f;
+                if (sg.q != nullptr) {
+#pragma unroll
+                    for (int r = 0; r < 4; ++r) qv[r] = (ch0 + r) < sg.q_log ? sg.q[ch0 + r] : 1.0f;
                 }
 #pragma unroll
                 for (int t = 0; t < PTW; ++t) {
                     floatx4 v = {acc[i][t][4 * g], acc[i][t][4 * g + 1], acc[i][t][4 * g + 2], acc[i][t][4 * g + 3]};
                     v = v + bias;
-                    if (p.nplain) {
-                        if (p.nq != nullptr) v = v * qv;
-                    } else {
+                    if (sg.q != nullptr) v = v * qv;
+                    if (sg.gate) {
 #pragma unroll
                         for (int r = 0; r < 4; ++r) v[r] = TR::gate(v[r]);
                     }
@@ -652,15 +669,22 @@
             }
         }
         __syncthreads();
-        half_t* na = reinterpret_cast<half_t*>(p.na_out);
+        half_t* so = reinterpret_cast<half_t*>(sg.out);
 #pragma unroll
         for (int k = 0; k < NID; ++k) {
             int m, icg;
             idmap(k, m, icg);
             const int y = ty0 + m / TW, x = tx0 + m % TW;
-            if (y < p.H && x < p.W)
-                *reinterpret_cast<Vec16*>(na + ((long)y * p.W + x) * p.nlda + icg) = lds_load_vec<half_t>(bufX, LDX, m, icg);
-        }
+            if (y < p.H && x < p.W && icg < sg.nstore)
+                *reinterpret_cast<Vec16*>(so + ((long)y * p.W + x) * sg.ld + icg) = lds_load_vec<half_t>(bufX, LDX, m, icg);
+        }
+    };
+    if constexpr (MULTI) {
+#pragma nounroll
+        for (int s = 0; s < nstage; ++s) stage(p.stage[s], s + 1 < nstage ? p.stage[s + 1].wt : nullptr);
+    } else {
+        if (nstage > 0)
+            stage(TailStage{p.nwt, p.nb1, p.nplain ? p.nq : nullptr, p.n_log, !p.nplain, p.na_out, p.nlda, C}, nullptr);
     }
 #ifdef DCVC_DIAG
     if (p.stamps && tid == 0) {
diff --git a/opendcvc_amd/csrc/dcvc_nn.hip b/opendcvc_amd/csrc/dcvc_nn.hip
--- a/opendcvc_amd/csrc/dcvc_nn.hip
+++ b/opendcvc_amd/csrc/dcvc_nn.hip
@@ -175,6 +175,18 @@
                 lds_load_vec<T>(bufX, ldx, m, c);
     }
 }
+
+struct TailStage {
+    const void* wt;
+    const float* bias;
+    const float* q;
+    int q_log;
+    int gate;
+    void* out;
+    long ld;
+    int nstore;
+};
+constexpr int MAX_STAGES = 3;
 
 struct TailParams {
     const void* a;
@@ -212,6 +224,11 @@
     unsigned long long* stamps;
 };
 
+struct TailParamsMulti : TailParams {
+    int nstage;
+    TailStage stage[MAX_STAGES];
+};
+
 #ifdef DCVC_DIAG
 #define ABLATED(bit) ((p.ablate & (bit)) != 0)
 #define STAMP(var)                                                   \
@@ -896,6 +913,7 @@
     int dtype, cin, cout, cin_p, n_p, cs_p, kh, kw, stride, pad, epi;
     DevBuf w, b;
     DevBuf w_t128;
+    DevBuf b_t128;
     DevBuf w_c128[2];
     DevBuf w_s2;
 };
@@ -1008,7 +1026,7 @@
 }
 
 struct Switches {
-    bool t128, t32, h128, c128;
+    bool t128, t32, h128, c128, stages;
 #ifdef DCVC_DIAG
     int mt, conv_mt, ablate;
     bool stamps;
@@ -1025,6 +1043,7 @@
         s.t32 = on("DCVC_T32");
         s.h128 = on("DCVC_H128");
         s.c128 = on("DCVC_C128");
+        s.stages = on("DCVC_STAGES");
 #ifdef DCVC_DIAG
         s.mt = num("DCVC_MT");
         s.conv_mt = num("DCVC_CONV_MT");
@@ -1130,15 +1149,25 @@
 }
 #endif
 
+inline bool needs_multi(const TailParamsMulti& tp)
+{
+    return tp.nstage >= 2 || (tp.nstage == 1 && tp.stage[0].nstore != tp.C) || (tp.out == nullptr && tp.q != nullptr);
+}
+
 template <int C, class G = t128::G128, bool HEADIN = false>
-int launch_tail128(const TailParams& tp, int H, int W, hipStream_t st)
+int launch_tail128(const TailParamsMulti& tp, int H, int W, hipStream_t st)
 {
     const int grid = tile_grid(H, W, G::TH, G::TW);
     const size_t lds = t128::Cfg<C, G, HEADIN>::LDS;
 #ifdef DCVC_DIAG
     if (switches().stamps) return stamped_tail128<C, G, HEADIN>(tp, grid, lds, st);
 #endif
-    return launch_kernel(t128::dcb_tail128_kernel<C, G, HEADIN>, dim3(grid), t128::Geo<G>::NTHR, lds, st, tp);
+    if (needs_multi(tp)) {
+        if constexpr (!HEADIN) return launch_kernel(t128::dcb_tail128_kernel<C, G, false, true>, dim3(grid), t128::Geo<G>::NTHR, lds, st, tp);
+        dcvc::set_error("dcb_tail128_kernel<..., HEADIN> runs at most one successor stage");
+        return dcvc::E_ARG;
+    }
+    return launch_kernel(t128::dcb_tail128_kernel<C, G, HEADIN>, dim3(grid), t128::Geo<G>::NTHR, lds, st, static_cast<const TailParams&>(tp));
 }
 
 template <typename T, int MT, int NTW, int NW, bool RAG = false, bool HEADIN = false>
@@ -1159,6 +1188,8 @@
     const float* conv_q = nullptr;
     void* conv_out = nullptr;
     int64_t ldco = 0;
+    void* succ = nullptr;
+    int head_only = 0;
 };
 
 static int pick_mt_f16(int H, int W)
@@ -1198,10 +1229,10 @@
     bool headin = false;
     int mt = 2, ntw = 1;
     TailForm form{1, 4, false};
-    const void* nwt = nullptr;
+    bool fused = false;
 };
 
-static DcbPlan plan_dcb(const dcvc_dcb* h, const SrcPair& src, int H, int W, const ChainArgs& ch)
+static DcbPlan plan_dcb(const dcvc_dcb* h, const SrcPair& src, int H, int W, const ChainArgs& ch, bool quant = false)
 {
     const Switches& sw = switches();
     const bool f16 = h->dtype == DCVC_F16;
@@ -1209,8 +1240,12 @@
     pl.mt = f16 ? pick_mt_f16(H, W) : 2;
     pl.ntw = h->c_p / 64;
     const int mt = pl.mt, ntw = pl.ntw;
-    pl.nwt = ch.next ? ch.next->w1_t128.p : ch.conv ? ch.conv->w_t128.p : nullptr;
-    const bool t128 = sw.t128 && h->wt128.p != nullptr && (pl.nwt != nullptr || (!ch.next && !ch.conv));
+    const bool want = ch.next || ch.conv;
+    const bool single = want && !(ch.next && ch.conv) && !quant && !ch.succ &&
+                        (ch.next ? !ch.next->adapt : ch.conv->n_p == h->c_p);
+    const bool streams = (!ch.conv || (ch.conv->w_t128.p != nullptr && ch.conv->b_t128.p != nullptr)) &&
+                         (!ch.next || (ch.next->w1_t128.p != nullptr && (!ch.next->adapt || ch.next->wa_t128.p != nullptr)));
+    const bool t128 = sw.t128 && h->wt128.p != nullptr && (!want || (streams && (single || sw.stages)));
     const bool own_head = !ch.head_done && !ch.separate_head && !h->adapt && src.c1 == 0;
 
     if (has_tail128(f16, mt, ntw, true) && t128 && sw.t32 && h->w1_t128.p != nullptr && own_head) {
@@ -1223,6 +1258,8 @@
         pl.headin = has_tail_headin(f16, mt, ntw) && own_head;
         pl.form = tail_form(f16, ntw);
     }
+
+    pl.fused = want && (single || (pl.tail == DcbPlan::Tail::tail128 && !pl.headin));
 
     const int kin = src.c0 + src.c1;
     if (ch.head_done || pl.headin) {
@@ -1259,8 +1296,10 @@
     const size_t P = (size_t)H * W;
     T* slots = reinterpret_cast<T*>(scratch);
     T* a_buf = slots + (size_t)(ch.a_slot & 1) * P * C;
-    T* a_next = slots + (size_t)((ch.a_slot & 1) ^ 1) * P * C;
+    T* succ = ch.succ ? reinterpret_cast<T*>(ch.succ) : slots;
+    T* a_next = succ + (size_t)((ch.a_slot & 1) ^ 1) * P * C;
     T* id_buf = slots + 2 * P * C;
+    T* id_next = succ + 2 * P * C;
     HeadParams hp{};
     hp.src = src;
     hp.H = H;
@@ -1277,7 +1316,7 @@
     hp.split = src.c1 > 0;
     hp.wa128 = h->wa_t128.p;
     hp.w1128 = h->w1_t128.p;
-    TailParams tp{};
+    TailParamsMulti tp{};
     tp.a = a_buf;
     tp.lda = C;
     tp.ident = h->adapt ? (const void*)id_buf : src.x0;
@@ -1304,8 +1343,24 @@
     tp.hb1 = (const float*)h->b1.p;
     tp.hwt = h->w1_t128.p;
     tp.wt = h->wt128.p;
-    tp.nwt = pl.nwt;
-    if (ch.next) {
+    if (pl.tail == DcbPlan::Tail::tail128 && pl.fused) {
+        auto stage = [&](const void* wt, const void* bias, const float* q, int q_log, int gate, void* o, long ld, int nstore) {
+            tp.stage[tp.nstage++] = TailStage{wt, (const float*)bias, q, q_log, gate, o, ld, nstore};
+        };
+        if (ch.conv) stage(ch.conv->w_t128.p, ch.conv->b_t128.p, ch.conv_q, ch.conv->cout, 0, ch.conv_out, (long)ch.ldco, ch.conv->n_p);
+        if (ch.next && ch.next->adapt) stage(ch.next->wa_t128.p, ch.next->ba.p, nullptr, 0, 0, id_next, C, C);
+        if (ch.next) stage(ch.next->w1_t128.p, ch.next->b1.p, nullptr, 0, 1, a_next, C, C);
+        if (!needs_multi(tp)) {
+            const TailStage& s0 = tp.stage[0];
+            tp.nwt = s0.wt;
+            tp.nb1 = s0.bias;
+            tp.na_out = s0.out;
+            tp.nlda = s0.ld;
+            tp.nplain = !s0.gate;
+            tp.nq = s0.q;
+            tp.n_log = s0.q_log;
+        }
+    } else if (ch.next) {
         tp.nw1 = ch.next->w1.p;
         tp.nb1 = (const float*)ch.next->b1.p;
         tp.na_out = a_next;
@@ -1348,6 +1403,7 @@
     if (rc) return rc;
     DCVC_LAUNCH_CHECK();
     if (ev) DCVC_HIP(hipEventRecord(ev[1], st));
+    if (ch.head_only) return 0;
 
     if (pl.tail == DcbPlan::Tail::tail128) {
         if (pl.headin) {
@@ -1388,13 +1444,57 @@
     }
 }
 
-static int run_dcb(const dcvc_dcb* h, const SrcPair& src, int H, int W, const float* quant, void* out, int64_t ldo,
-                   void* scratch, hipStream_t st, hipEvent_t* ev, ChainArgs ch = ChainArgs())
-{
-    const DcbPlan pl = plan_dcb(h, src, H, W, ch);
+static int run_planned(const DcbPlan& pl, const dcvc_dcb* h, const SrcPair& src, int H, int W, const float* quant, void* out,
+                       int64_t ldo, void* scratch, hipStream_t st, hipEvent_t* ev, const ChainArgs& ch)
+{
     if (h->dtype != DCVC_F16) return dispatch_dcb<float, 2>(pl, h, src, H, W, quant, out, ldo, scratch, st, ev, ch);
     if (pl.mt == 2) return dispatch_dcb<half_t, 2>(pl, h, src, H, W, quant, out, ldo, scratch, st, ev, ch);
     return dispatch_dcb<half_t, 4>(pl, h, src, H, W, quant, out, ldo, scratch, st, ev, ch);
+}
+
+static int run_conv1x1(const dcvc_conv* h, const void* x, int64_t ldx, int H, int W, const float* quant, void* out, int64_t ldo,
+                       hipStream_t st);
+
+static int run_dcb(const dcvc_dcb* h, const SrcPair& src, int H, int W, const float* quant, void* out, int64_t ldo,
+                   void* scratch, hipStream_t st, hipEvent_t* ev, ChainArgs ch = ChainArgs())
+{
+    ChainArgs own = ch;
+    DcbPlan pl = plan_dcb(h, src, H, W, own, quant != nullptr);
+    if (own.next && own.conv && !pl.fused) {
+        own.next = nullptr;
+        own.succ = nullptr;
+        pl = plan_dcb(h, src, H, W, own, quant != nullptr);
+    }
+    if ((own.next || own.conv) && !pl.fused) {
+        own.next = nullptr;
+        own.succ = nullptr;
+        own.conv = nullptr;
+        pl = plan_dcb(h, src, H, W, own, quant != nullptr);
+    }
+    const size_t es = dcvc::elem_size(h->dtype);
+    if (out == nullptr && !own.conv) {
+        out = reinterpret_cast<char*>(scratch) + (size_t)3 * H * W * h->c_p * es;
+        ldo = h->c_p;
+    }
+    if (int rc = run_planned(pl, h, src, H, W, quant, own.conv ? nullptr : out, ldo, scratch, st, ev, own)) return rc;
+    const void* x = out;
+    int64_t ldx = ldo;
+    if (ch.conv) {
+        if (!own.conv)
+            if (int rc = run_conv1x1(ch.conv, x, ldx, H, W, ch.conv_q, ch.conv_out, ch.ldco, st)) return rc;
+        x = ch.conv_out;
+        ldx = ch.ldco;
+    }
+    if (ch.next && !own.next) {
+        const SrcPair nsrc{x, (long)ldx, ch.next->cin_p, nullptr, 0, 0};
+        ChainArgs hc;
+        hc.separate_head = 1;
+        hc.head_only = 1;
+        hc.a_slot = (ch.a_slot & 1) ^ 1;
+        const DcbPlan hpl = plan_dcb(ch.next, nsrc, H, W, hc);
+        return run_planned(hpl, ch.next, nsrc, H, W, nullptr, nullptr, 0, ch.succ ? ch.succ : scratch, st, nullptr, hc);
+    }
+    return 0;
 }
 
 template <typename T, int MT, int NTW>
@@ -1521,13 +1621,47 @@
                  "%s: input channels %d+%d do not match the layer (%d physical)", who, s.c0, s.c1, cin_p);
     DCVC_REQUIRE((s.x1 != nullptr) == (s.c1 > 0), "%s: x1/c1 mismatch", who);
     DCVC_REQUIRE(two_ok || s.c1 == 0, "%s: a block without adaptor takes a single source", who);
-    DCVC_REQUIRE(!head_done || !two_ok, "%s: a block with adaptor computes its own head", who);
+    DCVC_REQUIRE(!head_done || !two_ok || (s.c1 == 0 && cin_p % 64 == 0),
+                 "%s: a block with a two-source adaptor computes its own head", who);
     DCVC_REQUIRE(s.ld0 >= s.c0 && (s.c1 == 0 || s.ld1 >= s.c1), "%s: input row stride too small", who);
     const size_t es = dcvc::elem_size(dtype);
     DCVC_REQUIRE(((uintptr_t)s.x0 % 16) == 0 && (s.ld0 * es) % 16 == 0 &&
                      (s.c1 == 0 || (((uintptr_t)s.x1 % 16) == 0 && (s.ld1 * es) % 16 == 0)),
                  "%s: inputs must be 16-byte aligned", who);
     return 0;
+}
+
+static ConvParams conv_params(const dcvc_conv* h, const SrcPair& src, int H, int W, const float* in_scale, const float* quant,
+                              void* out, int64_t ldo)
+{
+    ConvParams cp{};
+    cp.src = src;
+    cp.H = H;
+    cp.W = W;
+    cp.Ho = (H + 2 * h->pad - h->kh) / h->stride + 1;
+    cp.Wo = (W + 2 * h->pad - h->kw) / h->stride + 1;
+    cp.KH = h->kh;
+    cp.KW = h->kw;
+    cp.stride = h->stride;
+    cp.pad = h->pad;
+    cp.N = h->n_p;
+    cp.n_log = h->cout;
+    cp.cs_p = h->cs_p;
+    cp.w = h->w.p;
+    cp.b = (const float*)h->b.p;
+    cp.q = quant;
+    cp.in_q = in_scale;
+    cp.in_qn = h->cin;
+    cp.epi = h->epi;
+    cp.out = out;
+    cp.ldo = ldo;
+    return cp;
+}
+
+static int run_conv1x1(const dcvc_conv* h, const void* x, int64_t ldx, int H, int W, const float* quant, void* out, int64_t ldo,
+                       hipStream_t st)
+{
+    return run_conv(h, conv_params(h, SrcPair{x, (long)ldx, h->cin_p, nullptr, 0, 0}, H, W, nullptr, quant, out, ldo), st);
 }
 
 }
@@ -1642,6 +1776,54 @@
     ch.conv_out = conv_out;
     ch.ldco = ldco;
     return run_dcb(h, src, H, W, nullptr, nullptr, 0, scratch, (hipStream_t)stream, nullptr, ch);
+}
+
+size_t dcvc_dcb_fused_scratch_bytes(const dcvc_dcb* h, int H, int W)
+{
+    if (!h) return 0;
+    return (size_t)H * W * h->c_p * dcvc::elem_size(h->dtype) * 4;
+}
+
+int dcvc_dcb_forward_fused(const dcvc_dcb* h, const void* x0, int64_t ld0, int c0, const void* x1, int64_t ld1, int c1,
+                           int H, int W, const float* quant, void* out, int64_t ldo, void* scratch, void* stream,
+                           int head_done, int a_slot, const dcvc_conv* conv, const float* conv_quant, void* conv_out,
+                           int64_t ldco, const dcvc_dcb* next, void* succ_scratch)
+{
+    DCVC_REQUIRE(h && x0 && scratch && (out || conv), "dcvc_dcb_forward_fused: null pointer");
+    DCVC_REQUIRE(!(conv || next) || !h->shortcut, "dcvc_dcb_forward_fused: a block with shortcut cannot feed a fused successor");
+    DCVC_REQUIRE(!quant || conv || !next, "dcvc_dcb_forward_fused: a quant step feeds a conv, not a block's head");
+    DCVC_REQUIRE(!head_done || !h->adapt || h->cin_p == h->c_p, "dcvc_dcb_forward_fused: head_done needs a square adaptor");
+    const size_t es = dcvc::elem_size(h->dtype);
+    if (conv) {
+        DCVC_REQUIRE(conv_out, "dcvc_dcb_forward_fused: null pointer");
+        DCVC_REQUIRE(conv->dtype == h->dtype && conv->kh == 1 && conv->kw == 1 && conv->stride == 1 && conv->pad == 0 &&
+                         conv->cin_p == h->c_p && conv->n_p <= h->c_p && conv->cin == h->c &&
+                         (conv->epi == DCVC_EPI_BIAS || conv->epi == DCVC_EPI_BIAS_QUANT),
+                     "dcvc_dcb_forward_fused: the conv must be 1x1, stride 1, of the block's input width and no wider (%d -> %d "
+                     "given, block %d), epilogue bias or bias*quant", conv->cin, conv->cout, h->c);
+        DCVC_REQUIRE((conv->epi == DCVC_EPI_BIAS_QUANT) == (conv_quant != nullptr), "dcvc_dcb_forward_fused: quant vector / epilogue mismatch");
+        DCVC_REQUIRE(ldco >= conv->n_p && ((uintptr_t)conv_out % 16) == 0 && (ldco * es) % 16 == 0,
+                     "dcvc_dcb_forward_fused: conv output row stride too small or not 16-byte aligned");
+    }
+    if (next)
+        DCVC_REQUIRE(next->c_p == h->c_p && next->dtype == h->dtype && next->cin_p == (conv ? conv->n_p : h->c_p) &&
+                         (!next->adapt || next->cin_p == next->c_p),
+                     "dcvc_dcb_forward_fused: cannot compute the next block's head (needs same width and type; an adaptor "
+                     "there must be square)");
+    const SrcPair src{x0, (long)ld0, c0, x1, (long)ld1, c1};
+    if (int rc = check_src("dcvc_dcb_forward_fused", src, h->cin_p, h->adapt != 0, h->dtype, H, W, head_done != 0)) return rc;
+    DCVC_REQUIRE(!out || (ldo >= h->c_p && ((uintptr_t)out % 16) == 0 && (ldo * es) % 16 == 0),
+                 "dcvc_dcb_forward_fused: output row stride too small or not 16-byte aligned");
+    ChainArgs ch;
+    ch.head_done = head_done;
+    ch.a_slot = a_slot;
+    ch.next = next;
+    ch.conv = conv;
+    ch.conv_q = conv_quant;
+    ch.conv_out = conv_out;
+    ch.ldco = ldco;
+    ch.succ = succ_scratch;
+    return run_dcb(h, src, H, W, quant, conv ? nullptr : out, ldo, scratch, (hipStream_t)stream, nullptr, ch);
 }
 
 int dcvc_dcb_profile(const dcvc_dcb* h, const void* x0, int64_t ld0, int c0, int H, int W, void* out, int64_t ldo,
@@ -1741,8 +1923,10 @@
     int rc = pack_any(dtype, h->w, Np, taps * Kp, [&](int n, int k) { return WC(n, k / Kp, k % Kp); });
     rc |= upload_f32(h->b, Np, [&](int n) { const int nl = to_log(n); return nl >= 0 ? b[nl] : 0.f; });
     const bool f16 = rc == 0 && dtype == DCVC_F16;
-    if (f16 && taps == 1 && epilogue != DCVC_EPI_SHUFFLE2 && Np == Kp && Np == round_up(cout, 64) && t128_width_ok(Np))
-        rc |= pack_t128_matrix(h->w_t128, Np, Kp, [&](int n, int k) { return WC(n, 0, k); });
+    if (f16 && taps == 1 && stride == 1 && pad == 0 && epilogue != DCVC_EPI_SHUFFLE2 && Np <= Kp && Kp % 64 == 0 && t128_width_ok(Kp)) {
+        rc |= pack_t128_matrix(h->w_t128, Kp, Kp, [&](int n, int k) { return WC(n, 0, k); });
+        rc |= upload_f32(h->b_t128, Kp, [&](int n) { return n < cout ? b[n] : 0.f; });
+    }
     if (f16 && kh == 3 && kw == 3 && stride == 1 && pad == 1 && Kp % 64 == 0 && Kp <= 256 && Np % 256 == 0 &&
         (epilogue == DCVC_EPI_BIAS || (epilogue == DCVC_EPI_SHUFFLE2 && h->cs_p % 256 == 0))) {
         rc |= pack_quarters(h->w_c128[0], Np / 128, 1, 9, Kp / 16, 4, WC);
@@ -1769,29 +1953,10 @@
 {
     DCVC_REQUIRE(h && x0 && out, "dcvc_conv_forward: null pointer");
     DCVC_REQUIRE(h->epi != DCVC_EPI_BIAS_QUANT || quant != nullptr, "dcvc_conv_forward: quant vector required");
-    ConvParams cp{};
-    cp.src = SrcPair{x0, (long)ld0, c0, x1, (long)ld1, c1};
-    if (int rc = check_src("dcvc_conv_forward", cp.src, h->cin_p, true, h->dtype, H, W)) return rc;
-    cp.H = H;
-    cp.W = W;
-    cp.Ho = (H + 2 * h->pad - h->kh) / h->stride + 1;
-    cp.Wo = (W + 2 * h->pad - h->kw) / h->stride + 1;
+    const SrcPair src{x0, (long)ld0, c0, x1, (long)ld1, c1};
+    if (int rc = check_src("dcvc_conv_forward", src, h->cin_p, true, h->dtype, H, W)) return rc;
+    const ConvParams cp = conv_params(h, src, H, W, in_scale, quant, out, ldo);
     DCVC_REQUIRE(cp.Ho > 0 && cp.Wo > 0, "dcvc_conv_forward: empty output");
-    cp.KH = h->kh;
-    cp.KW = h->kw;
-    cp.stride = h->stride;
-    cp.pad = h->pad;
-    cp.N = h->n_p;
-    cp.n_log = h->cout;
-    cp.cs_p = h->cs_p;
-    cp.w = h->w.p;
-    cp.b = (const float*)h->b.p;
-    cp.q = quant;
-    cp.in_q = in_scale;
-    cp.in_qn = h->cin;
-    cp.epi = h->epi;
-    cp.out = out;
-    cp.ldo = ldo;
     DCVC_REQUIRE(ldo >= (h->epi == DCVC_EPI_SHUFFLE2 ? h->cs_p : h->n_p), "dcvc_conv_forward: output row stride too small");
     hipStream_t st = (hipStream_t)stream;
     return run_conv(h, cp, st);
diff --git a/opendcvc_amd/models.py b/opendcvc_amd/models.py
--- a/opendcvc_amd/models.py
+++ b/opendcvc_amd/models.py
@@ -402,6 +402,7 @@
         self.max_dpb_size = 1
         self.curr_poc = 0
         self._ahead = None
+        self._fe1_carry = None
         self._pending = None
         self._stream_pending = None
         self._stream_parity = 0
@@ -444,12 +445,12 @@
         return n
 
     def reset_ref_feature(self):
-        self._ahead = None
+        self._ahead = self._fe1_carry = None
         if len(self.dpb) > 0:
             self.dpb[0].feature = None
 
     def add_ref_frame(self, feature=None, frame=None, increase_poc=True):
-        self._ahead = None
+        self._ahead = self._fe1_carry = None
         ref = RefFrame()
         ref.poc = self.curr_poc
         ref.frame = frame
@@ -461,7 +462,7 @@
             self.curr_poc += 1
 
     def clear_dpb(self):
-        self._ahead = None
+        self._ahead = self._fe1_carry = None
         self.dpb.clear()
 
     def set_curr_poc(self, poc):
@@ -483,11 +484,23 @@
     def _fe_input(self, variant, ref_buf):
         return ref_buf if variant == "p" else self._unshuffle8(ref_buf)
 
-    def _extractor_part1(self, variant, ref_buf):
-        return L.dcb_chain(self._fe1(variant), self._fe_input(variant, ref_buf))
-
-    def _extractor_part2(self, x1):
-        return L.dcb_chain(self._layers["fe2"], x1)
+    def _carry(self, name, block, H, W, device, slot=0):
+        nbytes = _lib.lib().dcvc_dcb_scratch_bytes(block.h, H, W)
+        return L.Carry(block, self._buffer("carry_" + name, (nbytes,), torch.uint8, device), slot)
+
+    def _extractor_part1(self, variant, ref_buf, carried_slot=None):
+        xin = self._fe_input(variant, ref_buf)
+        H, W = xin.shape[0], xin.shape[1]
+        blocks = self._fe1(variant)
+        carry = self._carry("fe2", self._layers["fe2"][0], H, W, xin.device)
+        carried = None if carried_slot is None else self._carry("fe1", blocks[0], H, W, xin.device, carried_slot)
+        x1 = L.dcb_chain(blocks, xin, carry=carry, carried=carried)
+        return x1, carry.slot
+
+    def _extractor_part2(self, x1, slot=None):
+        fe2 = self._layers["fe2"]
+        carried = None if slot is None else self._carry("fe2", fe2[0], x1.shape[0], x1.shape[1], x1.device, slot)
+        return L.dcb_chain(fe2, x1, carried=carried)
 
     def _extractor_both(self, variant, ref_buf):
         blocks = self._fe1(variant)
@@ -523,24 +536,40 @@
         n = self._layers
         return L.dcb_chain(n["spatial"], y_hat, params, then_conv=n["spatial_out"])
 
-    def _decoder(self, y_hat, ctx, q_decoder, out=None):
-        n = self._layers
-        return L.dcb_chain(n["dec_conv1"], n["dec_up"](y_hat), ctx, then_conv=n["dec_conv2"], conv_quant=q_decoder, out=out)
+    def _decoder(self, y_hat, ctx, q_decoder, out=None, head_ahead=False, extractor_ahead=None):
+        n = self._layers
+        up = n["dec_up"](y_hat)
+        if extractor_ahead is not None:
+            blocks = self._fe1("p") + n["fe2"]
+            H, W = up.shape[0], up.shape[1]
+            outs = [None] * len(blocks)
+            outs[len(blocks) - len(n["fe2"]) - 1] = self._buffer(f"ahead_x1_{extractor_ahead}", (H, W, blocks[0].c_p), up.dtype, up.device)
+            outs[-1] = self._buffer(f"ahead_ctx_{extractor_ahead}", (H, W, blocks[-1].c_p), up.dtype, up.device)
+            f, outs = L.dcb_chain(n["dec_conv1"], up, ctx, then_conv=n["dec_conv2"], conv_quant=q_decoder, out=out,
+                                  then_blocks=blocks, then_outs=outs)
+            return f, outs[len(blocks) - len(n["fe2"]) - 1], outs[-1]
+        if head_ahead:
+            carry = self._carry("fe1", n["fe1_p"][0], up.shape[0], up.shape[1], up.device)
+            f = L.dcb_chain(n["dec_conv1"], up, ctx, then_conv=n["dec_conv2"], conv_quant=q_decoder, out=out, carry=carry)
+            return f, carry.slot
+        return L.dcb_chain(n["dec_conv1"], up, ctx, then_conv=n["dec_conv2"], conv_quant=q_decoder, out=out)
 
     def _recon_head(self, feature, q_recon):
         n = self._layers
-        o = L.dcb_chain(n["recon"], feature, quant=q_recon)
-        return n["recon_head"](o)
+        return L.dcb_chain(n["recon"], feature, quant=q_recon, then_conv=n["recon_head"])
 
     def _recon(self, feature, q_recon):
         return self._picture_out(self._recon_head(feature, q_recon))
 
     def _recon_first(self, feature):
-        return L.dcb_chain(self._layers["recon"][:2], feature)
-
-    def _recon_second(self, mid, q_recon):
-        n = self._layers
-        return n["recon_head"](L.dcb_chain(n["recon"][2:], mid, quant=q_recon))
+        recon = self._layers["recon"]
+        carry = self._carry("recon", recon[2], feature.shape[0], feature.shape[1], feature.device)
+        return L.dcb_chain(recon[:2], feature, carry=carry), carry.slot
+
+    def _recon_second(self, mid, slot, q_recon):
+        n = self._layers
+        carried = self._carry("recon", n["recon"][2], mid.shape[0], mid.shape[1], mid.device, slot)
+        return L.dcb_chain(n["recon"][2:], mid, quant=q_recon, then_conv=n["recon_head"], carried=carried)
 
     def _pending_half(self, which):
         pd = self._pending
@@ -549,8 +578,8 @@
         if which == 0 and pd["mid"] is None:
             pd["mid"] = self._graphs.run(("dec_ra",) + pd["key"], lambda: self._recon_first(pd["feature"]))
         elif which == 1 and pd["mid"] is not None and pd["x_hat"] is None:
-            mid, qrec = pd["mid"], pd["q_recon"]
-            head = self._graphs.run(("dec_rb",) + pd["key"], lambda: self._recon_second(mid, qrec))
+            (mid, slot), qrec = pd["mid"], pd["q_recon"]
+            head = self._graphs.run(("dec_rb",) + pd["key"], lambda: self._recon_second(mid, slot, qrec))
             pd["x_hat"] = self._picture_out(head)
 
     @_frame_scoped
@@ -620,18 +649,20 @@
             self._prior_finish(0, y_hat, params[:, :, :C])
             return y_hat, ctx, z8, packed, z.shape[0] * z.shape[1]
 
+        akey = key if ahead is None else key + (ahead[4],)
         y_hat, ctx, z8, packed, zhw = self._graphs.run(
-            ("enc_front_ahead" if ahead is not None else "enc_front",) + key, front)
+            ("enc_front_ahead" if ahead is not None else "enc_front",) + akey, front)
         par = self._stream_parity
         self._stream_parity ^= 1
         job = handoff.stage(self, f"enc{par}", form, z8, packed, qp, zhw)
-        self._graphs.run(("enc_back", "ahead" if ahead is not None else "full") + key,
-                         lambda: self._decoder(y_hat, ctx, q["q_decoder"], out=fbuf))
         nxt = None
         if self._graphs.enabled:
-            def extractor_ahead():
-                return self._extractor_both("p", fbuf)
-            nxt = (H, W) + tuple(self._graphs.run(("enc_ahead", H, W), extractor_ahead))
+            aset = 0 if ahead is None else 1 - ahead[4]
+            res = self._graphs.run(("enc_back", "ahead" if ahead is not None else "full") + akey,
+                                   lambda: self._decoder(y_hat, ctx, q["q_decoder"], out=fbuf, extractor_ahead=aset))
+            nxt = (H, W) + tuple(res[1:]) + (aset,)
+        else:
+            self._decoder(y_hat, ctx, q["q_decoder"], out=fbuf)
 
         prev = self.finish_stream()
         self.add_ref_frame(fbuf, None)
@@ -661,14 +692,21 @@
         ec.decode_z(nz, self._z_group, qp * self.z_channel, zh * zw)
 
         q = self._stage_q(qp)
+        fbuf = self._feature_buf((2 * yh, 2 * yw, arch.DMC_CH_D), dtype, device)
+        own_ref = self.dpb[0].feature is not None and self.dpb[0].feature.data_ptr() == fbuf.data_ptr()
         variant, ref_buf = self._stage_reference(dtype, device)
-        fbuf = self._feature_buf((2 * yh, 2 * yw, arch.DMC_CH_D), dtype, device)
         key = (variant, sps["height"], sps["width"])
         zb = ec.pinned("z_dec", nz)
 
-        x1 = self._graphs.run(("dec_0",) + key, lambda: self._extractor_part1(variant, ref_buf))
+        fc, self._fe1_carry = self._fe1_carry, None
+        cs = fc[2] if (variant == "p" and own_ref and fc is not None and fc[:2] == (sps["height"], sps["width"])) else None
+        x1, fe2_slot = self._graphs.run(("dec_0" if cs is None else "dec_0c",) + key + (() if cs is None else (cs,)),
+                                        lambda: self._extractor_part1(variant, ref_buf, carried_slot=cs))
+        if cs is not None:
+            key = key + ("c",)
         ec.get_decoded(zb.view(np.int8, nz))
         fr.end_z()
+        key_x = key
         key = key + fr.suffix
 
         def after_z():
@@ -680,7 +718,7 @@
         params, y_hat, st0 = self._graphs.run(("dec_1",) + key, after_z)
         ev = torch.cuda.Event()
         ev.record()
-        ctx = self._graphs.run(("dec_2",) + key[:3], lambda: self._extractor_part2(x1))
+        ctx = self._graphs.run(("dec_2",) + key_x, lambda: self._extractor_part2(x1, fe2_slot))
         self._pending_half(0)
         if fr.host_waits:
             ev.synchronize()
@@ -703,14 +741,14 @@
             y_fin = torch.empty_like(y_hat)
             fr.restore(st1, 2, 1, sp[:, :, C:], y_hat, yh, yw, C, out=y_fin)
             self._prior_finish(0, y_fin, params[:, :, :C])
-            feature = self._decoder(y_fin, ctx, q["q_decoder"], out=fbuf)
-            return None if defer_output else self._recon_head(feature, q["q_recon"])
+            feature, slot = self._decoder(y_fin, ctx, q["q_decoder"], out=fbuf, head_ahead=True)
+            return (None if defer_output else self._recon_head(feature, q["q_recon"])), slot
 
         x_prev = None
         if prev is not None:
             x_prev = prev["x_hat"]
             self._pending = None
-        head = self._graphs.run(("dec_4d" if defer_output else "dec_4",) + key, after_step1)
+        head, fe1_slot = self._graphs.run(("dec_4d" if defer_output else "dec_4",) + key, after_step1)
         x_hat = None if head is None else self._picture_out(head)
         try:
             fr.close()
@@ -719,6 +757,7 @@
                 self._pending = prev
             raise
         self.add_ref_frame(fbuf, x_hat)
+        self._fe1_carry = (sps["height"], sps["width"], fe1_slot)
         if defer_output:
             qrec = self._buffer("q_recon_pending", q["q_recon"].shape, torch.float32, device)
             qrec.copy_(q["q_recon"], non_blocking=True)
diff --git a/opendcvc_amd/nn.py b/opendcvc_amd/nn.py
--- a/opendcvc_amd/nn.py
+++ b/opendcvc_amd/nn.py
@@ -125,27 +125,91 @@
                                            _p(conv_quant), _p(out), ldo), "dcvc_dcb_forward_then_conv")
         return out
 
-    def can_follow(self, prev, prev_quant):
-        return (not self.has_adaptor and self.c_p == prev.c_p and self.dtype == prev.dtype and prev_quant is None
-                and not prev.shortcut)
-
-
-def dcb_chain(blocks, x0, x1=None, quant=None, out=None, return_all=False, then_conv=None, conv_quant=None):
+    def run(self, x0, x1=None, quant=None, out=None, head_done=False, a_slot=0, next_block=None, conv=None, conv_quant=None,
+            scratch=None, succ=None):
+        if (scratch is None and succ is None and not (head_done and self.has_adaptor) and
+                (next_block is None or not next_block.has_adaptor) and
+                (conv is None or (quant is None and next_block is None and conv.fusable_after(self)))):
+            if conv is not None:
+                return self.then_conv(x0, x1, conv, conv_quant, out=out, head_done=head_done, a_slot=a_slot)
+            return self(x0, x1, quant=quant, out=out, head_done=head_done, a_slot=a_slot, next_block=next_block)
+        L = _lib.lib()
+        co = conv.cout_p if conv is not None else self.c_p
+        src, out, ldo = _io(x0, x1, out, lambda H, W: (H, W, co), self.dtype)
+        shared = Scratch.get(L.dcvc_dcb_fused_scratch_bytes(self.h, *src[6:]), x0.device)
+        if scratch is not None and succ is None:
+            succ = shared
+        if scratch is None:
+            scratch = shared
+        need = (L.dcvc_dcb_fused_scratch_bytes if conv is not None else L.dcvc_dcb_scratch_bytes)(self.h, *src[6:])
+        for name, t, nbytes in (("scratch", scratch, need), ("succ", succ, L.dcvc_dcb_scratch_bytes(self.h, *src[6:]))):
+            if t is not None and t.numel() * t.element_size() < nbytes:
+                raise DcvcError(f"{name} buffer too small for a {src[6]}x{src[7]} map")
+        blk_out = (None, 0) if conv is not None else (_p(out), ldo)
+        conv_args = (conv.h, _p(conv_quant), _p(out), ldo) if conv is not None else (None, None, None, 0)
+        check(L.dcvc_dcb_forward_fused(self.h, *src, _p(quant), *blk_out, _p(scratch), _stream(), int(head_done), int(a_slot),
+                                       *conv_args, next_block.h if next_block is not None else None, _p(succ)),
+              "dcvc_dcb_forward_fused")
+        return out
+
+    def carry_buffer(self, H, W, device):
+        return torch.empty(_lib.lib().dcvc_dcb_scratch_bytes(self.h, H, W), dtype=torch.uint8, device=device)
+
+    def can_follow(self, prev, prev_quant, conv=None):
+        if self.c_p != prev.c_p or self.dtype != prev.dtype or prev.shortcut:
+            return False
+        if conv is None:
+            return not self.has_adaptor and prev_quant is None
+        return self.cin_p == conv.cout_p and self.cin_p == self.c_p
+
+
+class Carry:
+
+    def __init__(self, block, buf, slot=0):
+        self.block, self.buf, self.slot = block, buf, slot
+
+
+def dcb_chain(blocks, x0, x1=None, quant=None, out=None, return_all=False, then_conv=None, conv_quant=None, then_blocks=None,
+              then_outs=None, carry=None, carried=None):
+    if then_blocks and then_conv is None:
+        raise DcvcError("dcb_chain: then_blocks continue from then_conv's output")
+    if carried is not None and carried.block is not blocks[0]:
+        raise DcvcError("dcb_chain: the carry holds another block's head")
+    seq = list(blocks) + list(then_blocks or [])
+    nb = len(blocks)
+    base = carried.slot if carried is not None else 0
     x = x0
-    fused = False
+    fused = carried is not None
     outs = []
-    for i, b in enumerate(blocks):
-        last = i + 1 == len(blocks)
-        if last and then_conv is not None and quant is None and not return_all and then_conv.fusable_after(b):
-            return b.then_conv(x, x1 if i == 0 else None, then_conv, conv_quant, out=out, head_done=fused, a_slot=i & 1)
-        qi = quant if last else None
-        nxt = None if last or not blocks[i + 1].can_follow(b, qi) else blocks[i + 1]
-        x = b(x, x1 if i == 0 else None, quant=qi, out=out if (last and then_conv is None) else None, head_done=fused, a_slot=i & 1,
-              next_block=nxt)
+    conv_out = None
+    for i, b in enumerate(seq):
+        end = i + 1 == len(seq)
+        conv_here = then_conv is not None and i == nb - 1
+        qi = quant if i == nb - 1 else None
+        conv = then_conv if conv_here and not return_all and then_conv.fusable_behind(b) else None
+        nxt = carry.block if end and carry is not None else None if end else seq[i + 1]
+        if nxt is not None and ((conv_here and conv is None) or not nxt.can_follow(b, qi, conv)):
+            if end:
+                raise DcvcError("dcb_chain: this run cannot compute the carried block's head")
+            nxt = None
+        oi = out if (i == nb - 1 and (conv is not None or not conv_here)) else then_outs[i - nb] if (i >= nb and then_outs) else None
+        x = b.run(x, x1 if i == 0 else None, quant=qi, out=oi,
+                  head_done=fused, a_slot=(base + i) & 1, next_block=nxt, conv=conv, conv_quant=conv_quant if conv is not None else None,
+                  scratch=carried.buf if carried is not None and i == 0 else None,
+                  succ=carry.buf if end and carry is not None else None)
+        if conv_here and conv is None:
+            x = then_conv(x, quant=conv_quant, out=out)
+        if conv_here:
+            conv_out = x
+        else:
+            outs.append(x)
         fused = nxt is not None
-        outs.append(x)
+    if carry is not None:
+        carry.slot = (base + len(seq)) & 1
+    if then_blocks:
+        return conv_out, outs[nb - 1:]
     if then_conv is not None:
-        return then_conv(x, quant=conv_quant, out=out)
+        return conv_out
     return outs if return_all else x
 
 
@@ -179,6 +243,11 @@
                 self.cin_p == block.c_p and self.cout_p == block.c_p and self.dtype == block.dtype and
                 not block.shortcut and self.epi in (_lib.EPI_BIAS, _lib.EPI_BIAS_QUANT))
 
+    def fusable_behind(self, block):
+        return (self.kh == 1 and self.kw == 1 and self.stride == 1 and self.pad == 0 and self.cin == block.c and
+                self.cin_p == block.c_p and self.cout_p <= block.c_p and self.dtype == block.dtype and
+                not block.shortcut and self.epi in (_lib.EPI_BIAS, _lib.EPI_BIAS_QUANT))
+
     def out_hw(self, H, W):
         Ho = (H + 2 * self.pad - self.kh) // self.stride + 1
         Wo = (W + 2 * self.pad - self.kw) // self.stride + 1
```

After: 441.4, median of 6. +1.8%, better.
